# vibevoice-community/VibeVoice

Hardware: AMD Instinct MI355X
Metric: audio-sec/wall-sec (higher is better)
Workload: dtype bf16

## Files before the change

include/vvhip.h:

```cpp
#ifndef VVHIP_H
#define VVHIP_H
#include <stdint.h>
#ifdef __cplusplus
extern "C" {
#endif
typedef struct vv_ctx vv_ctx;

typedef struct vv_config {
    int lm_hidden, lm_layers, lm_heads, lm_kv_heads, lm_head_dim, lm_inter, lm_vocab;
    float lm_eps;
    int head_layers, head_ffn, latent_dim;
    float head_eps;
    int n_filters, n_ratios, ratios[8];
    int n_stages, enc_depths[8];
    int sem_dim;
    int has_acoustic_encoder;
    float codec_eps;
    int n_slots;
    int max_ctx;
    int max_rows;
    int xsplit;
    int attn_splits;
    int enc_frames;
    int use_graph;
// ... 56 lines not shown
int vv_diffusion_sample_rows(vv_ctx*, void* stream, int n, const float* cond_dev, const float* noise_dev,
                             const float* step_noise_dev, const float* cfg_rows_dev, float* latent_out_dev);
int vv_set_schedule_general(vv_ctx* ctx, int n_steps, const float* t, const float* coef8, int stochastic, void* stream);
int vv_diffusion_sample_general(vv_ctx* ctx, void* stream, int n, const float* cond_dev, const float* noise_dev,
                                const float* step_noise_dev, float cfg_scale, const float* cfg_rows_dev, float* latent_out_dev);
int vv_head_forward(vv_ctx* ctx, void* stream, int n, const float* noisy_dev, const float* t_host,
                    const float* cond_dev, float* out_dev);

int vv_codec_decode(vv_ctx* ctx, void* stream, int slot, int frames, const float* latent_dev,
                    float* audio_out_dev, int apply_speech_factors);
int vv_semantic_encode(vv_ctx* ctx, void* stream, int slot, int frames, const float* audio_dev,
                       float* sem_out_dev);
int vv_codec_chain_batch(vv_ctx* ctx, void* stream, int n, const int* slots, const float* latent_dev,
                         float* audio_out_dev, float* sem_out_dev, int apply_speech_factors);
int vv_acoustic_encode(vv_ctx* ctx, void* stream, int frames, const float* wav_dev, float* mean_out_dev);
int vv_acoustic_encode_ragged(vv_ctx* ctx, void* stream, int frames, long long valid_samples, const float* wav_dev, float* mean_out_dev);
int vv_set_enc_pass_frames(vv_ctx* ctx, int frames_per_pass);
int vv_audio_to_pcm16(vv_ctx* ctx, void* stream, int n, int samples, const float* audio_dev, int16_t* pcm_out_dev);
int vv_resampler_set(vv_ctx* ctx, int rs, int L, int M, int T, const float* coef_host, int n_streams, void* stream);
int vv_resampler_reset(vv_ctx* ctx, void* stream, int rs, int n, const int* stream_ids_host);
typedef struct vv_resample_row { int stream; int n_in; int flush; } vv_resample_row;
int vv_resample_rows(vv_ctx* ctx, void* stream, int rs, int n, const vv_resample_row* rows_host, const float* audio_dev, int ld_in,
                     void* out_dev, int ld_out, int out_fmt, int* n_out_host);
int vv_resample_once(vv_ctx* ctx, void* stream, int L, int M, int T, const float* coef_dev, int n, int n_in, const float* audio_dev,
                     int ld_in, float* out_dev, int ld_out);
int vv_tempo_set(vv_ctx* ctx, int tp, const float* window_host, int n_streams, void* stream);
int vv_tempo_reset(vv_ctx* ctx, void* stream, int tp, int n, const int* stream_ids_host);
#define VV_TEMPO_OVER_CAPACITY 3
typedef struct vv_tempo_row { int stream; int n_in; int flush; int P; int Q; } vv_tempo_row;
int vv_tempo_rows(vv_ctx* ctx, void* stream, int tp, int n, const vv_tempo_row* rows_host, const float* audio_dev, int ld_in,
                  void* out_dev, int ld_out, int out_fmt, int* n_out_host, int* offsets_dev, int ld_off);
int vv_tempo_once(vv_ctx* ctx, void* stream, const float* window_dev, int P, int Q, int n, int n_in, const float* audio_dev, int ld_in,
                  float* out_dev, int ld_out, int* offsets_dev, int ld_off);
int vv_level_set(vv_ctx* ctx, int lv, int A, int H, float ceiling, int n_streams, void* stream);
int vv_level_reset(vv_ctx* ctx, void* stream, int lv, int n, const int* stream_ids_host);
typedef struct vv_level_row { int stream; int n_in; int flush; float gain; } vv_level_row;
int vv_level_rows(vv_ctx* ctx, void* stream, int lv, int n, const vv_level_row* rows_host, const float* audio_dev, int ld_in, void* out_dev,
                  int ld_out, int out_fmt, int* n_out_host);
int vv_level_once(vv_ctx* ctx, void* stream, int A, int H, float gain, float ceiling, int n, int n_in, const float* audio_dev, int ld_in,
                  float* out_dev, int ld_out);
int vv_loud_set(vv_ctx* ctx, int ld, const int* taps_host, int n_streams, void* stream);
int vv_loud_reset(vv_ctx* ctx, void* stream, int ld, int n, const int* stream_ids_host);
typedef struct vv_loud_row { int stream; int n_in; int flush; float t; float g0; float wmax; } vv_loud_row;
int vv_loud_rows(vv_ctx* ctx, void* stream, int ld, int n, const vv_loud_row* rows_host, const float* audio_dev, int ld_in, void* out_dev,
                 int ld_out, int out_fmt, int* n_out_host);
int vv_loud_energy(vv_ctx* ctx, void* stream, const double* taps_dev, int n, int n_in, const float* audio_dev, int ld_in,
                   long long* energies_dev, int ld_e, long long* fine_dev, int ld_f);
int vv_loud_once(vv_ctx* ctx, void* stream, const double* taps_dev, float t, float g0, float wmax, int n, int n_in, const float* audio_dev,
                 int ld_in, float* out_dev, int ld_out, float* gain_dev, int ld_gain, long long* energies_dev, int ld_e);
int vv_codec_reset(vv_ctx* ctx, void* stream, int slot);
int vv_connect(vv_ctx* ctx, void* stream, int n, const float* latent_dev, const float* sem_dev,
               float* embeds_out_dev);

int64_t vv_packed_bytes(int N, int K);
int vv_pack_matrix(void* stream, const float* src_dev, void* dst_dev, int N, int K);
int vv_unpack_matrix(void* stream, const void* packed_dev, float* dst_dev, int N, int K);
int vv_lora_merge_raw(void* stream, const void* base_packed_dev, void* dst_packed_dev, int N, int K,
                      const float* a_dev, const float* b_dev, int r, float scale, int delta_bf16);
int vv_gemm_raw(void* stream, const void* w_packed_dev, const void* w2_packed_dev, const float* x_dev,
                float* y_dev, int T, int N, int K, int ldx, int ldy, int pro, int epi,
                const float* nw_dev, float eps, const float* bias_dev, const float* nscale_dev,
                int xsplit, int ksplit, int nontemporal);
#define VV_GEMV_REFUSED 1
typedef struct vv_gemv_case_args {
    const void* W; const void* W2; const float* X; float* Y;
    int T, N, K, ldx, ldy;
    int pro, epi;
    const float* nw; float eps; const float* bias; const float* nscale;
    const float* mod_scale; const float* mod_shift; int ld_mod;
    const float* addvec; int x_row_mod, add_rows_per_vec;
    const float* gate; int ld_gate;
    float* z; float* x0p; const float* coef; float cfg; int n_cfg; const float* sde_noise;
    int kgrid; float* yparts; const float* xa; int n_xa; const float* ya; int n_ya; int part_stride;
    int sl_n, sl_T, sl_x, sl_y; int sl_id[8];
    const float* dw_hist; const float* dw_w; const float* dw_b; const float* dw_gamma; const float* dw_nw;
    float* dw_xout; float* dw_hnew;
    const float* cfg_rows;
} vv_gemv_case_args;
int vv_gemv_case(void* stream, const vv_gemv_case_args* args, int xsplit, int* form_out);
int64_t vv_w13_twin_bytes(int N, int K);
int vv_w13_pack_matrix(void* stream, const void* packed_dev, void* twin_dev, int N, int K);
int vv_w13_unpack_matrix(void* stream, const void* twin_dev, void* packed_dev, int N, int K);
int vv_w13_gemv_case(void* stream, const vv_gemv_case_args* args, const void* twin_dev, const void* twin2_dev, int mr, int wpb);
int vv_gemm3_raw(vv_ctx* ctx, void* stream, const void* w_packed_dev, const void* w2_packed_dev, const float* x_dev, int T, int N, int K,
                 int epi, const float* nw_dev, float eps, const float* bias_dev, float* y_dev, void* xp_scratch, void* yp_scratch);
int vv_profile_begin(vv_ctx* ctx);
int vv_profile_end(vv_ctx* ctx, int64_t* launches, double* total_ms, double* bytes);
int vv_profile_replay(vv_ctx* ctx, void* stream, int reps, int64_t* launches, double* total_ms, double* bytes);
int vv_profile_replay_family(vv_ctx* ctx, void* stream, int family, int reps, int64_t* launches, double* total_ms, double* bytes);
int64_t vv_stat(vv_ctx* ctx, int what);

#pragma GCC visibility pop
#ifdef __cplusplus
}
#endif
#endif
```

vibevoice_amd/_lib.py:

```python
import ctypes as C
import os

HERE = os.path.dirname(os.path.abspath(__file__))
LIB_PATH = os.environ.get("VVHIP_LIB", os.path.join(HERE, "libvvhip.so"))


class VVConfig(C.Structure):
    _fields_ = [
        ("lm_hidden", C.c_int), ("lm_layers", C.c_int), ("lm_heads", C.c_int), ("lm_kv_heads", C.c_int),
        ("lm_head_dim", C.c_int), ("lm_inter", C.c_int), ("lm_vocab", C.c_int), ("lm_eps", C.c_float),
        ("head_layers", C.c_int), ("head_ffn", C.c_int), ("latent_dim", C.c_int), ("head_eps", C.c_float),
        ("n_filters", C.c_int), ("n_ratios", C.c_int), ("ratios", C.c_int * 8),
        ("n_stages", C.c_int), ("enc_depths", C.c_int * 8), ("sem_dim", C.c_int),
        ("has_acoustic_encoder", C.c_int), ("codec_eps", C.c_float),
        ("n_slots", C.c_int), ("max_ctx", C.c_int), ("max_rows", C.c_int), ("xsplit", C.c_int),
        ("attn_splits", C.c_int), ("enc_frames", C.c_int), ("use_graph", C.c_int), ("tts_layers", C.c_int),
    ]


class VVRow(C.Structure):
    _fields_ = [("cache", C.c_int), ("pos", C.c_int)]


_P = C.c_void_p
# ... 35 lines not shown
class VVLoudRow(C.Structure):
    _fields_ = [("stream", C.c_int), ("n_in", C.c_int), ("flush", C.c_int), ("t", C.c_float), ("g0", C.c_float), ("wmax", C.c_float)]


GEMV_REFUSED = 1
TEMPO_OVER_CAPACITY = 3
_SIGS = {
    "vv_create": (C.c_int, [C.POINTER(VVConfig), C.POINTER(_P)]),
    "vv_create_shared": (C.c_int, [C.POINTER(VVConfig), _P, C.POINTER(_P)]),
    "vv_destroy": (None, [_P]),
    "vv_last_error": (C.c_char_p, [_P]),
    "vv_num_weights": (C.c_int, [_P]),
    "vv_weight_info": (C.c_int, [_P, C.c_int, C.c_char_p, C.c_int, C.POINTER(C.c_int64), C.POINTER(C.c_int)]),
    "vv_upload": (C.c_int, [_P, C.c_char_p, _P, C.c_int, C.c_int64]),
    "vv_set_speech_factors": (C.c_int, [_P, C.c_float, C.c_float]),
    "vv_set_valid_tokens": (C.c_int, [_P, C.POINTER(C.c_int), C.c_int]),
    "vv_set_schedule": (C.c_int, [_P, C.c_int, C.POINTER(C.c_float), C.POINTER(C.c_float), _P]),
    "vv_set_schedule_sde": (C.c_int, [_P, C.c_int, C.POINTER(C.c_float), C.POINTER(C.c_float), _P]),
    "vv_set_schedule_general": (C.c_int, [_P, C.c_int, C.POINTER(C.c_float), C.POINTER(C.c_float), C.c_int, _P]),
    "vv_lm_forward": (C.c_int, [_P, _P, C.c_int, C.POINTER(VVRow), _P, _P]),
    "vv_lm_forward_range": (C.c_int, [_P, _P, C.c_int, C.POINTER(VVRow), _P, _P, C.c_int, C.c_int, C.c_int]),
    "vv_kv_import": (C.c_int, [_P, _P, C.c_int, C.c_int, C.c_int, _P, _P, C.c_int]),
    "vv_kv_import_at": (C.c_int, [_P, _P, C.c_int, C.c_int, C.c_int, C.c_int, _P, _P, C.c_int]),
    "vv_add_type_embedding": (C.c_int, [_P, _P, C.c_int, _P, C.c_int, _P]),
    "vv_eos_logit": (C.c_int, [_P, _P, C.c_int, _P, _P]),
    "vv_embed": (C.c_int, [_P, _P, C.c_int, C.POINTER(C.c_int), _P]),
    "vv_lm_logits": (C.c_int, [_P, _P, C.c_int, _P, _P]),
    "vv_lm_logits_full": (C.c_int, [_P, _P, C.c_int, _P, _P]),
    "vv_lm_warp_valid": (C.c_int, [_P, _P, C.c_int, _P, _P, C.c_float, C.c_float, C.c_int, C.c_int, C.c_float, C.c_float, _P, _P]),
    "vv_noise_rows": (C.c_int, [_P, _P, C.c_int, C.POINTER(VVNoiseKey), C.c_uint32, C.c_int, C.c_int, C.c_int, _P]),
    "vv_diffusion_sample": (C.c_int, [_P, _P, C.c_int, _P, _P, C.c_float, _P]),
    "vv_diffusion_sample_sde": (C.c_int, [_P, _P, C.c_int, _P, _P, _P, C.c_float, _P]),
    "vv_diffusion_sample_rows": (C.c_int, [_P, _P, C.c_int, _P, _P, _P, _P, _P]),
    "vv_diffusion_sample_general": (C.c_int, [_P, _P, C.c_int, _P, _P, _P, C.c_float, _P, _P]),
    "vv_head_forward": (C.c_int, [_P, _P, C.c_int, _P, C.POINTER(C.c_float), _P, _P]),
    "vv_codec_decode": (C.c_int, [_P, _P, C.c_int, C.c_int, _P, _P, C.c_int]),
    "vv_semantic_encode": (C.c_int, [_P, _P, C.c_int, C.c_int, _P, _P]),
    "vv_codec_chain_batch": (C.c_int, [_P, _P, C.c_int, _P, _P, _P, _P, C.c_int]),
    "vv_acoustic_encode": (C.c_int, [_P, _P, C.c_int, _P, _P]),
    "vv_acoustic_encode_ragged": (C.c_int, [_P, _P, C.c_int, C.c_longlong, _P, _P]),
    "vv_kv_move": (C.c_int, [_P, _P, C.c_int, C.c_int, C.c_int]),
    "vv_kv_export": (C.c_int, [_P, _P, C.c_int, C.c_int, C.c_int, C.c_int, _P, _P, C.c_int]),
    "vv_kv_snapshot_bytes": (C.c_int64, [_P, C.c_int]),
    "vv_kv_snapshot": (C.c_int, [_P, _P, C.c_int, C.c_int, _P, _P]),
    "vv_kv_restore": (C.c_int, [_P, _P, C.c_int, C.c_int, _P, _P]),
    "vv_set_enc_pass_frames": (C.c_int, [_P, C.c_int]),
    "vv_audio_to_pcm16": (C.c_int, [_P, _P, C.c_int, C.c_int, _P, _P]),
    "vv_resampler_set": (C.c_int, [_P, C.c_int, C.c_int, C.c_int, C.c_int, _P, C.c_int, _P]),
    "vv_resampler_reset": (C.c_int, [_P, _P, C.c_int, C.c_int, C.POINTER(C.c_int)]),
    "vv_resample_rows": (C.c_int, [_P, _P, C.c_int, C.c_int, C.POINTER(VVResampleRow), _P, C.c_int, _P, C.c_int, C.c_int,
                                   C.POINTER(C.c_int)]),
    "vv_resample_once": (C.c_int, [_P, _P, C.c_int, C.c_int, C.c_int, _P, C.c_int, C.c_int, _P, C.c_int, _P, C.c_int]),
    "vv_tempo_set": (C.c_int, [_P, C.c_int, _P, C.c_int, _P]),
    "vv_tempo_reset": (C.c_int, [_P, _P, C.c_int, C.c_int, C.POINTER(C.c_int)]),
    "vv_tempo_rows": (C.c_int, [_P, _P, C.c_int, C.c_int, C.POINTER(VVTempoRow), _P, C.c_int, _P, C.c_int, C.c_int, C.POINTER(C.c_int), _P,
                                C.c_int]),
    "vv_tempo_once": (C.c_int, [_P, _P, _P, C.c_int, C.c_int, C.c_int, C.c_int, _P, C.c_int, _P, C.c_int, _P, C.c_int]),
    "vv_level_set": (C.c_int, [_P, C.c_int, C.c_int, C.c_int, C.c_float, C.c_int, _P]),
    "vv_level_reset": (C.c_int, [_P, _P, C.c_int, C.c_int, C.POINTER(C.c_int)]),
    "vv_level_rows": (C.c_int, [_P, _P, C.c_int, C.c_int, C.POINTER(VVLevelRow), _P, C.c_int, _P, C.c_int, C.c_int, C.POINTER(C.c_int)]),
    "vv_level_once": (C.c_int, [_P, _P, C.c_int, C.c_int, C.c_float, C.c_float, C.c_int, C.c_int, _P, C.c_int, _P, C.c_int]),
    "vv_loud_set": (C.c_int, [_P, C.c_int, _P, C.c_int, _P]),
    "vv_loud_reset": (C.c_int, [_P, _P, C.c_int, C.c_int, C.POINTER(C.c_int)]),
    "vv_loud_rows": (C.c_int, [_P, _P, C.c_int, C.c_int, C.POINTER(VVLoudRow), _P, C.c_int, _P, C.c_int, C.c_int, C.POINTER(C.c_int)]),
    "vv_loud_energy": (C.c_int, [_P, _P, _P, C.c_int, C.c_int, _P, C.c_int, _P, C.c_int, _P, C.c_int]),
    "vv_loud_once": (C.c_int, [_P, _P, _P, C.c_float, C.c_float, C.c_float, C.c_int, C.c_int, _P, C.c_int, _P, C.c_int, _P, C.c_int, _P, C.c_int]),
    "vv_codec_reset": (C.c_int, [_P, _P, C.c_int]),
    "vv_connect": (C.c_int, [_P, _P, C.c_int, _P, _P, _P]),
    "vv_packed_bytes": (C.c_int64, [C.c_int, C.c_int]),
    "vv_pack_matrix": (C.c_int, [_P, _P, _P, C.c_int, C.c_int]),
    "vv_unpack_matrix": (C.c_int, [_P, _P, _P, C.c_int, C.c_int]),
    "vv_lora_merge_raw": (C.c_int, [_P, _P, _P, C.c_int, C.c_int, _P, _P, C.c_int, C.c_float, C.c_int]),
    "vv_weight_read": (C.c_int, [_P, _P, C.c_char_p, _P]),
    "vv_weight_shape": (C.c_int, [_P, C.c_char_p, C.POINTER(C.c_int), C.POINTER(C.c_int)]),
    "vv_lora_merge": (C.c_int, [_P, _P, C.c_char_p, _P, _P, C.c_int, C.c_float, C.c_int]),
    "vv_lora_reset": (C.c_int, [_P, _P, C.c_char_p]),
    "vv_gemm_raw": (C.c_int, [_P, _P, _P, _P, _P, C.c_int, C.c_int, C.c_int, C.c_int, C.c_int, C.c_int, C.c_int,
                              _P, C.c_float, _P, _P, C.c_int, C.c_int, C.c_int]),
    "vv_gemv_case": (C.c_int, [_P, C.POINTER(VVGemvCase), C.c_int, C.POINTER(C.c_int)]),
    "vv_w13_twin_bytes": (C.c_int64, [C.c_int, C.c_int]),
    "vv_w13_pack_matrix": (C.c_int, [_P, _P, _P, C.c_int, C.c_int]),
    "vv_w13_unpack_matrix": (C.c_int, [_P, _P, _P, C.c_int, C.c_int]),
    "vv_w13_gemv_case": (C.c_int, [_P, C.POINTER(VVGemvCase), _P, _P, C.c_int, C.c_int]),
    "vv_gemm3_raw": (C.c_int, [_P, _P, _P, _P, _P, C.c_int, C.c_int, C.c_int, C.c_int, _P, C.c_float, _P, _P, _P, _P]),
    "vv_profile_begin": (C.c_int, [_P]),
    "vv_profile_end": (C.c_int, [_P, C.POINTER(C.c_int64), C.POINTER(C.c_double), C.POINTER(C.c_double)]),
    "vv_profile_replay": (C.c_int, [_P, _P, C.c_int, C.POINTER(C.c_int64), C.POINTER(C.c_double), C.POINTER(C.c_double)]),
    "vv_profile_replay_family": (C.c_int, [_P, _P, C.c_int, C.c_int, C.POINTER(C.c_int64), C.POINTER(C.c_double), C.POINTER(C.c_double)]),
    "vv_stat": (C.c_int64, [_P, C.c_int]),
    "vv_build_id": (C.c_char_p, []),
    "vv_check": (C.c_int, [_P, _P]),
}

EXPORTS = tuple(_SIGS)
_lib = None


def load():
    global _lib
    if _lib is not None:
        return _lib
    if not os.path.exists(LIB_PATH):
        raise RuntimeError(
            f"{LIB_PATH} is missing: the HIP engine has not been built "
            "(run `python -m vibevoice_amd.build`); there is no CPU/PyTorch fallback")
    from . import build as _build
    if _build.have_sources() and _build.binary_id(LIB_PATH) != _build.source_id():
        import sys
        print(f"[vibevoice_amd] {LIB_PATH} was built from other sources (binary id {_build.binary_id(LIB_PATH)}, sources "
              f"{_build.source_id()}): rebuilding with hipcc (about two minutes)", file=sys.stderr, flush=True)
        try:
            _build.build_locked()
        except Exception as ex:
            raise RuntimeError(
                f"{LIB_PATH} was built from different sources (binary id {_build.binary_id(LIB_PATH)}, sources "
                f"{_build.source_id()}) and could not be rebuilt ({ex}); run `python -m vibevoice_amd.build`") from ex
    lib = C.CDLL(LIB_PATH)
    for name, (res, args) in _SIGS.items():
        fn = getattr(lib, name)
        fn.restype = res
        fn.argtypes = args
    _lib = lib
    return lib
```

vibevoice_amd/csrc/engine.hip:

```cpp
#include "engine_ctx.h"
#include "vv_w13.h"

thread_local char g_err[512] = "";
std::shared_mutex g_dev_mu;
std::mutex g_family_mu;

int fail(vv_ctx* ctx, const char* fmt, ...) {
    va_list ap; va_start(ap, fmt);
    char* dst = ctx ? ctx->err : g_err;
    vsnprintf(dst, 512, fmt, ap);
    va_end(ap);
    if (ctx) snprintf(g_err, 512, "%s", ctx->err);
    return -1;
}

int ring_acquire(vv_ctx* ctx) {
    const int slot = ctx->ring_i;
    ctx->ring_i = (ctx->ring_i + 1) % vv_ctx::RING;
    if (ctx->ring_used[slot]) hipEventSynchronize(ctx->ring_ev[slot]);
    ctx->ring_used[slot] = true;
    return slot;
}

void* dalloc(vv_ctx* ctx, size_t bytes, bool zero) {
// ... 9 lines not shown
void dfree(vv_ctx* ctx, void* p) {
    if (!p) return;
    if (ctx) ctx->allocs.erase(p);
    hipFree(p);
}

int add_w(vv_ctx* ctx, const std::string& name, int kind, int64_t nelem, bool optional) {
    Weight w; w.name = name; w.kind = kind; w.nelem = nelem; w.optional = optional;
    ctx->widx[name] = (int)ctx->w.size();
    ctx->w.push_back(w);
    return (int)ctx->w.size() - 1;
}
void add_mat(vv_ctx* ctx, const std::string& name, int N, int K, void* base, int ntile_off, int pk, int Cin, int Cout, int ksz,
             int stride, int64_t src_nelem) {
    int i = add_w(ctx, name, W_MAT, src_nelem < 0 ? (int64_t)N * K : src_nelem);
    Weight& w = ctx->w[i];
    w.N = N; w.K = K; w.pk = pk; w.Cin = Cin; w.Cout = Cout; w.ksz = ksz; w.stride = stride;
    const int k_tiles = (K + 31) / 32;
    w.dev = (char*)base + (int64_t)ntile_off * k_tiles * 1024;
}
void* walloc(vv_ctx* ctx, size_t bytes, bool zero) {
    if (!ctx->creating) return dalloc(ctx, bytes, zero);
    if (ctx->parent) {
        vv_ctx* p = ctx->parent;
        if (ctx->wshare_i >= p->wallocs.size() || p->wallocs[ctx->wshare_i].second != bytes) {
            fail(ctx, "vv_create_shared: weight allocation %zu (%zu bytes) does not match the parent's -- different model configuration", ctx->wshare_i, bytes);
            return nullptr;
        }
        void* q = p->wallocs[ctx->wshare_i++].first;
        ctx->wallocs.push_back({q, bytes});
        return q;
    }
    void* q = dalloc(ctx, bytes, zero);
    ctx->wallocs.push_back({q, bytes});
    return q;
}
void* alloc_packed(vv_ctx* ctx, int N, int K) { return walloc(ctx, (size_t)vv_packed_elems(N, K) * 2); }
float* add_vec(vv_ctx* ctx, const std::string& name, int64_t n, float* dst, int kind, int rep) {
    int i = add_w(ctx, name, kind, n);
    if (!dst) dst = (float*)walloc(ctx, (size_t)n * rep * 4);
    ctx->w[i].dev = dst; ctx->w[i].rep = rep;
    return dst;
}

VVGemm mk_gemm(const void* W, const float* X, float* Y, int T, int N, int K, int ldx, int ldy) {
    VVGemm g; memset(&g, 0, sizeof(g));
    g.W = (const u32x4*)W; g.X = X; g.Y = Y; g.T = T; g.N = N; g.K = K; g.ldx = ldx; g.ldy = ldy;
    g.pro = VV_PRO_NONE; g.epi = VV_EPI_STORE; g.ksplit = 0; g.nt = 0; g.eps = 1e-6f;
    return g;
}
int ksplit_parts(const vv_ctx* ctx, VVGemm& g, float* parts, int part_stride) {
    const int n_tiles = (g.N + 15) / 16, k_tiles = (g.K + 31) / 32;
    constexpr int max_tiles = 128;
    if (g.T > 4 || n_tiles > max_tiles || k_tiles < 96) return 0;
    const int ks = 3;
    g.kgrid = ks; g.yparts = parts; g.part_stride = part_stride;
    if (!vv_gemv_ok(&g)) { g.kgrid = 0; g.yparts = nullptr; g.part_stride = 0; return 0; }
    return ks - 1;
}
int graphed_run(vv_ctx* ctx, const std::string& key, hipStream_t st, const std::function<int()>& body) {
    if (!ctx->c.use_graph || ctx->prof_on) { VV_SHARED; return body(); }
    auto it = ctx->graphs.find(key);
    if (it == ctx->graphs.end()) {
        if (ctx->seen.size() > 8192) ctx->seen.clear();
        if (ctx->seen.insert(key).second) { VV_SHARED; return body(); }
        hipGraph_t graph = nullptr;
        GraphEntry ge; ge.last_use = 0;
        bool captured = false;
        {
            std::unique_lock<std::shared_mutex> lk(g_dev_mu);
            HIPCHK(ctx, hipStreamBeginCapture(st, hipStreamCaptureModeRelaxed));
            const int r = body();
            const hipError_t e = hipStreamEndCapture(st, &graph);
            if (r == 0 && e == hipSuccess) {
                size_t nn = 0;
                if (hipGraphGetNodes(graph, nullptr, &nn) == hipSuccess && nn) {
                    std::vector<hipGraphNode_t> nodes(nn);
                    if (hipGraphGetNodes(graph, nodes.data(), &nn) == hipSuccess)
                        for (size_t i = 0; i < nn; ++i) { hipGraphNodeType t; if (hipGraphNodeGetType(nodes[i], &t) == hipSuccess && t != hipGraphNodeTypeKernel) ctx->foreign_nodes++; }
                }
                HIPCHK(ctx, hipGraphInstantiate(&ge.exec, graph, nullptr, nullptr, 0));
                hipGraphDestroy(graph);
                captured = true;
            } else {
                (void)hipGetLastError();
                ctx->capture_fallbacks++;
                snprintf(ctx->last_capture_issue, sizeof(ctx->last_capture_issue), "capture of '%s': body rc %d, hipStreamEndCapture: %s", key.c_str(), r, hipGetErrorString(e));
            }
        }
        if (!captured) {
            VV_SHARED;
            const int r2 = body();
            if (r2 != 0) {
                char prev[200]; snprintf(prev, sizeof(prev), "%s", ctx->err);
                return fail(ctx, "%s; the eager re-run failed as well (%s).  If another host thread called a device-wide synchronize "
                                 "(torch.cuda.synchronize()) during the capture, the stream is lost: synchronize streams or events instead", ctx->last_capture_issue, prev);
            }
            return 0;
        }
        if (ctx->graphs.size() >= ctx->graph_cap) {
            std::vector<std::pair<uint64_t, std::string>> order;
            for (auto& g : ctx->graphs) order.push_back({g.second.last_use, g.first});
            std::sort(order.begin(), order.end());
            std::unique_lock<std::shared_mutex> lk(g_dev_mu);
            HIPCHK(ctx, hipDeviceSynchronize());
            for (size_t i = 0; i < order.size() / 4 + 1; ++i) {
                auto v = ctx->graphs.find(order[i].second);
                hipGraphExecDestroy(v->second.exec);
                ctx->graphs.erase(v);
            }
        }
        it = ctx->graphs.emplace(key, ge).first;
    }
    it->second.last_use = ++ctx->graph_tick;
    VV_SHARED;
    HIPCHK(ctx, hipGraphLaunch(it->second.exec, st));
    return 0;
}

int drop_graphs(vv_ctx* ctx, std::initializer_list<const char*> prefixes) {
    auto hit = [&](const std::string& key) {
        for (const char* p : prefixes) if (key.rfind(p, 0) == 0) return true;
        return false;
    };
    bool any = false;
    for (auto& g : ctx->graphs) if (hit(g.first)) { any = true; break; }
    if (!any) return 0;
    HIPCHK(ctx, hipDeviceSynchronize());
    for (auto it = ctx->graphs.begin(); it != ctx->graphs.end();) {
        if (hit(it->first)) { hipGraphExecDestroy(it->second.exec); it = ctx->graphs.erase(it); } else ++it;
    }
    return 0;
}

extern "C" const char* vv_last_error(vv_ctx* ctx) { return ctx ? ctx->err : g_err; }

#ifndef VV_BUILD_ID
#define VV_BUILD_ID "unknown"
#endif
extern "C" const char* vv_build_id() { return "VVHIP_BUILD_ID=" VV_BUILD_ID; }

static int create_impl(const vv_config* cfg, vv_ctx* parent, vv_ctx** out) {
    VV_SHARED;
    vv_ctx* ctx = new vv_ctx();
    ctx->c = *cfg; ctx->err[0] = 0;
    ctx->parent = parent; ctx->creating = true;
    vv_config& c = ctx->c;
    if (c.max_rows < 1 || c.max_rows > 16384) { delete ctx; return fail(nullptr, "max_rows must be in [1,16384]"); }
    if (c.lm_head_dim != 64 && c.lm_head_dim != 128) { delete ctx; return fail(nullptr, "head_dim must be 64 or 128"); }
    if (c.lm_kv_heads < 1 || c.lm_heads % c.lm_kv_heads != 0 || c.lm_heads / c.lm_kv_heads > 16) {
        const int hq = c.lm_heads, hkv = c.lm_kv_heads;
        delete ctx;
        return fail(nullptr, "lm_heads=%d / lm_kv_heads=%d: the GQA group size must be an integer <= 16", hq, hkv);
    }
    if (c.xsplit < 1 || c.xsplit > 3) c.xsplit = 2;
    if (c.attn_splits < 1) c.attn_splits = 128;
    if (c.enc_frames < 1) c.enc_frames = 1;
    if (getenv("VVHIP_GRAPH_CAP")) ctx->graph_cap = (size_t)std::max(4, atoi(getenv("VVHIP_GRAPH_CAP")));
    c.max_ctx = (c.max_ctx + 127) & ~127;
    const int H = ctx->H = c.lm_hidden, D = ctx->D = c.lm_head_dim, Hq = ctx->Hq = c.lm_heads, Hkv = ctx->Hkv = c.lm_kv_heads;
    const int I = ctx->I = c.lm_inter;
    const int QKV = ctx->QKV = (Hq + 2 * Hkv) * D;
    const int R = c.max_rows;
    ctx->embed = walloc(ctx, (size_t)c.lm_vocab * H * 2);
    { int i = add_w(ctx, "lm.embed_tokens.weight", W_TABLE, (int64_t)c.lm_vocab * H); ctx->w[i].dev = ctx->embed; }
    { int i = add_w(ctx, "lm_head.weight", W_TABLE, (int64_t)c.lm_vocab * H, true); ctx->w[i].dev = nullptr; }
    ctx->inv_freq = add_vec(ctx, "lm.rope.inv_freq", D / 2);
    ctx->lm_norm = add_vec(ctx, "lm.norm.weight", H);
    if (c.tts_layers > 0) {
        if (c.tts_layers >= c.lm_layers) { delete ctx; return fail(nullptr, "tts_layers must be < lm_layers"); }
        ctx->tts_types = add_vec(ctx, "tts_input_types.weight", 2 * (int64_t)H);
        ctx->eos_w1 = alloc_packed(ctx, H, H); add_mat(ctx, "eos.fc1.weight", H, H, ctx->eos_w1, 0);
        ctx->eos_b1 = add_vec(ctx, "eos.fc1.bias", H);
        ctx->eos_w2 = alloc_packed(ctx, 1, H); add_mat(ctx, "eos.fc2.weight", 1, H, ctx->eos_w2, 0);
        ctx->eos_b2 = add_vec(ctx, "eos.fc2.bias", 1);
    }
    {
        const char* e = getenv("VVHIP_W13");
        const bool on = !(e && e[0] == '0') && c.xsplit == 1;
        ctx->w13_on = parent ? parent->w13_on : on && vv_w13_shape_ok(c.head_ffn, H) && vv_w13_shape_ok(H, c.head_ffn);
        ctx->w13_lm = parent ? parent->w13_lm : on && !(e && !strcmp(e, "head"));
    }
    auto twin = [&](bool want, bool lm, const void* src, int N, int K, int n_par = 1) -> void* {
        if (!want || !vv_w13_shape_ok(N, K)) return nullptr;
        ctx->twins.push_back({walloc(ctx, (size_t)vv_w13_bytes(N, K)), src, N, K, lm});
        for (int j = 0; j < n_par; ++j) ctx->w[ctx->w.size() - 1 - j].twin = (int)ctx->twins.size() - 1;
        return ctx->twins.back().planes;
    };
    ctx->layers.resize(c.lm_layers);
    for (int l = 0; l < c.lm_layers; ++l) {
        auto& L = ctx->layers[l];
        char nm[128]; snprintf(nm, 128, "lm.layers.%d.", l);
        std::string p(nm);
        L.ln1 = add_vec(ctx, p + "input_layernorm.weight", H);
        L.ln2 = add_vec(ctx, p + "post_attention_layernorm.weight", H);
        L.wqkv = alloc_packed(ctx, QKV, H);
        L.bqkv = (float*)walloc(ctx, (size_t)QKV * 4);
        add_mat(ctx, p + "self_attn.q_proj.weight", Hq * D, H, L.wqkv, 0);
        add_mat(ctx, p + "self_attn.k_proj.weight", Hkv * D, H, L.wqkv, Hq * D / 16);
        add_mat(ctx, p + "self_attn.v_proj.weight", Hkv * D, H, L.wqkv, (Hq + Hkv) * D / 16);
        L.tqkv = twin(ctx->w13_lm, true, L.wqkv, QKV, H, 3);
        add_vec(ctx, p + "self_attn.q_proj.bias", Hq * D, L.bqkv);
        add_vec(ctx, p + "self_attn.k_proj.bias", Hkv * D, L.bqkv + Hq * D);
        add_vec(ctx, p + "self_attn.v_proj.bias", Hkv * D, L.bqkv + (Hq + Hkv) * D);
        L.wo = alloc_packed(ctx, H, Hq * D); add_mat(ctx, p + "self_attn.o_proj.weight", H, Hq * D, L.wo, 0); L.to = twin(ctx->w13_lm, true, L.wo, H, Hq * D);
        L.wg = alloc_packed(ctx, I, H); add_mat(ctx, p + "mlp.gate_proj.weight", I, H, L.wg, 0); L.tg = twin(ctx->w13_lm, true, L.wg, I, H);
        L.wu = alloc_packed(ctx, I, H); add_mat(ctx, p + "mlp.up_proj.weight", I, H, L.wu, 0); L.tu = twin(ctx->w13_lm, true, L.wu, I, H);
        L.wd = alloc_packed(ctx, H, I); add_mat(ctx, p + "mlp.down_proj.weight", H, I, L.wd, 0); L.td = twin(ctx->w13_lm, true, L.wd, H, I);
    }
    const int n_caches = 2 * c.n_slots;
    ctx->head_stride = (int64_t)c.max_ctx * D;
    ctx->layer_stride = ctx->head_stride * Hkv;
    ctx->cache_stride = ctx->layer_stride * c.lm_layers;
    ctx->kc = dalloc(ctx, (size_t)ctx->cache_stride * n_caches * 2);
    ctx->vc = dalloc(ctx, (size_t)ctx->cache_stride * n_caches * 2);
    ctx->rows_cap = std::max(2048, c.max_rows);
    ctx->rows_dev = (VVRow*)dalloc(ctx, sizeof(VVRow) * ctx->rows_cap);
    hipHostMalloc((void**)&ctx->rows_pin, sizeof(VVRow) * (size_t)ctx->rows_cap * vv_ctx::RING);
    for (int i = 0; i < vv_ctx::RING; ++i) hipEventCreateWithFlags(&ctx->ring_ev[i], hipEventDisableTiming);
    ctx->ids_cap = std::max(64, c.max_rows);
    ctx->ids_dev = (int*)dalloc(ctx, sizeof(int) * ctx->ids_cap);
    hipHostMalloc((void**)&ctx->ids_pin, sizeof(int) * (size_t)ctx->ids_cap * vv_ctx::RING);
    ctx->h = (float*)dalloc(ctx, (size_t)R * H * 4);
    ctx->h_parts = (float*)dalloc(ctx, (size_t)2 * R * H * 4);
    ctx->qkv = (float*)dalloc(ctx, (size_t)R * QKV * 4);
    ctx->qrot = (float*)dalloc(ctx, (size_t)R * Hq * D * 4);
    ctx->attn = (float*)dalloc(ctx, (size_t)R * Hq * D * 4);
    ctx->act = (float*)dalloc(ctx, (size_t)R * I * 4);
    if (R >= 64 && (H % 8) == 0 && ((Hq * D) % 8) == 0 && (I % 8) == 0) {
        ctx->xp = dalloc(ctx, (size_t)vv_packed_elems(R, std::max(H, Hq * D)) * 2);
        ctx->actp = dalloc(ctx, (size_t)vv_packed_elems(R, I) * 2);
        ctx->tile3_ok = c.xsplit == 1;
        if (ctx->tile3_ok) {
            ctx->gws.g3_bytes = (size_t)8 * std::min(R, 1024) * std::max(ctx->QKV, H) * 4;
            ctx->gws.g3_partials = (float*)dalloc(ctx, ctx->gws.g3_bytes, false);
            if (!ctx->gws.g3_partials) ctx->gws.g3_bytes = 0;
        }
        const char* no_ks = getenv("VVHIP_NO_KSPLIT");
        if (ctx->tile3_ok && R >= 1024 && !(no_ks && no_ks[0] == '1')) {
            ctx->gws.partials = (float*)dalloc(ctx, (size_t)256 * 32 * 512 * 16, false);
            ctx->gws.flags = (unsigned*)dalloc(ctx, 256 * sizeof(unsigned));
            if (hipHostMalloc((void**)&ctx->gws.err, sizeof(unsigned), hipHostMallocMapped) == hipSuccess && ctx->gws.err) *ctx->gws.err = 0u;
            else ctx->gws.err = nullptr;
        }
    }
    ctx->attn2_ok = c.xsplit == 1;
    if (c.xsplit == 1 && R > 4 && (H % 32) == 0 && ((Hq * D) % 32) == 0 && (I % 32) == 0) {
        const int kx = std::max(H, Hq * D), ka = std::max(I, c.head_ffn);
        ctx->p16_x = dalloc(ctx, (size_t)vv_packed_elems(16, kx) * 2);
        ctx->p16_act = dalloc(ctx, (size_t)vv_packed_elems(16, ka + 32) * 2);
        ctx->p16_y = dalloc(ctx, (size_t)vv_packed_elems(16, kx) * 2);
        ctx->ssq_a = (float*)dalloc(ctx, (size_t)(H / 16) * 16 * 4);
        ctx->ssq_b = (float*)dalloc(ctx, (size_t)(H / 16) * 16 * 4);
        ctx->p16_ok = ctx->p16_x && ctx->p16_act && ctx->p16_y && ctx->ssq_a && ctx->ssq_b;
    }
    ctx->rope_tab = dalloc(ctx, (size_t)c.max_ctx * (D / 2) * 8, false);
    ctx->ws_rows = std::min(R, 64);
    const size_t np = (size_t)ctx->ws_rows * Hkv * c.attn_splits * 16;
    ctx->pm = (float*)dalloc(ctx, np * 4); ctx->pl = (float*)dalloc(ctx, np * 4); ctx->po = (float*)dalloc(ctx, np * D * 4);
    const int L = c.latent_dim, HL = c.head_layers, HF = ctx->HF = c.head_ffn;
    const int MODW = ctx->MODW = HL * 3 * H + 2 * H;
    ctx->h_in = alloc_packed(ctx, H, L); add_mat(ctx, "head.noisy_images_proj.weight", H, L, ctx->h_in, 0);
    ctx->h_cond = alloc_packed(ctx, H, H); add_mat(ctx, "head.cond_proj.weight", H, H, ctx->h_cond, 0);
    ctx->h_t0 = alloc_packed(ctx, H, 256); add_mat(ctx, "head.t_embedder.mlp.0.weight", H, 256, ctx->h_t0, 0);
    ctx->h_t2 = alloc_packed(ctx, H, H); add_mat(ctx, "head.t_embedder.mlp.2.weight", H, H, ctx->h_t2, 0);
    ctx->h_ada = alloc_packed(ctx, MODW, H);
    ctx->hl.resize(HL);
    auto htwin = [&](const void* src, int N, int K) {
        twin(ctx->w13_on, false, src, N, K);
        return (int)ctx->w.size() - 1;
    };
    for (int l = 0; l < HL; ++l) {
        char nm[128]; snprintf(nm, 128, "head.layers.%d.", l);
        std::string p(nm);
        ctx->hl[l].norm = add_vec(ctx, p + "norm.weight", H);
        add_mat(ctx, p + "adaLN_modulation.1.weight", 3 * H, H, ctx->h_ada, l * 3 * H / 16);
        ctx->hl[l].wg = alloc_packed(ctx, HF, H); add_mat(ctx, p + "ffn.gate_proj.weight", HF, H, ctx->hl[l].wg, 0); ctx->hl[l].ig = htwin(ctx->hl[l].wg, HF, H);
        ctx->hl[l].wu = alloc_packed(ctx, HF, H); add_mat(ctx, p + "ffn.up_proj.weight", HF, H, ctx->hl[l].wu, 0); ctx->hl[l].iu = htwin(ctx->hl[l].wu, HF, H);
        ctx->hl[l].wd = alloc_packed(ctx, H, HF); add_mat(ctx, p + "ffn.down_proj.weight", H, HF, ctx->hl[l].wd, 0); ctx->hl[l].id = htwin(ctx->hl[l].wd, H, HF);
    }
    add_mat(ctx, "head.final_layer.adaLN_modulation.1.weight", 2 * H, H, ctx->h_ada, HL * 3 * H / 16);
    ctx->h_out = alloc_packed(ctx, L, H); add_mat(ctx, "head.final_layer.linear.weight", L, H, ctx->h_out, 0);
    const int R2 = 16;
    ctx->cproj = (float*)dalloc(ctx, (size_t)R2 * H * 4);
    ctx->mod = (float*)dalloc(ctx, (size_t)R2 * MODW * 4);
    for (HeadGen& g : ctx->hg) {
        g.zz = (float*)dalloc(ctx, (size_t)R2 * L * 4);
        g.x0p = (float*)dalloc(ctx, (size_t)R2 * L * 4);
        g.xh = (float*)dalloc(ctx, (size_t)R2 * H * 4);
    }
    ctx->head_tail = c.xsplit == 1 && L == 64 && (H % 32) == 0 && vv_head_tail_init() == 0;
    if (const char* e = getenv("VVHIP_SOLVER_FUSE"); e && e[0] == '0') ctx->solver_fuse = false;
    if (const char* e = getenv("VVHIP_NAN_PROBE"); e && e[0] == '1') {
        ctx->probe_rec = (unsigned*)dalloc(ctx, PROBE_MAX * 16);
        ctx->probe_on = ctx->probe_rec != nullptr;
    }
    ctx->xh_parts = (float*)dalloc(ctx, (size_t)4 * R2 * H * 4);
    ctx->hact = (float*)dalloc(ctx, (size_t)R2 * HF * 4);
    ctx->eps = (float*)dalloc(ctx, (size_t)R2 * L * 4);
    ctx->tmp1 = (float*)dalloc(ctx, (size_t)64 * H * 4);
    ctx->tmp2 = (float*)dalloc(ctx, (size_t)64 * 256 * 4);
    auto mk_conn = [&](vv_ctx::Conn& cn, const std::string& p, int din) {
        cn.fc1 = alloc_packed(ctx, H, din); add_mat(ctx, p + "fc1.weight", H, din, cn.fc1, 0);
        cn.b1 = add_vec(ctx, p + "fc1.bias", H);
        cn.norm = add_vec(ctx, p + "norm.weight", H);
        cn.fc2 = alloc_packed(ctx, H, H); add_mat(ctx, p + "fc2.weight", H, H, cn.fc2, 0);
        cn.b2 = add_vec(ctx, p + "fc2.bias", H);
    };
    mk_conn(ctx->ac_conn, "ac_conn.", L);
    if (c.sem_dim > 0) mk_conn(ctx->sem_conn, "sem_conn.", c.sem_dim);
    ctx->ct1 = (float*)dalloc(ctx, (size_t)256 * H * 4);
    if (build_codec(ctx, ctx->dec, "dec.", true, L, 1, c.n_slots)) { *out = ctx; return -1; }
    if (c.sem_dim > 0 && build_codec(ctx, ctx->senc, "senc.", false, c.sem_dim, 1, c.n_slots)) { *out = ctx; return -1; }
    if (c.has_acoustic_encoder && build_codec(ctx, ctx->aenc, "aenc.", false, L, c.enc_frames, 1)) { *out = ctx; return -1; }
    if (hipDeviceSynchronize() != hipSuccess || ctx->err[0]) { *out = ctx; return fail(ctx, "vv_create: allocation failed: %s", ctx->err); }
    ctx->creating = false;
    if (parent) {
        if (ctx->wshare_i != parent->wallocs.size() || ctx->w.size() != parent->w.size()) {
            *out = ctx;
            return fail(ctx, "vv_create_shared: the child registered %zu weight buffers / %zu parameters, the parent %zu / %zu -- different model configuration",
                        ctx->wshare_i, ctx->w.size(), parent->wallocs.size(), parent->w.size());
        }
        for (size_t i = 0; i < ctx->w.size(); ++i) {
            if (ctx->w[i].name != parent->w[i].name || ctx->w[i].nelem != parent->w[i].nelem) { *out = ctx; return fail(ctx, "vv_create_shared: parameter table differs at '%s'", ctx->w[i].name.c_str()); }
            ctx->w[i].loaded = parent->w[i].loaded;
            if (ctx->w[i].name == "lm_head.weight") ctx->w[i].dev = parent->w[i].dev;
        }
        ctx->lm_head = parent->lm_head; ctx->lm_head_loaded = parent->lm_head_loaded;
        ctx->scaling = parent->scaling; ctx->bias = parent->bias;
        { std::lock_guard<std::mutex> fl(g_family_mu); parent->n_children++; }
    }
    *out = ctx;
    return 0;
}

extern "C" int vv_create(const vv_config* cfg, vv_ctx** out) { return create_impl(cfg, nullptr, out); }

extern "C" int vv_create_shared(const vv_config* cfg, vv_ctx* parent, vv_ctx** out) {
    if (!parent) return fail(nullptr, "vv_create_shared: no parent context");
    if (parent->parent) return fail(nullptr, "vv_create_shared: the parent is itself a shared context; share from the owner of the weights");
    for (auto& w : parent->w)
        if (!w.loaded && !w.optional) return fail(nullptr, "vv_create_shared: parent parameter '%s' is not uploaded yet", w.name.c_str());
    vv_config a = *cfg, b = parent->c;
    a.n_slots = b.n_slots; a.max_ctx = b.max_ctx; a.max_rows = b.max_rows; a.attn_splits = b.attn_splits; a.use_graph = b.use_graph;
    if (a.xsplit < 1 || a.xsplit > 3) a.xsplit = 2;
    if (a.enc_frames < 1) a.enc_frames = 1;
    if (memcmp(&a, &b, sizeof(vv_config)) != 0) return fail(nullptr, "vv_create_shared: the model fields of the configuration differ from the parent's");
    int r = create_impl(cfg, parent, out);
    if (r != 0 && *out) { vv_ctx* c = *out; c->parent = nullptr; }
    return r;
}

static void destroy_impl(vv_ctx* ctx) {
    if (!ctx) return;
    hipDeviceSynchronize();
    {
        std::lock_guard<std::mutex> fl(g_family_mu);
        if (ctx->n_children > 0) { ctx->zombie = true; return; }
    }
    vv_ctx* par = ctx->parent;
    for (auto& g : ctx->graphs) hipGraphExecDestroy(g.second.exec);
    if (ctx->side_ready) {
        for (int j = 0; j < 8; ++j) { hipStreamDestroy(ctx->side[j]); hipEventDestroy(ctx->ev_join[j]); }
        hipEventDestroy(ctx->ev_fork);
    }
    for (void* p : ctx->allocs) hipFree(p);
    ctx->allocs.clear();
    if (ctx->stage) hipFree(ctx->stage);
    hipHostFree(ctx->rows_pin); hipHostFree(ctx->ids_pin);
    if (ctx->gws.err) hipHostFree(ctx->gws.err);
    for (int i = 0; i < vv_ctx::RING; ++i) if (ctx->ring_ev[i]) hipEventDestroy(ctx->ring_ev[i]);
    delete ctx;
    bool last_child = false;
    if (par) { std::lock_guard<std::mutex> fl(g_family_mu); last_child = (--par->n_children == 0 && par->zombie); }
    if (last_child) destroy_impl(par);
}
extern "C" void vv_destroy(vv_ctx* ctx) {
    VV_SHARED;
    destroy_impl(ctx);
}

extern "C" int vv_num_weights(vv_ctx* ctx) { return (int)ctx->w.size(); }
extern "C" int vv_weight_info(vv_ctx* ctx, int idx, char* name, int cap, int64_t* nelem, int* loaded) {
    if (idx < 0 || idx >= (int)ctx->w.size()) return fail(ctx, "weight index out of range");
    const Weight& w = ctx->w[idx];
    snprintf(name, cap, "%s", w.name.c_str());
    if (nelem) *nelem = w.nelem;
    if (loaded) *loaded = (w.loaded || w.optional) ? 1 : 0;
    return 0;
}

extern "C" int vv_upload(vv_ctx* ctx, const char* name, const void* src, int src_dtype, int64_t nelem) {
    VV_SHARED;
    auto it = ctx->widx.find(name);
    if (it == ctx->widx.end()) return fail(ctx, "unknown parameter '%s'", name);
    Weight& w = ctx->w[it->second];
    if (ctx->parent) return fail(ctx, "parameter '%s': this context shares its parent's weights -- upload through the parent", name);
    {
        std::lock_guard<std::mutex> fl(g_family_mu);
        if (ctx->n_children > 0)
            return fail(ctx, "parameter '%s': %d shared context(s) were created from this one and hold snapshots derived from its parameters -- "
                             "destroy them (model.close_lanes()), upload / merge, then fork again", name, ctx->n_children);
    }
    if (nelem != w.nelem) return fail(ctx, "parameter '%s': expected %lld elements, got %lld", name, (long long)w.nelem, (long long)nelem);
    const size_t esz = src_dtype ? 2 : 4;
    hipPointerAttribute_t attr;
    bool on_dev = (hipPointerGetAttributes(&attr, src) == hipSuccess) && (attr.type == hipMemoryTypeDevice);
    (void)hipGetLastError();
    const void* dsrc = src;
    if (!on_dev) {
        const size_t need = (size_t)nelem * esz;
        if (need > ctx->stage_bytes) {
            if (ctx->stage) hipFree(ctx->stage);
            ctx->stage = nullptr; ctx->stage_bytes = 0;
            HIPCHK(ctx, hipMalloc(&ctx->stage, need));
            ctx->stage_bytes = need;
        }
        HIPCHK(ctx, hipMemcpy(ctx->stage, src, need, hipMemcpyHostToDevice));
        dsrc = ctx->stage;
    }
    hipStream_t st = 0;
    if (w.kind == W_TABLE) {
        if (w.name == "lm_head.weight" && !ctx->lm_head_loaded) {
            ctx->lm_head = dalloc(ctx, (size_t)nelem * 2, false);
            if (!ctx->lm_head) return -1;
            ctx->lm_head_loaded = true; w.dev = ctx->lm_head;
        }
        if (src_dtype) HIPCHK(ctx, hipMemcpy(w.dev, dsrc, (size_t)nelem * 2, hipMemcpyDeviceToDevice));
        else VVCHK(vv_cvt_launch(dsrc, w.dev, nelem, 1, st));
    } else if (w.kind == W_MAT) {
        VVCHK(vv_pack_launch(dsrc, src_dtype, w.dev, w.N, w.K, w.pk, w.Cin, w.Cout, w.ksz, w.stride, st));
        VVTRY(lora_rebase(ctx, it->second, st));
        VVTRY(w13_repack(ctx, it->second, st));
    } else {
        const float* f32 = (const float*)dsrc;
        float* tmp = nullptr;
        if (src_dtype) {
            tmp = (float*)dalloc(ctx, (size_t)nelem * 4, false);
            if (!tmp) return -1;
            VVCHK(vv_cvt_launch(dsrc, tmp, nelem, 0, st));
            f32 = tmp;
        }
        if (w.kind == W_DW) {
            VVCHK(vv_dw_transpose_launch(f32, (float*)w.dev, (int)(nelem / 7), st));
        } else if (w.kind == W_BIAS_REP) {
            for (int r = 0; r < w.rep; ++r)
                HIPCHK(ctx, hipMemcpyAsync((float*)w.dev + (size_t)r * nelem, f32, (size_t)nelem * 4, hipMemcpyDeviceToDevice, st));
        } else {
            HIPCHK(ctx, hipMemcpyAsync(w.dev, f32, (size_t)nelem * 4, hipMemcpyDeviceToDevice, st));
        }
        HIPCHK(ctx, hipStreamSynchronize(st));
        dfree(ctx, tmp);
    }
    HIPCHK(ctx, hipStreamSynchronize(st));
    w.loaded = true;
    ctx->rope_ready = false;
    return 0;
}

int w13_repack(vv_ctx* ctx, int widx, hipStream_t st) {
    const Weight& w = ctx->w[widx];
    if (w.twin < 0) return 0;
    W13Twin& t = ctx->twins[w.twin];
    const int tile0 = (int)(((const char*)w.dev - (const char*)t.src) / ((int64_t)(t.K / 32) * 1024));
    VVCHK(vv_w13_pack_rows_launch(t.src, t.planes, t.N, t.K, tile0, w.N / 16, st));
    t.exact = -1;
    return 0;
}

static bool w13_ok_words(const W13Twin& t, std::vector<unsigned>& ok, bool folded) {
    const int n_tiles = t.N / 16;
    ok.resize(folded ? 1 : n_tiles);
    return hipMemcpy(ok.data(), (const char*)t.planes + vv_w13_plane_bytes(t.N, t.K) + (size_t)(folded ? 2 * n_tiles : n_tiles) * 4, ok.size() * 4,
                     hipMemcpyDeviceToHost) == hipSuccess;
}

extern "C" int vv_set_speech_factors(vv_ctx* ctx, float scaling, float bias) {
    VV_SHARED;
    ctx->scaling = scaling; ctx->bias = bias;
    return drop_graphs(ctx, {"dec:1:", "chain:1:"});
}

extern "C" int vv_set_valid_tokens(vv_ctx* ctx, const int* ids, int n) {
    VV_SHARED;
    if (n < 1 || n > 16) return fail(ctx, "n_valid must be in [1,16]");
    const int H = ctx->H;
    const void* table = ctx->lm_head_loaded ? ctx->lm_head : ctx->embed;
    void* rows = dalloc(ctx, (size_t)n * H * 2, false);
    if (!rows) return -1;
    for (int i = 0; i < n; ++i) {
        if (ids[i] < 0 || ids[i] >= ctx->c.lm_vocab) return fail(ctx, "token id %d out of range", ids[i]);
        HIPCHK(ctx, hipMemcpy((char*)rows + (size_t)i * H * 2, (const char*)table + (size_t)ids[i] * H * 2, (size_t)H * 2, hipMemcpyDeviceToDevice));
    }
    if (!ctx->valid_w) ctx->valid_w = alloc_packed(ctx, 16, H);
    VVCHK(vv_pack_launch(rows, 1, ctx->valid_w, n, H, 0, 0, 0, 0, 0, 0));
    HIPCHK(ctx, hipDeviceSynchronize());
    dfree(ctx, rows);
    ctx->n_valid = n;
    for (int i = 0; i < n; ++i) ctx->valid_ids[i] = ids[i];
    return 0;
}
extern "C" int vv_check(vv_ctx* ctx, void* stream) {
    if (!ctx) return -1;
    return ksplit_check(ctx, (hipStream_t)stream);
}
extern "C" int vv_audio_to_pcm16(vv_ctx* ctx, void* stream, int n, int samples, const float* audio_dev, int16_t* pcm_out_dev) {
    VV_SHARED;
    hipStream_t st = (hipStream_t)stream;
    if (n < 1 || samples < 1) return fail(ctx, "vv_audio_to_pcm16: n and samples must be positive");
    VVCHK(vv_pcm16_launch(audio_dev, (short*)pcm_out_dev, n, samples, st));
    return 0;
}
extern "C" int vv_connect(vv_ctx* ctx, void* stream, int n, const float* latent_dev, const float* sem_dev, float* out_dev) {
    VV_SHARED;
    hipStream_t st = (hipStream_t)stream;
    const int H = ctx->H, L = ctx->c.latent_dim;
    for (int i0 = 0; i0 < n; i0 += 16) {
        const int nn = std::min(16, n - i0);
        float* out = out_dev + (size_t)i0 * H;
        VVGemm a1 = mk_gemm(ctx->ac_conn.fc1, latent_dev + (size_t)i0 * L, ctx->ct1, nn, H, L, L, H);
        a1.epi = VV_EPI_BIAS; a1.bias = ctx->ac_conn.b1; GEMM(a1);
        VVGemm a2 = mk_gemm(ctx->ac_conn.fc2, ctx->ct1, out, nn, H, H, H, H);
        a2.pro = VV_PRO_RMS; a2.nw = ctx->ac_conn.norm; a2.eps = 1e-6f; a2.epi = VV_EPI_BIAS; a2.bias = ctx->ac_conn.b2; GEMM(a2);
        if (sem_dev) {
            const int S = ctx->c.sem_dim;
            VVGemm s1 = mk_gemm(ctx->sem_conn.fc1, sem_dev + (size_t)i0 * S, ctx->ct1, nn, H, S, S, H);
            s1.epi = VV_EPI_BIAS; s1.bias = ctx->sem_conn.b1; GEMM(s1);
            VVGemm s2 = mk_gemm(ctx->sem_conn.fc2, ctx->ct1, out, nn, H, H, H, H);
            s2.pro = VV_PRO_RMS; s2.nw = ctx->sem_conn.norm; s2.eps = 1e-6f; s2.epi = VV_EPI_RESID; s2.bias = ctx->sem_conn.b2; GEMM(s2);
        }
    }
    return 0;
}

extern "C" int64_t vv_packed_bytes(int N, int K) { return vv_packed_elems(N, K) * 2; }
extern "C" int vv_pack_matrix(void* stream, const float* src_dev, void* dst_dev, int N, int K) {
    return vv_pack_launch(src_dev, 0, dst_dev, N, K, 0, 0, 0, 0, 0, (hipStream_t)stream);
}
extern "C" int64_t vv_stat(vv_ctx* ctx, int what) {
    switch (what) {
        case 0: return ctx->launches;
        case 2: return ctx->prof_raw_ns;
        case 3: return ctx->prof_ev_over_ns;
        case 5: return ctx->foreign_nodes;
        case 4: return ctx->capture_fallbacks;
        case 6: return ctx->seam_launches;
        case 8: return ctx->solver_fused;
        case 7: return ctx->lora_base_bytes;
        case 9: case 11: {
            VV_SHARED;
            if (hipDeviceSynchronize() != hipSuccess) return -1;
            std::vector<unsigned> tail;
            if (what == 11) {
                int64_t n = 0;
                for (const W13Twin& t : ctx->twins) {
                    if (!w13_ok_words(t, tail, false)) return -1;
                    for (unsigned v : tail) n += v == 0;
                }
                return n;
            }
            auto exact = [&](int widx) {
                const int ti = ctx->w[widx].twin;
                return ti >= 0 && w13_ok_words(ctx->twins[ti], tail, true) && tail[0] == 1;
            };
            int64_t n = 0;
            for (const auto& l : ctx->hl) {
                if (exact(l.ig) && exact(l.iu)) n += 2;
                if (exact(l.id)) n += 1;
            }
            return n;
        }
        case 10: {
            int64_t n = 0;
            for (const W13Twin& t : ctx->twins) n += t.lm;
            return n;
        }
        default: return (int64_t)ctx->graphs.size();
    }
}
```

vibevoice_amd/csrc/engine_ctx.h:

```cpp
#pragma once
#include <algorithm>
#include <cmath>
#include <cstdarg>
#include <cstdio>
#include <cstdlib>
#include <cstring>
#include <functional>
#include <initializer_list>
#include <map>
#include <mutex>
#include <set>
#include <shared_mutex>
#include <string>
#include <vector>
#include "../../include/vvhip.h"
#include "vv_common.h"
#include "vv_launch.h"

namespace vv_engine {
struct VVShiftH { float* buf; int T, hist, C; };
enum WKind { W_MAT = 0, W_VEC = 1, W_DW = 2, W_TABLE = 3, W_BIAS_REP = 4 };

struct Weight {
    std::string name;
    int kind = W_VEC;
    int64_t nelem = 0;
    void* dev = nullptr;
    int N = 0, K = 0, pk = 0, Cin = 0, Cout = 0, ksz = 0, stride = 0;
    int rep = 1;
    bool loaded = false;
    bool optional = false;
    int twin = -1;
};

struct W13Twin { void* planes; const void* src; int N, K; bool lm; int exact = -1, used = -1; };

struct Block {
    int C;
    float *norm_w, *ffn_norm_w, *gamma, *ffn_gamma, *dw_w, *dw_b, *b1, *b2;
    void *w1, *w2;
    float* nb;
    float* nst;
    int64_t nb_stride;
};

struct ConvG {
    void* w; float* bias;
    int K, N, ldx;
    int rows_per_frame;
};

struct Stage {
    int C, Tpf;
    int hist;
    float* xs;
    float* xs2;
    float* xfinal;
    bool fused;
    bool pp;
    int64_t sl_stride;
    std::vector<Block> blocks;
    ConvG in;
};

struct CodecNet {
    bool decoder = false;
    int Fmax = 1, in_dim = 1, out_dim = 1, in_hist = 6, in_Tpf = 1;
    std::vector<float*> in_buf;
    std::vector<std::vector<Stage>> st;
    ConvG head;
    std::vector<float*> u;
    std::map<std::pair<uint64_t, int>, std::pair<void*, int>> shift_tab;
    int maxC = 1;
    int kd = 0, ke = 1 << 30;
    bool head_batch = false;
    int64_t in_stride = 0, u_stride = 0;
};

struct GraphEntry { hipGraphExec_t exec; uint64_t last_use; };

struct HeadGen { float *xh = nullptr, *zz = nullptr, *x0p = nullptr, *m2 = nullptr; };

}
using namespace vv_engine;

constexpr int PROBE_MAX = 1024;

struct vv_ctx {
    vv_config c;
    char err[512];
    std::vector<Weight> w;
    std::map<std::string, int> widx;
    int H, D, Hq, Hkv, I, QKV;
    struct Layer { float *ln1, *ln2, *bqkv; void *wqkv, *wo, *wg, *wu, *wd; void *tqkv, *to, *tg, *tu, *td; };
    std::vector<Layer> layers;
    float *lm_norm = nullptr, *inv_freq = nullptr;
    int ws_rows = 0;
    void* rope_tab = nullptr; bool rope_ready = false;
    float *tts_types = nullptr, *eos_b1 = nullptr, *eos_b2 = nullptr; void *eos_w1 = nullptr, *eos_w2 = nullptr;
    void *embed = nullptr, *lm_head = nullptr;
    bool lm_head_loaded = false;
    void* valid_w = nullptr; int n_valid = 0;
    int valid_ids[16] = {0};
    void *kc = nullptr, *vc = nullptr;
    int64_t cache_stride = 0, head_stride = 0, layer_stride = 0;
    VVRow* rows_dev = nullptr; VVRow* rows_pin = nullptr; int rows_cap = 2048;
    int* ids_dev = nullptr; int* ids_pin = nullptr; int ids_cap = 64;
    static constexpr int RING = 32;
    hipEvent_t ring_ev[RING] = {}; bool ring_used[RING] = {}; int ring_i = 0;
    float *h = nullptr, *qkv = nullptr, *qrot = nullptr, *attn = nullptr, *act = nullptr;
    float *h_parts = nullptr, *xh_parts = nullptr;
    void *xp = nullptr, *actp = nullptr;
    bool tile3_ok = false, attn2_ok = false;
    VVGemmWs gws = {nullptr, nullptr, nullptr, nullptr, 0};
    void *p16_x = nullptr, *p16_act = nullptr, *p16_y = nullptr, *p16_shift = nullptr; float *ssq_a = nullptr, *ssq_b = nullptr; bool p16_ok = false;
    size_t p16_shift_tile = 0;
    float *pm = nullptr, *pl = nullptr, *po = nullptr;
    int HF = 0, MODW = 0;
    struct HLayer { float* norm; void *wg, *wu, *wd; int ig, iu, id; };
    bool w13_on = false, w13_lm = false;
    std::vector<W13Twin> twins;
    std::vector<HLayer> hl;
    void *h_in = nullptr, *h_cond = nullptr, *h_t0 = nullptr, *h_t2 = nullptr, *h_ada = nullptr, *h_out = nullptr;
    int n_steps = 0;
    float *temb = nullptr, *coef = nullptr, *tvals = nullptr;
    bool sde_on = false;
    bool general_on = false;
    float* mod_all = nullptr; size_t mod_all_bytes = 0;
    float* ada_in = nullptr;
    void* ada_p = nullptr;
    float *cproj = nullptr, *mod = nullptr, *hact = nullptr, *eps = nullptr;
    HeadGen hg[2];
    bool head_tail = false;
    bool solver_fuse = true;
    float *tmp1 = nullptr, *tmp2 = nullptr;
    struct Conn { void *fc1, *fc2; float *b1, *b2, *norm; } ac_conn, sem_conn;
    float *ct1 = nullptr;
    CodecNet dec, aenc, senc;
    int enc_pass = 0;
    hipStream_t side[8] = {}; hipEvent_t ev_fork = nullptr, ev_join[8] = {}; bool side_ready = false;
    float scaling = 1.f, bias = 0.f;
    int hop = 3200;
    void* stage = nullptr; size_t stage_bytes = 0;
    std::map<std::string, GraphEntry> graphs;
    uint64_t graph_tick = 0; size_t graph_cap = 512;
    std::set<std::string> seen;
    std::set<void*> allocs;
    vv_ctx* parent = nullptr; int n_children = 0; bool zombie = false, creating = false;
    unsigned* probe_rec = nullptr; std::vector<std::string> probe_names; bool probe_on = false; int probe_calls = 0;
    int64_t foreign_nodes = 0;
    int64_t capture_fallbacks = 0; char last_capture_issue[256] = "";
    std::vector<std::pair<void*, size_t>> wallocs; size_t wshare_i = 0;
    struct LoraBase { void* snap; size_t bytes; bool merged; };
    std::map<int, LoraBase> lora_base;
    int64_t lora_base_bytes = 0;
    struct RowStage { int n_streams = 0; std::vector<int64_t> total; std::vector<char> flushed; };
    struct Resampler : RowStage { int L = 0, M = 0, T = 0; float* coef = nullptr; float* hist = nullptr; };
    static constexpr int N_RESAMPLERS = 4;
    Resampler rs[N_RESAMPLERS];
    struct Tempo : RowStage { float* window = nullptr; float* hist = nullptr; int* dstate = nullptr; std::vector<int> P, Q; };
    static constexpr int N_TEMPOS = 4;
    Tempo tp[N_TEMPOS];
    struct Level : RowStage { int A = 0, H = 0; float c = 0.f; float* hist = nullptr; std::vector<float> gain; };
    static constexpr int N_LEVELS = 4;
    Level lv[N_LEVELS];
    struct Loud : RowStage { double* taps = nullptr; int* hist = nullptr; VVLdState* state = nullptr; long long* part = nullptr;
                             std::vector<float> t, g0, wmax; };
    static constexpr int N_LOUDS = 4;
    Loud loud[N_LOUDS];
    int64_t launches = 0;
    int64_t solver_fused = 0;
    int64_t seam_launches = 0;
    bool prof_on = false;
    std::vector<hipEvent_t> prof_ev;
    int prof_n = 0;
    double prof_bytes = 0.0;
    struct ProfRec { int T, N, K, pro, epi, dual; double bytes; int gemv; };
    std::vector<ProfRec> prof_rec;
    std::vector<VVGemm> prof_gemv;
    double prof_gemv_bytes = 0.0;
    struct ProfLaunch { int family; double bytes; std::function<int(hipStream_t)> fn; };
    std::vector<ProfLaunch> prof_other;
    int64_t prof_raw_ns = 0, prof_ev_over_ns = 0;
    hipStream_t prof_stream = nullptr;
#ifdef VV_GEMM_TIMING
    unsigned long long* tl_base = nullptr; int tl_idx = 0;
    struct TlRec { int T, N, K, pro, epi; };
    std::vector<TlRec> tl_rec;
#endif
};

extern thread_local char g_err[512];
extern std::shared_mutex g_dev_mu;
#define VV_SHARED std::shared_lock<std::shared_mutex> _vv_dev_lk(g_dev_mu)
extern std::mutex g_family_mu;
int fail(vv_ctx* ctx, const char* fmt, ...);
#define HIPCHK(ctx, e) do { hipError_t _e = (e); if (_e != hipSuccess) return fail(ctx, "%s:%d hip error %s", __FILE__, __LINE__, hipGetErrorString(_e)); } while (0)
#define VVCHK(e) do { int _r = (e); if (_r != 0) return _r < 0 ? fail(ctx, "%s:%d launch failed (%d): hip error %d (%s)", __FILE__, __LINE__, _r, g_vv_launch_err, hipGetErrorString((hipError_t)g_vv_launch_err)) : _r; } while (0)
#define VVTRY(e) do { if (int _r = (e)) return _r; } while (0)

void* dalloc(vv_ctx* ctx, size_t bytes, bool zero = true);
void dfree(vv_ctx* ctx, void* p);
void* walloc(vv_ctx* ctx, size_t bytes, bool zero = true);
void* alloc_packed(vv_ctx* ctx, int N, int K);
int add_w(vv_ctx* ctx, const std::string& name, int kind, int64_t nelem, bool optional = false);
void add_mat(vv_ctx* ctx, const std::string& name, int N, int K, void* base, int ntile_off, int pk = 0, int Cin = 0, int Cout = 0,
             int ksz = 0, int stride = 0, int64_t src_nelem = -1);
float* add_vec(vv_ctx* ctx, const std::string& name, int64_t n, float* dst = nullptr, int kind = W_VEC, int rep = 1);
VVGemm mk_gemm(const void* W, const float* X, float* Y, int T, int N, int K, int ldx, int ldy);
int ksplit_parts(const vv_ctx* ctx, VVGemm& g, float* parts, int part_stride);
int ring_acquire(vv_ctx* ctx);
int build_codec(vv_ctx* ctx, CodecNet& net, const std::string& pfx, bool decoder, int vae_dim, int Fmax, int n_slots);
int ksplit_check(vv_ctx* ctx, hipStream_t st);
int p16_gemv(vv_ctx* ctx, hipStream_t st, const void* W, const void* W2, const void* Xp, float* Y, void* Yp, const float* bias,
             const float* gate, int T, int N, int K, int ldy, int ld_gate, int epi);
int p16_go(vv_ctx* ctx, hipStream_t st, const VVGemv16p& a, int epi, int flags);
VVGemv16p p16_args(const void* W, const void* W2, const void* Xp, float* Y, void* Yp, int T, int N, int K, int ldy);
void nan_probe(vv_ctx* ctx, hipStream_t st, const char* name, const void* p, size_t n);
void nan_probe_report(vv_ctx* ctx, hipStream_t st, const char* what);
int gemm_prof(vv_ctx* ctx, const VVGemm& g, hipStream_t st);
int lora_rebase(vv_ctx* ctx, int widx, hipStream_t st);
int w13_repack(vv_ctx* ctx, int widx, hipStream_t st);

#ifdef VV_GEMM_TIMING
int gemm_tl(vv_ctx* ctx, VVGemm g, hipStream_t st);
#define GEMM(g) do { ctx->launches++; VVCHK(gemm_tl(ctx, g, st)); } while (0)
#else
#define GEMM(g) do { ctx->launches++; if (ctx->prof_on) VVCHK(gemm_prof(ctx, g, st)); else VVCHK(vv_gemm_launch(g, ctx->c.xsplit, st)); } while (0)
#endif

int graphed_run(vv_ctx* ctx, const std::string& key, hipStream_t st, const std::function<int()>& body);
int drop_graphs(vv_ctx* ctx, std::initializer_list<const char*> prefixes);
template <class F>
static int graphed(vv_ctx* ctx, const std::string& key, hipStream_t st, F&& body) { return graphed_run(ctx, key, st, std::ref(body)); }
```

vibevoice_amd/csrc/engine_head.hip:

```cpp
#include "engine_ctx.h"
#include "pass_plan.h"
#include "vv_w13.h"

static int set_schedule(vv_ctx* ctx, int n_steps, const float* t, const float* coef, int width, void* stream, bool stochastic = false) {
    VV_SHARED;
    hipStream_t st = (hipStream_t)stream;
    if (n_steps < 1 || n_steps > 64) return fail(ctx, "n_steps must be in [1,64]");
    const int H = ctx->H;
    if (!ctx->temb) {
        ctx->temb = (float*)dalloc(ctx, (size_t)64 * H * 4);
        ctx->coef = (float*)dalloc(ctx, 64 * 8 * 4);
        ctx->tvals = (float*)dalloc(ctx, 64 * 4);
    }
    const bool general = width == 8;
    if (general && !ctx->hg[0].m2) {
        for (HeadGen& g : ctx->hg) g.m2 = (float*)dalloc(ctx, (size_t)8 * ctx->c.latent_dim * 4);
        if (!ctx->hg[0].m2 || !ctx->hg[1].m2) return fail(ctx, "vv_set_schedule_general: out of device memory");
    }
    float rows[64 * 8] = {};
    for (int i = 0; i < n_steps; ++i)
        for (int j = 0; j < width; ++j) rows[i * 8 + j] = coef[i * width + j];
    ctx->sde_on = general ? stochastic : (width == 6);
    ctx->general_on = general;
    HIPCHK(ctx, hipStreamSynchronize(st));
// ... 167 lines not shown
                      r.step_noise ? r.step_noise + (size_t)s.step * r.n * ctx->c.latent_dim : nullptr};
    s.end = &end;
    const int hr = head_eval(ctx, st, p, s);
    return {hr, hr == 1};
}

static StepDone step_general(vv_ctx* ctx, hipStream_t st, const VVHeadPlan& p, const SampleReq& r, const HeadStep& s) {
    const int L = ctx->c.latent_dim;
    if (head_eval(ctx, st, p, s) < 0) return {-1, false};
    VVSolverStep v{};
    v.eps = s.eps_out; v.coef = ctx->coef + s.step * 8; v.cfg = r.cfg; v.cfg_rows = r.cfg_rows; v.n = r.n; v.L = L;
    v.noise = r.step_noise ? r.step_noise + (size_t)s.step * r.n * L : nullptr;
    v.z_in = s.cur.zz; v.m1_in = s.cur.x0p; v.m2_in = s.cur.m2;
    v.z_out = s.nxt.zz; v.m1_out = s.nxt.x0p; v.m2_out = s.nxt.m2;
    if (s.step + 1 < p.n_steps && ctx->solver_fuse) { v.Win = (const u32x4*)ctx->h_in; v.Xout = s.nxt.xh; v.H = ctx->H; v.xs = ctx->c.xsplit; }
    ctx->launches++;
    const int sr = vv_solver_step_launch(&v, st);
    if (sr == VV_RC_NO_FORM) return {fail(ctx, "vv_diffusion_sample_general: solver.hip has no form for n = %d, latent_dim = %d", r.n, L), false};
    if (sr < 0) return {fail(ctx, "%s:%d launch failed (%d): hip error %d (%s)", __FILE__, __LINE__, sr, g_vv_launch_err, hipGetErrorString((hipError_t)g_vv_launch_err)), false};
    if (sr == 1) ctx->solver_fused++;
    return {sr == 1, true};
}

static int sample_body(vv_ctx* ctx, hipStream_t st, const SampleReq& r) {
    const int H = ctx->H, L = ctx->c.latent_dim, HL = ctx->c.head_layers;
    const int n = r.n, rows = 2 * n;
    ctx->seam_launches = ctx->solver_fused = 0;
    ctx->probe_names.clear();
    nan_probe(ctx, st, "cond (input)", r.cond, (size_t)rows * H);
    nan_probe(ctx, st, "noise (input)", r.noise, (size_t)n * L);
    VVCHK(vv_sampler_init_launch(r.noise, ctx->hg[0].zz, ctx->hg[0].x0p, n * L, st));
    VVGemm gc = mk_gemm(ctx->h_cond, r.cond, ctx->cproj, rows, H, H, H, H);
    gc.nt = 1;
    GEMM(gc);
    const int MODW = ctx->MODW;
    const VVHeadPlan p = head_plan(ctx, rows, ctx->n_steps, true);
    const bool batch_ada = p.ada != VV_ADA_PER_STEP;
    if (batch_ada) {
        const int total = rows * ctx->n_steps;
        if (p.ada == VV_ADA_TILE) {
            ctx->launches += 2;
            VVCHK(vv_ada_pack_launch(ctx->cproj, ctx->temb, ctx->ada_p, rows, ctx->n_steps, H, st));
            VVCHK(vv_gemm3_launch(ctx->h_ada, nullptr, ctx->ada_p, ctx->mod_all, nullptr, nullptr, total, MODW, H, MODW, VV_EPI_STORE, nullptr, st));
        } else {
        VVCHK(vv_ada_in_launch(ctx->cproj, ctx->temb, ctx->ada_in, rows, ctx->n_steps, H, st));
        ctx->launches++;
        for (int t0 = 0; t0 < total; t0 += 16) {
            const int T = std::min(16, total - t0);
            VVGemm ga = mk_gemm(ctx->h_ada, ctx->ada_in + (size_t)t0 * H, ctx->mod_all + (size_t)t0 * MODW, T, MODW, H, H, MODW);
            GEMM(ga);
        }
        }
    }
    nan_probe(ctx, st, "cproj", ctx->cproj, (size_t)rows * H);
    if (batch_ada) nan_probe(ctx, st, "mod_all", ctx->mod_all, (size_t)rows * ctx->n_steps * MODW);
    if (p.sh_tiles) {
        ctx->launches++;
        VVCHK(vv_pack16_tiles_launch(ctx->mod_all, MODW, (int64_t)rows * MODW, HL + 1, (int64_t)3 * H, ctx->p16_shift,
                                     (int64_t)ctx->p16_shift_tile, rows, H, ctx->n_steps * (HL + 1), st));
    }
    int gen = 0; bool have_x = false;
    for (int i = 0; i < ctx->n_steps; ++i) {
        const HeadGen& cur = ctx->hg[gen];
        const HeadStep s{.step = i, .z = cur.zz, .temb = ctx->temb + (size_t)i * H,
                         .mod = batch_ada ? ctx->mod_all + (size_t)i * rows * MODW : nullptr,
                         .sh_tiles = p.sh_tiles ? (const unsigned char*)ctx->p16_shift + (size_t)i * (HL + 1) * ctx->p16_shift_tile : nullptr,
                         .eps_out = ctx->eps, .cur = cur, .nxt = ctx->hg[gen ^ 1], .have_x = have_x, .end = nullptr};
        const StepDone d = p.solver_step ? step_general(ctx, st, p, r, s) : step_shipped(ctx, st, p, r, s);
        if (d.rc < 0) return -1;
        have_x = d.rc == 1;
        gen ^= d.flipped;
        if (ctx->probe_on) {
            const HeadGen& now = ctx->hg[gen];
            char nm[64];
            snprintf(nm, 64, "step %d z%s", i, p.solver_step ? " (general)" : have_x ? " (seam, next gen)" : ""); nan_probe(ctx, st, nm, now.zz, (size_t)rows * L);
            if (!p.solver_step) { snprintf(nm, 64, "step %d x0p", i); nan_probe(ctx, st, nm, now.x0p, (size_t)n * L); }
            if (!p.solver_step && have_x) { snprintf(nm, 64, "step %d next xh", i); nan_probe(ctx, st, nm, now.xh, (size_t)rows * H); }
        }
    }
    VVCHK(vv_copy_launch(r.out, ctx->hg[gen].zz, (size_t)n * L * 4, st));
    return 0;
}

static int head_w13_resolve(vv_ctx* ctx, hipStream_t st) {
    if (!ctx->w13_on) return 0;
    bool changed = false, waited = false;
    for (W13Twin& t : ctx->twins) {
        if (t.lm || t.exact >= 0) continue;
        if (!waited) { HIPCHK(ctx, hipStreamSynchronize(st)); waited = true; }
        unsigned ok = 0;
        HIPCHK(ctx, hipMemcpy(&ok, (const char*)t.planes + vv_w13_plane_bytes(t.N, t.K) + (size_t)2 * (t.N / 16) * 4, 4, hipMemcpyDeviceToHost));
        t.exact = ok == 1;
        if (t.used >= 0 && t.used != t.exact) changed = true;
        t.used = t.exact;
    }
    return changed ? drop_graphs(ctx, {"samp:", "sde:", "rows:", "gen:"}) : 0;
}

static int run_sampler(vv_ctx* ctx, hipStream_t st, const char* key, const SampleReq& r) {
    ctx->launches = 0;
    { VV_SHARED; VVTRY(head_w13_resolve(ctx, st)); }
    const int rc = graphed(ctx, key, st, [&]() { return sample_body(ctx, st, r); });
    nan_probe_report(ctx, st, key);
    return rc;
}

extern "C" int vv_diffusion_sample(vv_ctx* ctx, void* stream, int n, const float* cond_dev, const float* noise_dev, float cfg_scale, float* latent_out_dev) {
    if (ctx->n_steps < 1) return fail(ctx, "vv_set_schedule has not been called");
    if (n < 1 || n > 8) return fail(ctx, "vv_diffusion_sample: n must be in [1,8]");
    if (ctx->general_on) return fail(ctx, "the installed table is a general one (vv_set_schedule_general): sample with vv_diffusion_sample_general");
    if (ctx->sde_on) return fail(ctx, "the schedule is stochastic (vv_set_schedule_sde): sample with vv_diffusion_sample_sde and its per-step noise");
    char key[128]; snprintf(key, 128, "samp:%d:%p:%p:%p:%a", n, (const void*)cond_dev, (const void*)noise_dev, (void*)latent_out_dev, cfg_scale);
    return run_sampler(ctx, (hipStream_t)stream, key, {n, cond_dev, noise_dev, nullptr, cfg_scale, nullptr, latent_out_dev});
}

extern "C" int vv_diffusion_sample_sde(vv_ctx* ctx, void* stream, int n, const float* cond_dev, const float* noise_dev,
                                       const float* step_noise_dev, float cfg_scale, float* latent_out_dev) {
    if (ctx->n_steps < 1) return fail(ctx, "vv_set_schedule_sde has not been called");
    if (n < 1 || n > 8) return fail(ctx, "vv_diffusion_sample_sde: n must be in [1,8]");
    if (ctx->general_on) return fail(ctx, "the installed table is a general one (vv_set_schedule_general): sample with vv_diffusion_sample_general");
    if (!ctx->sde_on) return fail(ctx, "the schedule is deterministic (vv_set_schedule): sample with vv_diffusion_sample");
    if (!step_noise_dev) return fail(ctx, "vv_diffusion_sample_sde: step_noise is null");
    char key[160]; snprintf(key, 160, "sde:%d:%p:%p:%p:%p:%a", n, (const void*)cond_dev, (const void*)noise_dev, (const void*)step_noise_dev,
                            (void*)latent_out_dev, cfg_scale);
    return run_sampler(ctx, (hipStream_t)stream, key, {n, cond_dev, noise_dev, step_noise_dev, cfg_scale, nullptr, latent_out_dev});
}

extern "C" int vv_diffusion_sample_rows(vv_ctx* ctx, void* stream, int n, const float* cond_dev, const float* noise_dev,
                                        const float* step_noise_dev, const float* cfg_rows_dev, float* latent_out_dev) {
    if (ctx->n_steps < 1) return fail(ctx, "vv_set_schedule / vv_set_schedule_sde has not been called");
    if (n < 1 || n > 8) return fail(ctx, "vv_diffusion_sample_rows: n must be in [1,8]");
    if (ctx->general_on) return fail(ctx, "the installed table is a general one (vv_set_schedule_general): sample with vv_diffusion_sample_general");
    if (!cfg_rows_dev) return fail(ctx, "vv_diffusion_sample_rows: cfg_rows is null");
    if (ctx->sde_on && !step_noise_dev) return fail(ctx, "the schedule is stochastic (vv_set_schedule_sde): vv_diffusion_sample_rows needs its per-step noise");
    if (!ctx->sde_on && step_noise_dev) return fail(ctx, "the schedule is deterministic (vv_set_schedule): vv_diffusion_sample_rows takes no step noise");
    char key[192]; snprintf(key, 192, "rows:%d:%p:%p:%p:%p:%p", n, (const void*)cond_dev, (const void*)noise_dev, (const void*)step_noise_dev,
                            (const void*)cfg_rows_dev, (void*)latent_out_dev);
    return run_sampler(ctx, (hipStream_t)stream, key, {n, cond_dev, noise_dev, step_noise_dev, 0.f, cfg_rows_dev, latent_out_dev});
}

extern "C" int vv_diffusion_sample_general(vv_ctx* ctx, void* stream, int n, const float* cond_dev, const float* noise_dev,
                                           const float* step_noise_dev, float cfg_scale, const float* cfg_rows_dev, float* latent_out_dev) {
    if (ctx->n_steps < 1) return fail(ctx, "vv_set_schedule_general has not been called");
    if (n < 1 || n > 8) return fail(ctx, "vv_diffusion_sample_general: n must be in [1,8]");
    if (!ctx->general_on) return fail(ctx, "the installed table is a shipped one (vv_set_schedule / vv_set_schedule_sde): sample with vv_diffusion_sample, _sde or _rows");
    if (ctx->sde_on && !step_noise_dev) return fail(ctx, "the general table is stochastic: vv_diffusion_sample_general needs its per-step noise");
    if (!ctx->sde_on && step_noise_dev) return fail(ctx, "the general table is deterministic: vv_diffusion_sample_general takes no step noise");
    char key[224]; snprintf(key, 224, "gen:%d:%p:%p:%p:%p:%p:%a", n, (const void*)cond_dev, (const void*)noise_dev, (const void*)step_noise_dev,
                            (const void*)cfg_rows_dev, (void*)latent_out_dev, cfg_rows_dev ? 0.f : cfg_scale);
    return run_sampler(ctx, (hipStream_t)stream, key, {n, cond_dev, noise_dev, step_noise_dev, cfg_scale, cfg_rows_dev, latent_out_dev});
}

extern "C" int vv_head_forward(vv_ctx* ctx, void* stream, int n, const float* noisy_dev, const float* t_host, const float* cond_dev, float* out_dev) {
    VV_SHARED;
    hipStream_t st = (hipStream_t)stream;
    if (n < 1 || n > 16) return fail(ctx, "vv_head_forward: n must be in [1,16]");
    const int H = ctx->H;
    for (int i = 1; i < n; ++i) if (t_host[i] != t_host[0]) return fail(ctx, "vv_head_forward: all rows must share one timestep");
    VVTRY(head_w13_resolve(ctx, st));
    float* tdev = ctx->tmp2 + 63 * 256;
    HIPCHK(ctx, hipStreamSynchronize(st));
    HIPCHK(ctx, hipMemcpy(tdev + 128, t_host, 4, hipMemcpyHostToDevice));
    VVCHK(vv_tfreq_launch(tdev + 128, ctx->tmp2, 1, st));
    VVGemm g = mk_gemm(ctx->h_t0, ctx->tmp2, ctx->tmp1, 1, H, 256, 256, H); GEMM(g);
    VVCHK(vv_silu_launch(ctx->tmp1, H, st));
    VVGemm g2 = mk_gemm(ctx->h_t2, ctx->tmp1, ctx->tmp1 + H, 1, H, H, H, H); GEMM(g2);
    VVGemm gc = mk_gemm(ctx->h_cond, cond_dev, ctx->cproj, n, H, H, H, H); GEMM(gc);
    const HeadStep s{.step = 0, .z = noisy_dev, .temb = ctx->tmp1 + H, .mod = nullptr, .sh_tiles = nullptr, .eps_out = out_dev,
                     .cur = ctx->hg[0], .nxt = ctx->hg[1], .have_x = false, .end = nullptr};
    if (head_eval(ctx, st, head_plan(ctx, n, 1, false), s)) return -1;
    HIPCHK(ctx, hipStreamSynchronize(st));
    return 0;
}
```

vibevoice_amd/csrc/engine_lm.hip:

```cpp
#include "engine_ctx.h"
#include "pass_plan.h"

int p16_gemv(vv_ctx* ctx, hipStream_t st, const void* W, const void* W2, const void* Xp, float* Y, void* Yp, const float* bias,
                    const float* gate, int T, int N, int K, int ldy, int ld_gate, int epi) {
    if (ctx->prof_on) {
        const double by = (double)vv_packed_elems(N, K) * 2.0 * (W2 ? 2.0 : 1.0) + (double)vv_packed_elems(16, K) * 2.0 +
                          (Yp ? (double)T * N * 2.0 : (double)T * N * 4.0 * (epi == VV_EPI_RESID || epi == VV_EPI_GATED_RESID ? 2.0 : 1.0));
        ctx->prof_other.push_back({1, by, [=](hipStream_t s) { return vv_gemv16p_launch(W, W2, Xp, Y, Yp, bias, gate, T, N, K, ldy, ld_gate, epi, s); }});
    }
    return vv_gemv16p_launch(W, W2, Xp, Y, Yp, bias, gate, T, N, K, ldy, ld_gate, epi, st);
}

int p16_go(vv_ctx* ctx, hipStream_t st, const VVGemv16p& a, int epi, int flags) {
    if (ctx->prof_on) {
        const double by = (double)vv_packed_elems(a.N, a.K) * 2.0 * (a.W2 ? 2.0 : 1.0) + (double)vv_packed_elems(16, a.K) * 2.0 * ((flags & 2) ? 2.0 : 1.0) +
                          ((epi == VV_EPI_SWIGLU) ? (double)a.T * a.N * 2.0 : (double)a.T * a.N * 4.0 * (epi == VV_EPI_RESID || epi == VV_EPI_GATED_RESID ? 2.0 : 1.0)) +
                          ((flags & 4) ? (double)a.T * a.N * 2.0 : 0.0);
        const VVGemv16p ac = a;
        ctx->prof_other.push_back({1, by, [=](hipStream_t s) { return vv_gemv16p_launch2(&ac, epi, flags, s); }});
    }
    return vv_gemv16p_launch2(&a, epi, flags, st);
}
VVGemv16p p16_args(const void* W, const void* W2, const void* Xp, float* Y, void* Yp, int T, int N, int K, int ldy) {
    VVGemv16p a{};
// ... 22 lines not shown
    const int H = ctx->H, D = ctx->D, Hq = ctx->Hq, Hkv = ctx->Hkv, I = ctx->I, QKV = ctx->QKV;
    for (int l = l0; l < l1; ++l) {
        auto& L = ctx->layers[l];
        char *kl = lm_kc(ctx, l), *vl = lm_vc(ctx, l);
        ctx->launches += 9;
        VVCHK(vv_pack_rows_launch(ctx->h, H, L.ln1, c.lm_eps, ctx->xp, R, H, st));
        const int fq = vv_gemm_qkv_rope_launch(L.wqkv, ctx->xp, L.bqkv, R, H, D, Hq, Hkv, ctx->rows_dev, ctx->rope_tab, ctx->qrot, kl, vl,
                                               ctx->cache_stride, ctx->head_stride, &ctx->gws, st);
        if (fq < 0) return fail(ctx, "vv_gemm_qkv_rope_launch failed (%d)", fq);
        if (fq == 0) {
            VVCHK(vv_gemm3_launch(L.wqkv, nullptr, ctx->xp, ctx->qkv, nullptr, L.bqkv, R, QKV, H, QKV, VV_EPI_BIAS, &ctx->gws, st));
            VVCHK(vv_rope_append_launch(D, ctx->qkv, ctx->rows_dev, ctx->inv_freq, ctx->qrot, kl, vl,
                                        R, Hq, Hkv, ctx->cache_stride, ctx->head_stride, st));
        }
        const bool apk = ((Hq * D) & 31) == 0;
        VVCHK(vv_attn_prefill4_launch(D, ctx->qrot, ctx->rows_dev, kl, vl, R, Hq, Hkv, ctx->cache_stride, ctx->head_stride, ctx->attn,
                                      apk ? ctx->xp : nullptr, st));
        if (!apk) VVCHK(vv_pack_rows_launch(ctx->attn, Hq * D, nullptr, 0.f, ctx->xp, R, Hq * D, st));
        VVCHK(vv_gemm3_launch(L.wo, nullptr, ctx->xp, ctx->h, nullptr, nullptr, R, H, Hq * D, H, VV_EPI_RESID, &ctx->gws, st));
        VVCHK(vv_pack_rows_launch(ctx->h, H, L.ln2, c.lm_eps, ctx->xp, R, H, st));
        VVCHK(vv_gemm3_launch(L.wg, L.wu, ctx->xp, nullptr, ctx->actp, nullptr, R, I, H, 0, VV_EPI_SWIGLU, &ctx->gws, st));
        VVCHK(vv_gemm3_launch(L.wd, nullptr, ctx->actp, ctx->h, nullptr, nullptr, R, H, I, H, VV_EPI_RESID, &ctx->gws, st));
    }
    return lm_finish(ctx, st, R, hidden_out, final_norm);
}

static int lm_decode_attn(vv_ctx* ctx, hipStream_t st, int R, int l, const VVLmPlan& p, void* out_packed) {
    const vv_config& c = ctx->c;
    const int D = ctx->D, Hq = ctx->Hq, Hkv = ctx->Hkv;
    char *kl = lm_kc(ctx, l), *vl = lm_vc(ctx, l);
    const int attn_S = p.attn_S;
    ctx->launches += (attn_S > 1) ? 2 : 1;
    if (ctx->prof_on) {
        const double by = (double)p.kv_positions * Hkv * D * 2.0 * 2.0 + (double)R * (ctx->QKV + Hq * D) * 4.0;
        const int xs = c.xsplit; vv_ctx* cx = ctx;
        ctx->prof_other.push_back({2, by, [=](hipStream_t s) {
            return vv_attn_fused_launch(D, xs, cx->qkv, cx->rows_dev, cx->rope_tab, kl, vl, R, Hq, Hkv, cx->cache_stride,
                                        cx->head_stride, attn_S, cx->pm, cx->pl, cx->po, cx->attn, out_packed, s); }});
    }
    VVCHK(vv_attn_fused_launch(D, c.xsplit, ctx->qkv, ctx->rows_dev, ctx->rope_tab, kl, vl, R, Hq, Hkv, ctx->cache_stride,
                               ctx->head_stride, attn_S, ctx->pm, ctx->pl, ctx->po, ctx->attn, out_packed, st));
    return 0;
}

static int lm_p16_layer(vv_ctx* ctx, hipStream_t st, int R, int l, int l0, int l1, const VVLmPlan& p) {
    const vv_config& c = ctx->c;
    const int H = ctx->H, Hq = ctx->Hq, D = ctx->D, I = ctx->I, QKV = ctx->QKV;
    auto& L = ctx->layers[l];
    if (l > l0) {
        ctx->launches += 1;
        VVGemv16p a = p16_args(L.wqkv, nullptr, ctx->p16_x, ctx->qkv, nullptr, R, QKV, H, QKV);
        a.bias = L.bqkv; a.ssq_in = ctx->ssq_b; a.ssq_tiles = H / 16; a.eps = c.lm_eps;
        VVCHK(p16_go(ctx, st, a, VV_EPI_BIAS, 1));
    } else {
        ctx->launches += 2;
        VVCHK(vv_pack16_launch(ctx->h, H, 1, L.ln1, c.lm_eps, nullptr, nullptr, 0, ctx->p16_x, R, H, st));
        VVCHK(p16_gemv(ctx, st, L.wqkv, nullptr, ctx->p16_x, ctx->qkv, nullptr, L.bqkv, nullptr, R, QKV, H, QKV, 0, VV_EPI_BIAS));
    }
    VVTRY(lm_decode_attn(ctx, st, R, l, p, ctx->p16_y));
    ctx->launches += 3;
    VVGemv16p ao = p16_args(L.wo, nullptr, ctx->p16_y, ctx->h, ctx->p16_x, R, H, Hq * D, H);
    ao.pk_nw = L.ln2; ao.ssq_out = ctx->ssq_a;
    VVCHK(p16_go(ctx, st, ao, VV_EPI_RESID, 4));
    VVGemv16p ag = p16_args(L.wg, L.wu, ctx->p16_x, nullptr, ctx->p16_act, R, I, H, 0);
    ag.ssq_in = ctx->ssq_a; ag.ssq_tiles = H / 16; ag.eps = c.lm_eps;
    VVCHK(p16_go(ctx, st, ag, VV_EPI_SWIGLU, 1));
    VVGemv16p ad = p16_args(L.wd, nullptr, ctx->p16_act, ctx->h, nullptr, R, H, I, H);
    if (l + 1 < l1) {
        ad.Yp = (unsigned char*)ctx->p16_x; ad.pk_nw = ctx->layers[l + 1].ln1; ad.ssq_out = ctx->ssq_b;
        VVCHK(p16_go(ctx, st, ad, VV_EPI_RESID, 4));
    } else VVCHK(p16_go(ctx, st, ad, VV_EPI_RESID, 0));
    return 0;
}

static int lm_gemv_layer(vv_ctx* ctx, hipStream_t st, int R, int l, int l1, const VVLmPlan& p, int& hp) {
    const vv_config& c = ctx->c;
    const int H = ctx->H, D = ctx->D, Hq = ctx->Hq, Hkv = ctx->Hkv, I = ctx->I, QKV = ctx->QKV;
    const int hps = ctx->c.max_rows * H;
    auto& L = ctx->layers[l];
    VVGemm g = mk_gemm(L.wqkv, ctx->h, ctx->qkv, R, QKV, H, H, QKV);
    g.pro = VV_PRO_RMS; g.nw = L.ln1; g.eps = c.lm_eps; g.epi = VV_EPI_BIAS; g.bias = L.bqkv; g.nt = 1;
    g.xa = ctx->h_parts; g.n_xa = hp; g.part_stride = hps;
    const auto w13 = [&](const VVGemm& a, const void* t) { return p.w13 && t && vv_gemv_w13_form(&a, c.xsplit) >= 0; };
    if (w13(g, L.tqkv)) g.w13 = L.tqkv;
    GEMM(g);
    if (p.attn == VV_ATTN_FUSED) {
        VVTRY(lm_decode_attn(ctx, st, R, l, p, nullptr));
    } else {
        char *kl = lm_kc(ctx, l), *vl = lm_vc(ctx, l);
        ctx->launches += 3;
        VVCHK(vv_rope_append_launch(D, ctx->qkv, ctx->rows_dev, ctx->inv_freq, ctx->qrot, kl, vl,
                                    R, Hq, Hkv, ctx->cache_stride, ctx->head_stride, st));
        if (p.attn == VV_ATTN_PREFILL4)
            VVCHK(vv_attn_prefill4_launch(D, ctx->qrot, ctx->rows_dev, kl, vl, R, Hq, Hkv, ctx->cache_stride, ctx->head_stride, ctx->attn, nullptr, st));
        else {
            for (int k = 0; k < p.attn_groups; ++k) {
                const int g0 = k * ctx->ws_rows, ng = std::min(ctx->ws_rows, R - g0);
                if (g0) ctx->launches += 2;
                VVCHK(vv_attn_launch(D, c.xsplit, ctx->qrot + (size_t)g0 * Hq * D, ctx->rows_dev + g0, kl, vl, ng, Hq, Hkv, ctx->cache_stride,
                                     ctx->head_stride, p.attn_S, ctx->pm, ctx->pl, ctx->po, ctx->attn + (size_t)g0 * Hq * D, st));
            }
        }
    }
    VVGemm go = mk_gemm(L.wo, ctx->attn, ctx->h, R, H, Hq * D, Hq * D, H);
    go.epi = VV_EPI_RESID; go.nt = 1;
    go.ya = ctx->h_parts; go.n_ya = hp; go.part_stride = hps;
    GEMM(go);
    hp = 0;
    VVGemm gm = mk_gemm(L.wg, ctx->h, ctx->act, R, I, H, H, I);
    gm.W2 = (const u32x4*)L.wu; gm.pro = VV_PRO_RMS; gm.nw = L.ln2; gm.eps = c.lm_eps; gm.epi = VV_EPI_SWIGLU; gm.nt = 1;
    if (L.tu && w13(gm, L.tg)) { gm.w13 = L.tg; gm.w13_2 = L.tu; }
    GEMM(gm);
    VVGemm gd = mk_gemm(L.wd, ctx->act, ctx->h, R, H, I, I, H);
    gd.epi = VV_EPI_RESID; gd.nt = 1;
    if (l + 1 < l1) hp = ksplit_parts(ctx, gd, ctx->h_parts, hps);
    if (w13(gd, L.td)) gd.w13 = L.td;
    GEMM(gd);
    return 0;
}

static int lm_body(vv_ctx* ctx, hipStream_t st, int R, const float* x_in, float* hidden_out, int l0, int l1, int final_norm, const VVLmPlan& p) {
    VVCHK(vv_copy_launch(ctx->h, x_in, (size_t)R * ctx->H * 4, st));
    if (p.zero_v_tail) VVTRY(lm_zero_v_tail(ctx, st, R, l0, l1));
    if (p.route == VV_LM_PREFILL) return lm_prefill_layers(ctx, st, R, hidden_out, l0, l1, final_norm);
    int hp = 0;
    for (int l = l0; l < l1; ++l)
        VVTRY(p.route == VV_LM_P16 ? lm_p16_layer(ctx, st, R, l, l0, l1, p) : lm_gemv_layer(ctx, st, R, l, l1, p, hp));
    return lm_finish(ctx, st, R, hidden_out, final_norm);
}

int ksplit_check(vv_ctx* ctx, hipStream_t st) {
    if (!(ctx->gws.err && *ctx->gws.err)) return 0;
    {
        VV_SHARED;
        hipStreamSynchronize(st);
        if (ctx->gws.flags) { hipMemsetAsync(ctx->gws.flags, 0, 256 * sizeof(unsigned), st); hipStreamSynchronize(st); }
    }
    *ctx->gws.err = 0u;
    return fail(ctx, "prefill GEMM: a K-split hand-off timed out (lost producer workgroup); the prompt pass that was in flight is invalid -- "
                     "the arrival words were re-armed, retry the pass (VVHIP_NO_KSPLIT=1 disables the split)");
}
extern "C" int vv_lm_forward(vv_ctx* ctx, void* stream, int n_rows, const vv_row* rows, const float* x_in_dev, float* hidden_out_dev) {
    return vv_lm_forward_range(ctx, stream, n_rows, rows, x_in_dev, hidden_out_dev, 0, ctx->c.lm_layers, 1);
}
extern "C" int vv_lm_forward_range(vv_ctx* ctx, void* stream, int n_rows, const vv_row* rows, const float* x_in_dev,
                                   float* hidden_out_dev, int l0, int l1, int final_norm) {
    hipStream_t st = (hipStream_t)stream;
    if (l0 < 0 || l1 > ctx->c.lm_layers || l0 >= l1) return fail(ctx, "layer range [%d,%d) invalid", l0, l1);
    if (n_rows < 1 || n_rows > ctx->c.max_rows) return fail(ctx, "n_rows %d out of range [1,%d]", n_rows, ctx->c.max_rows);
    if (ksplit_check(ctx, st)) return -1;
    (void)hipGetLastError();
    for (int i = 0; i < n_rows; ++i) {
        if (rows[i].cache < 0 || rows[i].cache >= 2 * ctx->c.n_slots) return fail(ctx, "row %d: cache id %d out of range", i, rows[i].cache);
        if (rows[i].pos < 0 || rows[i].pos >= ctx->c.max_ctx) return fail(ctx, "row %d: position %d exceeds max_ctx %d", i, rows[i].pos, ctx->c.max_ctx);
    }
    const int slot = ring_acquire(ctx);
    VVRow* pin = ctx->rows_pin + (size_t)slot * ctx->rows_cap;
    for (int i = 0; i < n_rows; ++i) { pin[i].cache = rows[i].cache; pin[i].pos = rows[i].pos; }
    HIPCHK(ctx, hipMemcpyAsync(ctx->rows_dev, pin, sizeof(VVRow) * n_rows, hipMemcpyHostToDevice, st));
    HIPCHK(ctx, hipEventRecord(ctx->ring_ev[slot], st));
    ctx->launches = 0;
    if (!ctx->rope_ready) {
        VVCHK(vv_rope_table_launch(ctx->inv_freq, ctx->rope_tab, ctx->c.max_ctx, ctx->D / 2, st));
        ctx->rope_ready = true;
    }
    VVLmPlan plan;
    if (vv_lm_pass_plan(pin, n_rows, {ctx->ws_rows, ctx->c.attn_splits, ctx->Hkv, ctx->tile3_ok, ctx->attn2_ok, ctx->p16_ok, ctx->w13_lm}, &plan))
        return fail(ctx, "a launch of %d rows must be consecutive positions of one cache (decode / ragged launches take <= %d rows)", n_rows, ctx->ws_rows);
    char key[160]; snprintf(key, 160, "lm:%d:%p:%p:%d:%d:%d:%d:%d", n_rows, (const void*)x_in_dev, (void*)hidden_out_dev, l0, l1, final_norm,
                            plan.key_mode, plan.key_split);
    return graphed(ctx, key, st, [&]() { return lm_body(ctx, st, n_rows, x_in_dev, hidden_out_dev, l0, l1, final_norm, plan); });
}

extern "C" int vv_kv_import_at(vv_ctx* ctx, void* stream, int cache, int layer, int pos0, int n_pos, const void* k_dev, const void* v_dev, int src_dtype) {
    VV_SHARED;
    hipStream_t st = (hipStream_t)stream;
    if (cache < 0 || cache >= 2 * ctx->c.n_slots) return fail(ctx, "cache id %d out of range", cache);
    if (layer < 0 || layer >= ctx->c.lm_layers) return fail(ctx, "layer %d out of range", layer);
    if (pos0 < 0 || n_pos < 0 || (int64_t)pos0 + n_pos > ctx->c.max_ctx) return fail(ctx, "positions [%d, %d) exceed max_ctx %d", pos0, pos0 + n_pos, ctx->c.max_ctx);
    if (n_pos == 0) return 0;
    const size_t off = ((size_t)cache * ctx->cache_stride + (size_t)layer * ctx->layer_stride) * 2;
    VVCHK(vv_kv_import_launch(k_dev, v_dev, src_dtype, (char*)ctx->kc + off, (char*)ctx->vc + off, n_pos, ctx->Hkv, ctx->D, ctx->head_stride, pos0, st));
    return 0;
}
extern "C" int vv_kv_move(vv_ctx* ctx, void* stream, int cache, int src_pos, int dst_pos) {
    VV_SHARED;
    hipStream_t st = (hipStream_t)stream;
    if (cache < 0 || cache >= 2 * ctx->c.n_slots) return fail(ctx, "cache id %d out of range", cache);
    if (src_pos < 0 || dst_pos < 0 || src_pos >= ctx->c.max_ctx || dst_pos >= ctx->c.max_ctx)
        return fail(ctx, "vv_kv_move: positions %d -> %d outside [0, %d)", src_pos, dst_pos, ctx->c.max_ctx);
    if (src_pos == dst_pos) return 0;
    const size_t off = (size_t)cache * ctx->cache_stride * 2;
    ctx->launches++;
    VVCHK(vv_kv_move_launch((char*)ctx->kc + off, (char*)ctx->vc + off, ctx->c.lm_layers, ctx->Hkv, ctx->D, ctx->layer_stride, ctx->head_stride,
                            src_pos, dst_pos, st));
    return 0;
}
extern "C" int vv_kv_import(vv_ctx* ctx, void* stream, int cache, int layer, int n_pos, const void* k_dev, const void* v_dev, int src_dtype) {
    return vv_kv_import_at(ctx, stream, cache, layer, 0, n_pos, k_dev, v_dev, src_dtype);
}
extern "C" int vv_kv_export(vv_ctx* ctx, void* stream, int cache, int layer, int pos0, int n_pos, void* k_out_dev, void* v_out_dev, int dst_dtype) {
    VV_SHARED;
    hipStream_t st = (hipStream_t)stream;
    if (cache < 0 || cache >= 2 * ctx->c.n_slots) return fail(ctx, "cache id %d out of range", cache);
    if (layer < 0 || layer >= ctx->c.lm_layers) return fail(ctx, "layer %d out of range", layer);
    if (pos0 < 0 || n_pos < 0 || (int64_t)pos0 + n_pos > ctx->c.max_ctx)
        return fail(ctx, "vv_kv_export: positions [%d, %lld) exceed max_ctx %d", pos0, (long long)pos0 + n_pos, ctx->c.max_ctx);
    if (dst_dtype != 0 && dst_dtype != 1) return fail(ctx, "vv_kv_export: dst_dtype %d (0 = fp32, 1 = bf16)", dst_dtype);
    if (n_pos == 0) return 0;
    if (!k_out_dev || !v_out_dev) return fail(ctx, "vv_kv_export: null output");
    if (((uintptr_t)k_out_dev | (uintptr_t)v_out_dev) & 15) return fail(ctx, "vv_kv_export: outputs must be 16-byte aligned");
    const size_t off = ((size_t)cache * ctx->cache_stride + (size_t)layer * ctx->layer_stride) * 2;
    VVCHK(vv_kv_export_launch((char*)ctx->kc + off, (char*)ctx->vc + off, k_out_dev, v_out_dev, dst_dtype, n_pos, ctx->Hkv, ctx->D, ctx->head_stride, pos0, st));
    return 0;
}
extern "C" int64_t vv_kv_snapshot_bytes(vv_ctx* ctx, int n_pos) {
    if (n_pos < 0 || n_pos > ctx->c.max_ctx) return fail(ctx, "vv_kv_snapshot_bytes: %d positions outside [0, max_ctx %d]", n_pos, ctx->c.max_ctx);
    return (int64_t)ctx->c.lm_layers * ctx->Hkv * ((n_pos + 31) & ~31) * ctx->D * 2;
}
static int kv_span_copy(vv_ctx* ctx, void* stream, const char* who, int cache, int n_pos, void* k_dev, void* v_dev, int to_cache) {
    VV_SHARED;
    hipStream_t st = (hipStream_t)stream;
    if (cache < 0 || cache >= 2 * ctx->c.n_slots) return fail(ctx, "%s: cache id %d out of range", who, cache);
    if (n_pos < 0 || n_pos > ctx->c.max_ctx) return fail(ctx, "%s: %d positions outside [0, max_ctx %d]", who, n_pos, ctx->c.max_ctx);
    if (n_pos == 0) return 0;
    if (!k_dev || !v_dev) return fail(ctx, "%s: null snapshot buffer", who);
    if (((uintptr_t)k_dev | (uintptr_t)v_dev) & 15) return fail(ctx, "%s: snapshot buffers must be 16-byte aligned", who);
    const size_t off = (size_t)cache * ctx->cache_stride * 2;
    VVCHK(vv_kv_span_copy_launch((char*)ctx->kc + off, (char*)ctx->vc + off, k_dev, v_dev, to_cache, ctx->c.lm_layers, ctx->Hkv, ctx->D,
                                 ctx->layer_stride, ctx->head_stride, n_pos, st));
    return 0;
}
extern "C" int vv_kv_snapshot(vv_ctx* ctx, void* stream, int cache, int n_pos, void* k_out_dev, void* v_out_dev) {
    return kv_span_copy(ctx, stream, "vv_kv_snapshot", cache, n_pos, k_out_dev, v_out_dev, 0);
}
extern "C" int vv_kv_restore(vv_ctx* ctx, void* stream, int cache, int n_pos, const void* k_dev, const void* v_dev) {
    return kv_span_copy(ctx, stream, "vv_kv_restore", cache, n_pos, (void*)k_dev, (void*)v_dev, 1);
}
extern "C" int vv_add_type_embedding(vv_ctx* ctx, void* stream, int n, const float* x_dev, int type, float* out_dev) {
    VV_SHARED;
    hipStream_t st = (hipStream_t)stream;
    if (!ctx->tts_types) return fail(ctx, "engine was not configured with tts_layers");
    if (type < 0 || type > 1) return fail(ctx, "type must be 0 (speech) or 1 (text)");
    VVCHK(vv_add_rows_launch(x_dev, ctx->tts_types + (size_t)type * ctx->H, out_dev, n, ctx->H, st));
    return 0;
}

extern "C" int vv_eos_logit(vv_ctx* ctx, void* stream, int n, const float* hidden_dev, float* out_dev) {
// ... 80 lines not shown
```

vibevoice_amd/csrc/engine_prof.hip:

```cpp
#include "engine_ctx.h"
#include "vv_w13.h"

static __global__ void vv_nan_probe_kernel(const float* __restrict__ p, int n, unsigned* __restrict__ rec) {
    unsigned cnt = 0, first = 0xffffffffu, mx = 0;
    for (int i = blockIdx.x * blockDim.x + threadIdx.x; i < n; i += gridDim.x * blockDim.x) {
        const float v = p[i];
        if (!(fabsf(v) <= 3.0e38f)) { cnt++; first = min(first, (unsigned)i); }
        else mx = max(mx, __float_as_uint(fabsf(v)));
    }
    if (cnt) { atomicAdd(rec, cnt); atomicMax(rec + 1, 0xffffffffu - first); }
    atomicMax(rec + 2, mx);
}
void nan_probe(vv_ctx* ctx, hipStream_t st, const char* name, const void* p, size_t n) {
    if (!ctx->probe_on || !p || n == 0) return;
    const int id = (int)ctx->probe_names.size();
    if (id >= PROBE_MAX) return;
    ctx->probe_names.push_back(name);
    if (id == 0) (void)vv_zero_launch(ctx->probe_rec, PROBE_MAX * 16, st);
    hipLaunchKernelGGL(vv_nan_probe_kernel, dim3(64), dim3(256), 0, st, (const float*)p, (int)n, ctx->probe_rec + 4 * id);
}
void nan_probe_report(vv_ctx* ctx, hipStream_t st, const char* what) {
    if (!ctx->probe_on) return;
    std::vector<unsigned> h(PROBE_MAX * 4);
    const hipError_t e1 = hipStreamSynchronize(st);
// ... 32 lines not shown
        for (size_t i = old; i < ctx->prof_ev.size(); ++i) hipEventCreate(&ctx->prof_ev[i]);
    }
    ctx->prof_stream = st;
    hipEventRecord(ctx->prof_ev[2 * ctx->prof_n], st);
    int r = vv_gemm_launch(g, ctx->c.xsplit, st);
    hipEventRecord(ctx->prof_ev[2 * ctx->prof_n + 1], st);
    ctx->prof_n++;
    ctx->prof_bytes += gemm_bytes(g);
    const bool is_gemv = vv_gemm_route(&g, ctx->c.xsplit) == VV_ROUTE_GEMV;
    ctx->prof_rec.push_back({g.T, g.N, g.K, g.pro, g.epi, g.W2 ? 1 : 0, gemm_bytes(g), is_gemv});
    if (is_gemv) { ctx->prof_gemv.push_back(g); ctx->prof_gemv_bytes += gemm_bytes(g); }
    return r;
}
#ifdef VV_GEMM_TIMING
constexpr int TL_MAX = 4096, TL_STRIDE = 16 + 2 * 3200;
int gemm_tl(vv_ctx* ctx, VVGemm g, hipStream_t st) {
    if (!ctx->tl_base && getenv("VVHIP_TIMELINE")) {
        if (hipMalloc(&ctx->tl_base, (size_t)TL_MAX * TL_STRIDE * 8) != hipSuccess) return -9;
        hipMemset(ctx->tl_base, 0, (size_t)TL_MAX * TL_STRIDE * 8);
    }
    const bool gv = vv_gemm_route(&g, ctx->c.xsplit) == VV_ROUTE_GEMV;
    const bool want = gv ? ((g.T <= 4 || g.T != 16 || g.N > 16384) && (g.N + 15) / 16 <= 3200) : (g.T > 16);
    if (ctx->tl_base && ctx->tl_idx < TL_MAX && want) {
        g.dbg = ctx->tl_base + (size_t)ctx->tl_idx * TL_STRIDE;
        ctx->tl_rec.push_back({g.T, g.N, g.K, g.pro, gv ? g.epi : g.epi + 100});
        ctx->tl_idx++;
    }
    return vv_gemm_launch(g, ctx->c.xsplit, st);
}
extern "C" int vv_timeline_dump(vv_ctx* ctx, unsigned long long* out_host, int* meta_host, int max_launches) {
    VV_SHARED;
    hipDeviceSynchronize();
    const int n = std::min(max_launches, ctx->tl_idx);
    if (n > 0) hipMemcpy(out_host, ctx->tl_base, (size_t)n * TL_STRIDE * 8, hipMemcpyDeviceToHost);
    for (int i = 0; i < n; ++i) { const auto& r = ctx->tl_rec[i]; int* m = meta_host + 5 * i; m[0] = r.T; m[1] = r.N; m[2] = r.K; m[3] = r.pro; m[4] = r.epi; }
    return n;
}
#endif

extern "C" int vv_gemm_raw(void* stream, const void* w, const void* w2, const float* x, float* y, int T, int N, int K,
                           int ldx, int ldy, int pro, int epi, const float* nw, float eps, const float* bias,
                           const float* nscale, int xsplit, int ksplit, int nontemporal) {
    VVGemm g = mk_gemm(w, x, y, T, N, K, ldx, ldy);
    g.W2 = (const u32x4*)w2; g.pro = pro; g.epi = epi; g.nw = nw; g.eps = eps; g.bias = bias; g.nscale = nscale;
    g.ksplit = ksplit & 0xff; g.nt = 1;
    g.dbg = (unsigned long long*)(uintptr_t)0;
    if (nontemporal > 1) g.dbg = reinterpret_cast<unsigned long long*>(const_cast<float*>(nscale));
    if (g.dbg) g.nscale = nullptr;
    return vv_gemm_launch(g, xsplit, (hipStream_t)stream);
}
static VVGemm case_gemm(const vv_gemv_case_args* c) {
    VVGemm g = mk_gemm(c->W, c->X, c->Y, c->T, c->N, c->K, c->ldx, c->ldy);
    g.W2 = (const u32x4*)c->W2; g.pro = c->pro; g.epi = c->epi; g.nw = c->nw; g.eps = c->eps; g.bias = c->bias; g.nscale = c->nscale;
    g.mod_scale = c->mod_scale; g.mod_shift = c->mod_shift; g.ld_mod = c->ld_mod;
    g.addvec = c->addvec; g.x_row_mod = c->x_row_mod; g.add_rows_per_vec = c->add_rows_per_vec;
    g.gate = c->gate; g.ld_gate = c->ld_gate;
    g.z = c->z; g.x0p = c->x0p; g.coef = c->coef; g.cfg = c->cfg; g.n_cfg = c->n_cfg; g.sde_noise = c->sde_noise;
    g.cfg_rows = c->cfg_rows;
    g.kgrid = c->kgrid; g.yparts = c->yparts; g.xa = c->xa; g.n_xa = c->n_xa; g.ya = c->ya; g.n_ya = c->n_ya; g.part_stride = c->part_stride;
    g.sl_n = c->sl_n; g.sl_T = c->sl_T; g.sl_x = c->sl_x; g.sl_y = c->sl_y;
    for (int j = 0; j < 8; ++j) g.sl_id[j] = c->sl_id[j];
    g.dw_hist = c->dw_hist; g.dw_w = c->dw_w; g.dw_b = c->dw_b; g.dw_gamma = c->dw_gamma; g.dw_nw = c->dw_nw;
    g.dw_xout = c->dw_xout; g.dw_hnew = c->dw_hnew;
    g.nt = 1;
    return g;
}
extern "C" int vv_gemv_case(void* stream, const vv_gemv_case_args* c, int xsplit, int* form_out) {
    if (!c || xsplit < 1 || xsplit > 3) return -1;
    VVGemm g = case_gemm(c);
    if (!vv_gemv_ok(&g)) return VV_GEMV_REFUSED;
    int form[5] = {0, 0, 0, 0, 0};
    const int r = vv_gemv_launch(g, xsplit, (hipStream_t)stream, form);
    if (r == VV_RC_NO_FORM) return VV_GEMV_REFUSED;
    if (r == 0 && form_out) for (int j = 0; j < 5; ++j) form_out[j] = form[j];
    return r;
}
extern "C" int64_t vv_w13_twin_bytes(int N, int K) { return vv_w13_shape_ok(N, K) ? vv_w13_bytes(N, K) : 0; }
extern "C" int vv_w13_pack_matrix(void* stream, const void* packed_dev, void* twin_dev, int N, int K) {
    return vv_w13_pack_launch(packed_dev, twin_dev, N, K, (hipStream_t)stream);
}
extern "C" int vv_w13_unpack_matrix(void* stream, const void* twin_dev, void* packed_dev, int N, int K) {
    return vv_w13_unpack_launch(twin_dev, packed_dev, N, K, (hipStream_t)stream);
}
extern "C" int vv_w13_gemv_case(void* stream, const vv_gemv_case_args* c, const void* twin_dev, const void* twin2_dev, int mr, int wpb) {
    if (!c) return -1;
    VVGemm g = case_gemm(c);
    g.w13 = twin_dev; g.w13_2 = twin2_dev;
    const int r = vv_gemv_w13_form_launch(g, mr, wpb, (hipStream_t)stream);
    return r == VV_RC_NO_FORM ? VV_GEMV_REFUSED : r;
}
extern "C" int vv_gemm3_raw(vv_ctx* ctx, void* stream, const void* w, const void* w2, const float* x_dev, int T, int N, int K, int epi,
                            const float* nw_dev, float eps, const float* bias_dev, float* y_dev, void* xp_scratch, void* yp_scratch) {
    hipStream_t st = (hipStream_t)stream;
    if (ctx && ksplit_check(ctx, st)) return -1;
    int r = vv_pack_rows_launch(x_dev, K, nw_dev, eps, xp_scratch, T, K, st);
    if (r) return r;
    r = vv_gemm3_launch(w, w2, xp_scratch, y_dev, yp_scratch, bias_dev, T, N, K, N, epi, ctx ? &ctx->gws : nullptr, st);
    if (r) return r;
    if (epi == VV_EPI_SWIGLU) r = vv_unpack_rows_launch(yp_scratch, y_dev, T, N, st);
    return r;
}
extern "C" int vv_profile_begin(vv_ctx* ctx) {
    { VV_SHARED; HIPCHK(ctx, hipDeviceSynchronize()); }
    ctx->prof_on = true; ctx->prof_n = 0; ctx->prof_bytes = 0.0; ctx->prof_rec.clear();
    ctx->prof_gemv.clear(); ctx->prof_gemv_bytes = 0.0; ctx->prof_other.clear();
    return 0;
}
extern "C" int vv_profile_end(vv_ctx* ctx, int64_t* launches, double* total_ms, double* bytes) {
    { VV_SHARED; HIPCHK(ctx, hipDeviceSynchronize()); }
    double ms = 0.0, raw_ms = 0.0;
    int64_t n_other = 0; double ms_other = 0.0, by_other = 0.0;
    double ev_over = 0.0;
    {
        const int reps = 64;
        std::vector<hipEvent_t> ev(2 * reps);
        for (auto& e : ev) hipEventCreate(&e);
        hipStream_t ps = ctx->prof_stream;
        if (ctx->tmp1) vv_silu_launch(ctx->tmp1, 64, ps);
        for (int i = 0; i < reps; ++i) { hipEventRecord(ev[2 * i], ps); hipEventRecord(ev[2 * i + 1], ps); }
        hipStreamSynchronize(ps);
        std::vector<float> d(reps);
        for (int i = 0; i < reps; ++i) { d[i] = 0.f; hipEventElapsedTime(&d[i], ev[2 * i], ev[2 * i + 1]); }
        std::sort(d.begin(), d.end());
        ev_over = d[reps / 2];
        for (auto& e : ev) hipEventDestroy(e);
    }
    const char* csv = getenv("VVHIP_PROF_CSV");
    FILE* f = csv ? fopen(csv, "w") : nullptr;
    if (f) fprintf(f, "idx,T,N,K,pro,epi,dual,bytes,us\n");
    for (int i = 0; i < ctx->prof_n; ++i) {
        float e = 0.f;
        HIPCHK(ctx, hipEventElapsedTime(&e, ctx->prof_ev[2 * i], ctx->prof_ev[2 * i + 1]));
        if (ctx->prof_rec[i].gemv) raw_ms += e;
        e = (float)std::max(0.0, (double)e - ev_over);
        if (ctx->prof_rec[i].gemv) ms += e;
        else { n_other++; ms_other += e; by_other += ctx->prof_rec[i].bytes; }
        if (f) { const auto& r = ctx->prof_rec[i]; fprintf(f, "%d,%d,%d,%d,%d,%d,%d,%.0f,%.3f\n", i, r.T, r.N, r.K, r.pro, r.epi, r.dual, r.bytes, e * 1e3); }
    }
    if (f) fclose(f);
    if (launches) { launches[0] = ctx->prof_n - n_other; launches[1] = n_other; }
    if (total_ms) { total_ms[0] = ms; total_ms[1] = ms_other; }
    if (bytes) { bytes[0] = ctx->prof_bytes - by_other; bytes[1] = by_other; }
    ctx->prof_raw_ns = (int64_t)(raw_ms * 1e6); ctx->prof_ev_over_ns = (int64_t)(ev_over * 1e6);
    ctx->prof_on = false;
    return 0;
}
extern "C" int vv_profile_replay_family(vv_ctx* ctx, void* stream, int family, int reps, int64_t* launches, double* total_ms, double* bytes) {
    hipStream_t st = (hipStream_t)stream;
    if (ctx->prof_on) return fail(ctx, "vv_profile_replay: call vv_profile_end first");
    int64_t n = 0; double by = 0.0;
    if (family == 0) { n = (int64_t)ctx->prof_gemv.size(); by = ctx->prof_gemv_bytes; }
    else for (const auto& l : ctx->prof_other) if (l.family == family) { ++n; by += l.bytes; }
    if (launches) *launches = 0;
    if (total_ms) *total_ms = 0.0;
    if (bytes) *bytes = 0.0;
    if (n == 0) return family == 0 ? fail(ctx, "vv_profile_replay: the last profile window recorded no GEMV launches") : 0;
    if (reps < 1) reps = 1;
    HIPCHK(ctx, hipStreamSynchronize(st));
    hipGraph_t graph; hipGraphExec_t exec;
    HIPCHK(ctx, hipStreamBeginCapture(st, hipStreamCaptureModeRelaxed));
    int rr = 0;
    if (family == 0) { for (const VVGemm& g : ctx->prof_gemv) { rr = vv_gemm_launch(g, ctx->c.xsplit, st); if (rr) break; } }
    else for (const auto& l : ctx->prof_other) if (l.family == family) { rr = l.fn(st); if (rr) break; }
    hipError_t e = hipStreamEndCapture(st, &graph);
    if (rr) return fail(ctx, "vv_profile_replay: launch failed (%d)", rr);
    HIPCHK(ctx, e);
    HIPCHK(ctx, hipGraphInstantiate(&exec, graph, nullptr, nullptr, 0));
    hipGraphDestroy(graph);
    hipEvent_t e0, e1;
    hipEventCreate(&e0); hipEventCreate(&e1);
    HIPCHK(ctx, hipGraphLaunch(exec, st));
    HIPCHK(ctx, hipEventRecord(e0, st));
// ... 16 lines not shown
```

vibevoice_amd/csrc/gemv.hip:

```cpp
#include <array>
#include <utility>
#include "vv_common.h"
#include "vv_device.h"
#include "vv_launch.h"
#include "vv_w13.h"

#ifdef VV_GEMM_TIMING
#define VV_STAMP(i) do { if (a.dbg && blockIdx.x == 0 && threadIdx.x == 0) a.dbg[i] = __builtin_amdgcn_s_memtime(); } while (0)
#define VV_BSTAMP(i) do { if (a.dbg && threadIdx.x == 0 && blockIdx.y * gridDim.x + blockIdx.x < 3200) a.dbg[16 + 2 * (blockIdx.y * gridDim.x + blockIdx.x) + (i)] = __builtin_amdgcn_s_memrealtime(); } while (0)
#else
#define VV_BSTAMP(i) do { } while (0)
#define VV_STAMP(i) do { } while (0)
#endif

namespace {

constexpr int U = 8;


template <int XS, int PRO, int EPI, int MR, int WPB, int PARTS = 0, int SL = 0, int WF = 0>
__global__ __launch_bounds__(WPB * 64) void vv_gemv_kernel(const u32x4* __restrict__ pW, const u32x4* __restrict__ pW2,
                                                           const float* __restrict__ pX, float* __restrict__ pY,
                                                           const float* __restrict__ pnw, int pT, int pN, int pK, int pldx,
                                                           int pldy, const VVGemm a) {
    constexpr bool DUAL = (EPI == VV_EPI_SWIGLU);
    constexpr int NM = DUAL ? 2 : 1;
    constexpr bool FOLD = (PRO == VV_PRO_RMS_MOD) && MR <= 4;
    constexpr int NOP = (PRO == VV_PRO_RMS_MOD && !FOLD) ? 2 : 1;
    constexpr int MRS = FOLD ? 2 * MR : MR;
    static_assert(WF == 0 || (XS == 1 && NOP == 1 && MR <= 4 && PARTS == 0 && SL == 0), "W13 forms: bf16 mode, decode rows, one operand");
    constexpr int GSB = MRS * 16 + (MR == 16 ? 16 : 0);
    __shared__ __attribute__((aligned(16))) unsigned char stg_all[WPB * NOP * XS * U * 4 * GSB];
    __shared__ f32x4 red[WPB][NM * NOP][64];
    __shared__ float ssq_sh[WPB][MR];
    __shared__ float ssq1_sh[PRO == VV_PRO_NORMDW ? WPB : 1];
    asm volatile("" ::"s"(a.mod_scale), "s"(a.mod_shift), "s"(a.addvec), "s"(a.bias), "s"(a.nscale), "s"(a.gate));
    asm volatile("" ::"s"(a.ld_mod), "s"(a.ld_gate), "s"(a.x_row_mod), "s"(a.add_rows_per_vec),
                 "s"(a.eps), "s"(a.z), "s"(a.x0p), "s"(a.coef), "s"(a.cfg), "s"(a.n_cfg));
    asm volatile("" ::"s"(a.yparts), "s"(a.xa), "s"(a.ya), "s"(a.n_xa), "s"(a.n_ya), "s"(a.part_stride));
    if constexpr (EPI == VV_EPI_CFG_DPM) asm volatile("" ::"s"(a.sde_noise), "s"(a.cfg_rows));
    VV_STAMP(0);
    VV_BSTAMP(0);
    int lane = threadIdx.x & 63;
    const int wave = __builtin_amdgcn_readfirstlane((int)(threadIdx.x >> 6));
    const int t_base = (MR == 16) ? (int)blockIdx.y * 16 : 0;
    const int T = min(MR, pT - t_base);
    const unsigned tile = blockIdx.x;
    const unsigned k_tiles = (unsigned)(pK + 31) >> 5;
    const unsigned KSB = (MR <= 4) ? gridDim.y : 1u;
    const unsigned ksb = (MR <= 4) ? blockIdx.y : 0u;
    const unsigned kchunk = (k_tiles + KSB - 1) / KSB;
    const unsigned kb0 = min(k_tiles, ksb * kchunk), kb1 = min(k_tiles, kb0 + kchunk);
    const unsigned kper = (kb1 - kb0 + WPB - 1) / WPB;
    const unsigned kt0 = kb0 + wave * kper;
    const unsigned kt1 = min(kb1, kt0 + kper);
    const bool has_k = kt0 < kt1;
    int frow = lane & 15, fq = lane >> 4;
    unsigned char* stg = stg_all + (size_t)wave * (NOP * XS * U * 4 * GSB);
    unsigned kk = lane * 4;
    unsigned st_off = ((kk >> 5) * 4 + ((kk & 31) >> 3)) * GSB + (kk & 7) * 2;

    const u32x4* wbase = WF ? nullptr : pW + (size_t)tile * k_tiles * 64 + lane;
    const u32x4* wbase2 = DUAL && !WF ? pW2 + (size_t)tile * k_tiles * 64 + lane : nullptr;
    const unsigned char* gbase = reinterpret_cast<const unsigned char*>(pW) + (size_t)tile * (k_tiles >> 2) * VV_W13_GROUP;
    const unsigned char* gbase2 = reinterpret_cast<const unsigned char*>(pW2) + (size_t)tile * (k_tiles >> 2) * VV_W13_GROUP;
    constexpr int RG = WF ? (DUAL ? 2 : 3) : 1;
    const unsigned g_lo = kt0 >> 2, g_hi = (kt1 + 3) >> 2, ph = kt0 & 3;
    VVW13Raw raw[RG][NM];
    auto g_load = [&](unsigned g, VVW13Raw (&dst)[NM]) {
        g = min(g, g_hi - 1);
        dst[0] = vv_w13_load(gbase + g * VV_W13_GROUP, lane);
        if constexpr (DUAL) dst[1] = vv_w13_load(gbase2 + g * VV_W13_GROUP, lane);
    };

    unsigned xoff_sl[SL ? MR : 1];
    if constexpr (SL) {
#pragma unroll
        for (int r = 0; r < MR; ++r) {
            const int rg = t_base + r;
            const int j = rg / a.sl_T, tt = rg - j * a.sl_T;
            xoff_sl[r] = (r < T) ? (a.sl_x ? (unsigned)(vv_slot_id(a.sl_id, j) * a.sl_x + tt * pldx) : (unsigned)(rg * pldx)) : 0u;
        }
    }
    constexpr int MODR = (PRO == VV_PRO_RMS_MOD) ? MR : 1;
    constexpr int ADDR = (PRO == VV_PRO_ADD_SILU) ? MR : 1;
    constexpr int PR = (PARTS == 1) ? MR : 1;
    constexpr int DWH = (PRO == VV_PRO_NORMDW) ? 6 : 1, DWT = (PRO == VV_PRO_NORMDW) ? 7 : 1;
    struct XR { float4 x[MR]; float4 p0[PR]; float4 p1[PR]; float4 sc[MODR]; float4 sh[MODR]; float4 addv[ADDR]; float4 nwv;
                float4 dh[DWH]; float4 dt[DWT]; float4 db, dg, dn; };
    auto x_load = [&](unsigned ktb, XR& R) {
        unsigned k = ktb * 32 + kk;
        const bool kin = k < min(kt1 * 32, (unsigned)pK);
        if (!kin) k = 0;
        R.nwv = pnw ? *reinterpret_cast<const float4*>(pnw + k) : float4{1.f, 1.f, 1.f, 1.f};
        if constexpr (PRO == VV_PRO_NORMDW) {
#pragma unroll
            for (int j = 0; j < 6; ++j) R.dh[j] = *reinterpret_cast<const float4*>(a.dw_hist + (unsigned)(j * pK) + k);
#pragma unroll
            for (int j = 0; j < 7; ++j) R.dt[j] = *reinterpret_cast<const float4*>(a.dw_w + (unsigned)(j * pK) + k);
            R.db = *reinterpret_cast<const float4*>(a.dw_b + k);
            R.dg = *reinterpret_cast<const float4*>(a.dw_gamma + k);
            R.dn = *reinterpret_cast<const float4*>(a.dw_nw + k);
        }
#pragma unroll
        for (int r = 0; r < MR; ++r) {
            if (r < T) {
                const int rg = t_base + r;
                const int xr_idx = a.x_row_mod > 0 ? rg % a.x_row_mod : rg;
                if constexpr (SL) R.x[r] = *reinterpret_cast<const float4*>(pX + xoff_sl[r] + k);
                else R.x[r] = *reinterpret_cast<const float4*>(pX + (unsigned)(xr_idx * pldx) + k);
                if constexpr (PARTS == 1) {
                    R.p0[r] = *reinterpret_cast<const float4*>(a.xa + (unsigned)(xr_idx * pldx) + k);
                    R.p1[r] = *reinterpret_cast<const float4*>(a.xa + (unsigned)(a.part_stride + xr_idx * pldx) + k);
                }
                if constexpr (PRO == VV_PRO_ADD_SILU) {
                    const int av = a.add_rows_per_vec > 0 ? rg / a.add_rows_per_vec : 0;
                    R.addv[r] = *reinterpret_cast<const float4*>(a.addvec + (unsigned)(av * pK) + k);
                }
                if constexpr (PRO == VV_PRO_RMS_MOD) {
                    R.sc[r] = *reinterpret_cast<const float4*>(a.mod_scale + (unsigned)(rg * a.ld_mod) + k);
                    R.sh[r] = *reinterpret_cast<const float4*>(a.mod_shift + (unsigned)(rg * a.ld_mod) + k);
                }
            }
        }
    };
    auto w_load = [&](unsigned ktb, u32x4 (&dst)[U][NM]) {
#pragma unroll
        for (int u = 0; u < U; ++u) {
            const unsigned kt = min(ktb + u, kt1 - 1);
            dst[u][0] = __builtin_nontemporal_load(wbase + kt * 64);
            if constexpr (DUAL) dst[u][1] = __builtin_nontemporal_load(wbase2 + kt * 64);
        }
    };
    XR R;
    u32x4 wA[U][NM], wB[U][NM];
    if constexpr (WF) {
        if (has_k) {
            x_load(kt0, R);
#pragma unroll
            for (int q = 0; q < RG; ++q) g_load(g_lo + q, raw[q]);
        }
    } else
    if (has_k) { x_load(kt0, R); w_load(kt0, wA); }
    __builtin_amdgcn_sched_barrier(0);
    VV_STAMP(1);
    float rs1 = 1.0f;
    if constexpr (PRO == VV_PRO_NORMDW) {
        float s1 = 0.f;
        for (unsigned ktb = kt0; ktb < kt1; ktb += U) {
// ... 433 lines not shown
```

vibevoice_amd/csrc/gemv_plan.h:

```cpp
#pragma once
#include "vv_common.h"

struct VVGemvForm { int xs, mr, wpb, parts, sl; };
struct VVGemvPlan { VVGemvForm form; dim3 grid; };

struct VVGemvPair { int pro, epi; };
struct VVGemvFamily {
    int mr, wpb, parts, sl, xs_max, n;
    const VVGemvPair* pair;
    template <int N>
    constexpr VVGemvFamily(int mr_, int wpb_, int parts_, int sl_, int xs_max_, const VVGemvPair (&p)[N])
        : mr(mr_), wpb(wpb_), parts(parts_), sl(sl_), xs_max(xs_max_), n(N), pair(p) {}
    constexpr bool has(int pro, int epi) const {
        for (int i = 0; i < n; ++i) if (pair[i].pro == pro && pair[i].epi == epi) return true;
        return false;
    }
};
inline constexpr VVGemvPair vv_gemv_pairs[] = {
    {VV_PRO_NONE, VV_EPI_STORE}, {VV_PRO_NONE, VV_EPI_BIAS}, {VV_PRO_NONE, VV_EPI_RESID}, {VV_PRO_NONE, VV_EPI_GATED_RESID},
    {VV_PRO_RMS, VV_EPI_BIAS}, {VV_PRO_RMS, VV_EPI_BIAS_GELU}, {VV_PRO_RMS, VV_EPI_SWIGLU}, {VV_PRO_RMS, VV_EPI_RESID}, {VV_PRO_RMS, VV_EPI_STORE},
    {VV_PRO_RMS_MOD, VV_EPI_SWIGLU}, {VV_PRO_RMS_MOD, VV_EPI_CFG_DPM}, {VV_PRO_RMS_MOD, VV_EPI_STORE},
    {VV_PRO_ADD_SILU, VV_EPI_STORE}, {VV_PRO_NORMDW, VV_EPI_BIAS_GELU}};
inline constexpr VVGemvPair vv_gemv_pairs_w4[] = {
    {VV_PRO_RMS, VV_EPI_SWIGLU}, {VV_PRO_RMS_MOD, VV_EPI_SWIGLU}, {VV_PRO_RMS, VV_EPI_BIAS_GELU}, {VV_PRO_RMS, VV_EPI_BIAS},
// ... 21 lines not shown
    {2, 4, 0, 0, 1, vv_gemv_pairs_w4},
    {4, 4, 0, 0, 1, vv_gemv_pairs_w4},
    {4, 16, 0, 0, 1, vv_gemv_pairs_w16},
    {16, 8, 0, 0, 2, vv_gemv_pairs_wide},
    {16, 4, 0, 0, 1, vv_gemv_pairs_wide4},
    {16, 4, 0, 0, 1, vv_gemv_pairs_wide_mod},
    {4, 8, 1, 0, 3, vv_gemv_pairs_parts_x},
    {2, 4, 1, 0, 1, vv_gemv_pairs_parts_x_wide},
    {4, 4, 1, 0, 1, vv_gemv_pairs_parts_x_wide},
    {4, 8, 2, 0, 3, vv_gemv_pairs_parts_y},
    {16, 8, 0, 1, 2, vv_gemv_pairs_slots},
    {16, 4, 0, 1, 1, vv_gemv_pairs_slots}};

inline bool vv_gemv_eligible(const VVGemm* a) {
    const VVGemvFamily* const fam = vv_gemv_families;
    if (a->T < 1) return false;
    if (a->T > 4 || a->sl_n > 0) { if (!fam[VV_GF_WIDE].has(a->pro, a->epi) && !fam[VV_GF_WIDE_MOD].has(a->pro, a->epi)) return false; }
    else if (!fam[VV_GF_DEFAULT].has(a->pro, a->epi)) return false;
    if (a->sl_n > 0) {
        if (a->sl_n > 8 || a->sl_T < 1 || a->T != a->sl_n * a->sl_T || a->sl_x < 0 || a->sl_y < 0 || (a->sl_x & 3) || (a->sl_y & 3)) return false;
        if (a->kgrid > 1 || a->n_xa || a->n_ya || a->x_row_mod > 0 || a->add_rows_per_vec > 0) return false;
        if (!fam[VV_GF_SLOTS].has(a->pro, a->epi)) return false;
        for (int j = 0; j < a->sl_n; ++j)
            if (a->sl_id[j] < 0 || (int64_t)a->sl_id[j] * a->sl_x + (int64_t)a->sl_T * a->ldx >= (1LL << 30) ||
                (int64_t)a->sl_id[j] * a->sl_y + (int64_t)a->sl_T * a->ldy >= (1LL << 30)) return false;
    }
    if ((a->x_row_mod > 0 || a->add_rows_per_vec > 0) && a->pro != VV_PRO_ADD_SILU) return false;
    if (a->epi == VV_EPI_CFG_DPM && (a->n_cfg < 1 || a->T != 2 * a->n_cfg || a->T > 16 || !a->z || !a->x0p || !a->coef)) return false;
    if (a->pro == VV_PRO_NORMDW) {
        if (a->T != 1 || a->sl_n > 0 || a->kgrid > 1 || a->n_xa || a->n_ya || !a->dw_hist || !a->dw_w || !a->dw_b || !a->dw_gamma ||
            !a->dw_nw || !a->dw_xout || !a->dw_hnew || a->dw_xout == a->X) return false;
        if ((((uintptr_t)a->dw_hist) | ((uintptr_t)a->dw_w) | ((uintptr_t)a->dw_b) | ((uintptr_t)a->dw_gamma) | ((uintptr_t)a->dw_nw) |
             ((uintptr_t)a->dw_xout) | ((uintptr_t)a->dw_hnew)) & 15) return false;
        if ((int64_t)7 * a->K >= (1LL << 30)) return false;
    }
    if ((a->K & 3) || (a->ldx & 3) || (((uintptr_t)a->X) & 15)) return false;
    if (a->pro == VV_PRO_RMS_MOD && (a->ld_mod & 3)) return false;
    if (a->nw && (((uintptr_t)a->nw) & 15)) return false;
    if (a->K < 32) return false;
    if ((int64_t)a->T * a->ldy >= (1LL << 30) || (int64_t)a->T * a->ldx >= (1LL << 30)) return false;
    if ((a->N & 3) || (a->ldy & 3)) return false;
    if ((((uintptr_t)a->Y) & 15) || (a->bias && (((uintptr_t)a->bias) & 15))) return false;
    if (a->nscale && (((uintptr_t)a->nscale) & 15)) return false;
    if (a->epi == VV_EPI_GATED_RESID && ((a->ld_gate & 3) || (((uintptr_t)a->gate) & 15))) return false;
    if (a->pro == VV_PRO_RMS_MOD && ((((uintptr_t)a->mod_scale) & 15) || (((uintptr_t)a->mod_shift) & 15))) return false;
    if (a->pro == VV_PRO_ADD_SILU && (((uintptr_t)a->addvec) & 15)) return false;
    if (a->kgrid > 1 && (a->T > 4 || a->kgrid != 3 || a->pro != VV_PRO_NONE || !a->yparts || (a->part_stride & 3) ||
                         (a->epi != VV_EPI_RESID && a->epi != VV_EPI_GATED_RESID) || (((uintptr_t)a->yparts) & 15))) return false;
    if ((a->n_xa > 0 && (!a->xa || (((uintptr_t)a->xa) & 15))) || (a->n_ya > 0 && (!a->ya || (((uintptr_t)a->ya) & 15)))) return false;
    if ((a->n_xa != 0 && a->n_xa != 2) || (a->n_ya != 0 && a->n_ya != 2) || (a->n_xa && a->n_ya)) return false;
    if ((a->n_xa || a->n_ya) && ((a->part_stride & 3) || a->T > 4 || !fam[a->n_xa > 0 ? VV_GF_PARTS_X : VV_GF_PARTS_Y].has(a->pro, a->epi))) return false;
    return true;
}

constexpr int VV_GEMV_WIDE_TILES = 256;
constexpr int VV_GEMV_W16_MAX_TILES = 128, VV_GEMV_W16_MIN_KTILES = 96;
constexpr int VV_GEMV_WIDE4_WGS = 128;

inline bool vv_gemv_plan(const VVGemm* a, int xs, VVGemvPlan* out) {
    if (!vv_gemv_eligible(a)) return false;
    const VVGemvFamily* const fam = vv_gemv_families;
    const int n_tiles = (a->N + 15) / 16, k_tiles = (a->K + 31) / 32;
    const bool rows16 = a->T > 4 || a->sl_n > 0;
    const int grid_y = rows16 ? (a->T + 15) / 16 : a->kgrid > 1 ? a->kgrid : 1;
    const auto fits = [&](int f) { return xs >= 1 && xs <= fam[f].xs_max && fam[f].has(a->pro, a->epi); };
    const bool wide = n_tiles > VV_GEMV_WIDE_TILES, wide4 = (int64_t)n_tiles * grid_y > VV_GEMV_WIDE4_WGS;
    int f = VV_GF_DEFAULT;
    if (a->sl_n > 0) f = wide4 && fits(VV_GF_SLOTS4) ? VV_GF_SLOTS4 : VV_GF_SLOTS;
    else if (rows16 && wide4 && fits(VV_GF_WIDE4)) f = VV_GF_WIDE4;
    else if (rows16) f = fits(VV_GF_WIDE) ? VV_GF_WIDE : VV_GF_WIDE_MOD;
    else if (a->n_xa > 0 && wide && a->T <= 2 && fits(VV_GF_PARTS_X_ROWS2_W4)) f = VV_GF_PARTS_X_ROWS2_W4;
    else if (a->n_xa > 0) f = wide && fits(VV_GF_PARTS_X_W4) ? VV_GF_PARTS_X_W4 : VV_GF_PARTS_X;
    else if (a->n_ya > 0) f = VV_GF_PARTS_Y;
    else if (a->kgrid > 1) f = VV_GF_DEFAULT;
    else if (wide && a->T <= 2 && fits(VV_GF_ROWS2_W4)) f = VV_GF_ROWS2_W4;
    else if (wide && fits(VV_GF_ROWS4_W4)) f = VV_GF_ROWS4_W4;
    else if (n_tiles <= VV_GEMV_W16_MAX_TILES && k_tiles >= VV_GEMV_W16_MIN_KTILES && fits(VV_GF_W16)) f = VV_GF_W16;
    if (!fits(f)) return false;
    out->form = {xs, fam[f].mr, fam[f].wpb, fam[f].parts, fam[f].sl};
    out->grid = dim3(n_tiles, grid_y);
    return true;
}

struct VVGemvW13Form { int pro, epi, mr, wpb; };
inline constexpr VVGemvW13Form vv_gemv_w13_forms[] = {
    {VV_PRO_RMS_MOD, VV_EPI_SWIGLU, 2, 4}, {VV_PRO_RMS_MOD, VV_EPI_SWIGLU, 4, 8}, {VV_PRO_NONE, VV_EPI_GATED_RESID, 4, 8},
    {VV_PRO_RMS, VV_EPI_BIAS, 2, 4}, {VV_PRO_RMS, VV_EPI_SWIGLU, 2, 4}, {VV_PRO_NONE, VV_EPI_RESID, 4, 8}};
constexpr int VV_GEMV_W13_FORMS = sizeof(vv_gemv_w13_forms) / sizeof(vv_gemv_w13_forms[0]);
inline int vv_gemv_w13_find(int pro, int epi, int mr, int wpb) {
    for (int i = 0; i < VV_GEMV_W13_FORMS; ++i) {
        const VVGemvW13Form& f = vv_gemv_w13_forms[i];
        if (f.pro == pro && f.epi == epi && f.mr == mr && f.wpb == wpb) return i;
    }
    return -1;
}
inline bool vv_gemv_w13_shape(const VVGemm* a, int xs) {
    return xs == 1 && (a->K & 127) == 0 && (a->N & 15) == 0 && a->T <= 4 && a->kgrid <= 1 && a->n_xa == 0 && a->n_ya == 0 && a->sl_n == 0;
}
inline int vv_gemv_w13_form(const VVGemm* a, int xs) {
    VVGemvPlan p;
    if (!vv_gemv_w13_shape(a, xs) || !vv_gemv_plan(a, xs, &p) || p.form.parts || p.form.sl) return -1;
    return vv_gemv_w13_find(a->pro, a->epi, p.form.mr, p.form.wpb);
}

constexpr int VV_TILE_BM = 64;
#define VV_TILE_COMBOS(X)                                                                      \
    X(VV_PRO_NONE, VV_EPI_STORE) X(VV_PRO_NONE, VV_EPI_BIAS) X(VV_PRO_NONE, VV_EPI_RESID)      \
    X(VV_PRO_RMS, VV_EPI_BIAS) X(VV_PRO_RMS, VV_EPI_BIAS_GELU) X(VV_PRO_RMS, VV_EPI_SWIGLU)    \
    X(VV_PRO_RMS, VV_EPI_STORE)

inline bool vv_tile_eligible(const VVGemm* a, int xs) {
    if (a->T < 32 || xs > 2) return false;
    {
        const int per_wg = 4 * (a->epi == VV_EPI_SWIGLU ? 1 : 2);
        const int64_t wgs = (int64_t)(((a->N + 15) / 16 + per_wg - 1) / per_wg) * ((a->T + VV_TILE_BM - 1) / VV_TILE_BM);
        const int min_wgs = a->sl_n > 0 ? 40 : 48;
        if (wgs < min_wgs) return false;
    }
    if (a->sl_n > 0) {
        if (a->sl_n > 8 || a->sl_T < 1 || a->T != a->sl_n * a->sl_T || a->sl_x < 0 || a->sl_y < 0 || (a->sl_x & 3) || (a->sl_y & 3)) return false;
    }
    if ((a->K & 3) || (a->ldx & 3) || (a->N & 3) || (a->ldy & 3)) return false;
    if ((((uintptr_t)a->X) | ((uintptr_t)a->Y)) & 15) return false;
    if ((a->nw && (((uintptr_t)a->nw) & 15)) || (a->bias && (((uintptr_t)a->bias) & 15)) || (a->nscale && (((uintptr_t)a->nscale) & 15))) return false;
    if (a->x_row_mod > 0 || a->add_rows_per_vec > 0 || a->kgrid > 1 || a->n_xa > 0 || a->n_ya > 0 || a->ksplit > 0) return false;
    if (a->K < 32) return false;
    if (a->epi == VV_EPI_SWIGLU && !a->W2) return false;
#define X(P, E) if (a->pro == P && a->epi == E) return true;
    VV_TILE_COMBOS(X)
#undef X
    return false;
}

enum { VV_ROUTE_TILE, VV_ROUTE_GEMV, VV_ROUTE_GENERAL, VV_ROUTE_NONE };
inline int vv_gemm_route(const VVGemm* a, int xs) {
    VVGemvPlan p;
    if (vv_tile_eligible(a, xs)) return VV_ROUTE_TILE;
    if (a->sl_n > 0) return xs <= 2 && vv_gemv_plan(a, xs, &p) ? VV_ROUTE_GEMV : VV_ROUTE_NONE;
    if (a->ksplit <= 0 && vv_gemv_plan(a, xs, &p)) return VV_ROUTE_GEMV;
    if (a->kgrid > 1 || a->n_xa > 0 || a->n_ya > 0) return VV_ROUTE_NONE;
    return VV_ROUTE_GENERAL;
}

struct VVGemmGeneralPlan {
    bool vec, dual;
    int wpb, maxr, nt;
    int ks, t_pad;
    dim3 grid;
    size_t lds;
};
constexpr int VV_GG_NT2_TILE_PAIRS = 4096;
constexpr int VV_GG_WAVES = 2048, VV_GG_MIN_KSTEPS = 8;
constexpr int VV_GG_FEW_TILES = 512;
inline int vv_pow2_floor(int v) { int p = 1; while (p * 2 <= v) p *= 2; return p; }

inline int vv_gemm_general_plan(const VVGemm* a, int xs, VVGemmGeneralPlan* p) {
    const int n_tiles = (a->N + 15) / 16, k_tiles = (a->K + 31) / 32, t_tiles = (a->T + 15) / 16;
    p->dual = a->epi == VV_EPI_SWIGLU;
    if (p->dual && !a->W2) return -1;
    p->vec = ((a->K & 3) == 0) && ((a->ldx & 3) == 0) && ((((uintptr_t)a->X) & 15) == 0) && (a->pro != VV_PRO_RMS_MOD || (a->ld_mod & 3) == 0);
    if (!p->vec && p->dual) return VV_RC_NO_FORM;
    p->t_pad = a->T < 16 ? a->T : 16;
    p->wpb = (p->t_pad <= 4 && p->vec) ? 8 : 4;
    p->maxr = p->wpb == 8 ? 4 : 16;
    p->nt = (!p->dual && p->vec && (long)n_tiles * t_tiles >= VV_GG_NT2_TILE_PAIRS) ? 2 : 1;
    const long work = ((long)n_tiles + p->nt - 1) / p->nt * t_tiles;
    int ks = 1;
    if (a->ksplit > 0) ks = a->ksplit;
    else {
        const int want = (int)((VV_GG_WAVES + work - 1) / work);
        ks = vv_pow2_floor(want < 1 ? 1 : want);
// ... 14 lines not shown
```

vibevoice_amd/csrc/vv_launch.h:

```cpp
#pragma once
#include "vv_common.h"
#include "gemv_plan.h"

struct VVSolverStep {
    const float* eps;
    const float* z_in; const float* m1_in; const float* m2_in;
    float* z_out; float* m1_out; float* m2_out;
    const float* coef;
    float cfg; const float* cfg_rows;
    const float* noise;
    int n, L;
    const u32x4* Win;
    float* Xout;
    int H, xs;
};
extern "C" {
int vv_gemm_launch(VVGemm a, int xs, hipStream_t s);
int vv_pack_launch(const void* src, int src_is_bf16, void* dst, int N, int K, int kind, int Cin, int Cout, int ksz, int stride, hipStream_t s);
int vv_rope_append_launch(int D, const float* qkv, const VVRow* rows, const float* inv_freq, float* q_out, void* kc, void* vc, int R, int Hq, int Hkv,
                          int64_t cache_stride, int64_t head_stride, hipStream_t s);
int vv_rope_table_launch(const float* inv_freq, void* tab, int n_pos, int half, hipStream_t s);
int vv_attn_fused_launch(int D, int xs, const float* qkv, const VVRow* rows, const void* rope_tab, void* kc, void* vc, int R, int Hq, int Hkv,
                         int64_t cache_stride, int64_t head_stride, int S, float* pm, float* pl, float* po, float* out, void* out_packed,
                         hipStream_t s);
int vv_attn_launch(int D, int xs, const float* q, const VVRow* rows, const void* kc, const void* vc, int R, int Hq, int Hkv, int64_t cache_stride,
                   int64_t head_stride, int S, float* pm, float* pl, float* po, float* out, hipStream_t s);
int vv_embed_launch(const void* table, const int* ids, float* out, int n, int H, hipStream_t s);
int vv_logits_full_launch(const void* table, const float* hidden, float* out, int n, int V, int H, hipStream_t s);
int vv_warp_valid_launch(const float* logits, const unsigned char* seen, float* out, int* survivors, int n, int V, const int* ids, int n_valid,
                         float pen, float temp, int do_sample, int top_k, float top_p, float min_p, hipStream_t s);
int vv_noise_rows_launch(float* out, int n, const uint32_t* keys, uint32_t stream0, int n_streams, int n_t, int width, hipStream_t s);
int vv_rmsnorm_rows_launch(const float* x, int ldx, float* y, int ldy, const float* w, int T, int C, float eps, hipStream_t s);
int vv_dwconv_res_launch(const float* nb, const float* x, float* xo, const float* w, const float* b, const float* gamma, int T, int C, hipStream_t s);
int vv_normdw_sliced_ok(int T, int C);
int vv_normdw_sliced_slots_launch(const float* xin, float* xout, float* nb, const float* nw, const float* w, const float* b, const float* gamma,
                                  int T, int C, float eps, const int* ids, int n, int64_t sx, int64_t snb, hipStream_t s);
int vv_normdw_rows_slots_launch(const float* xin, float* xout, float* nb, const float* nw, const float* w, const float* b, const float* gamma, int T,
                                int C, float eps, const int* ids, int n, int64_t sx, int64_t snb, hipStream_t s);
int vv_stem_conv_slots_launch(const float* in, const void* wp, const float* bias, float* out, int T, int N, const int* ids, int n, int64_t s_in,
                              int64_t s_out, hipStream_t s);
int vv_head_conv1_slots_launch(const float* x, const void* wp, const float* bias, float* out, int T, int Cin, const int* ids, int n, int64_t s_in,
                               int64_t s_out, hipStream_t s);
int vv_block1d_slots_launch(int C, int xs, const float* xin, float* xout, float* nst, const float* norm_w, const float* ffn_norm_w,
                            const float* gamma, const float* ffn_gamma, const float* dw_w, const float* dw_b, const float* b1, const float* b2,
                            const void* w1, const void* w2, int T, float eps, const int* ids, int n, int64_t sx, int64_t snst, hipStream_t s);
int vv_affine_slots_launch(const float* x, float* y, float mul, float add, int L, const int* ids, int n, int64_t stride, hipStream_t s);
int vv_normdw_launch(float* x, float* nb, const float* nw, const float* w, const float* b, const float* gamma, int T, int C, float eps,
                     hipStream_t s);
int vv_normdw_rows_ok(int T, int C);
int vv_shift_rows_launch(const void* tab, int n_entries, int maxC, hipStream_t s);
int vv_zero_hist_launch(const void* tab, int n_entries, hipStream_t s);
int vv_affine_launch(const float* x, float* y, float mul, float add, int n, hipStream_t s);
int vv_copy_launch(void* dst, const void* src, size_t bytes, hipStream_t s);
int vv_zero_launch(void* dst, size_t bytes, hipStream_t s);
int vv_sampler_init_launch(const float* noise, float* z, float* x0p, int nL, hipStream_t s);
int vv_tfreq_launch(const float* t, float* out, int n, hipStream_t s);
int vv_silu_launch(float* x, int n, hipStream_t s);
int vv_ada_in_launch(const float* cproj, const float* temb, float* out, int rows, int n_steps, int H, hipStream_t s);
int vv_add_rows_launch(const float* x, const float* v, float* y, int n, int C, hipStream_t s);
int vv_relu_launch(float* x, int n, hipStream_t s);
int vv_kv_import_launch(const void* k, const void* v, int src_bf16, void* kc, void* vc, int L, int Hkv, int D, int64_t head_stride, int pos0,
                        hipStream_t s);
int vv_kv_move_launch(void* kc, void* vc, int layers, int Hkv, int D, int64_t layer_stride, int64_t head_stride, int src, int dst, hipStream_t s);
int vv_kv_zero_v_tail_launch(void* vc, const VVRow* rows, int R, int layers, int Hkv, int D, int64_t cache_stride, int64_t layer_stride,
                             int64_t head_stride, int max_ctx, hipStream_t s);
int vv_kv_span_copy_launch(void* kc, void* vc, void* ks, void* vs, int to_cache, int layers, int Hkv, int D, int64_t layer_stride,
                           int64_t head_stride, int n_pos, hipStream_t s);
int vv_kv_export_launch(const void* kc, const void* vc, void* k, void* v, int dst_bf16, int L, int Hkv, int D, int64_t head_stride, int pos0,
                        hipStream_t s);
int vv_pcm16_launch(const float* x, short* out, int n, int samples, hipStream_t s);
int vv_cvt_launch(const void* src, void* dst, int64_t n, int to_bf16, hipStream_t s);
int vv_dw_transpose_launch(const float* src, float* dst, int C, hipStream_t s);
int vv_pack_rows_launch(const float* x, int ldx, const float* nw, float eps, void* xp, int T, int K, hipStream_t s);
int vv_unpack_rows_launch(const void* xp, float* x, int T, int K, hipStream_t s);
int vv_pack16_launch(const float* x, int ldx, int mode, const float* nw, float eps, const float* sc, const float* sh, int ld_mod, void* xp, int T,
                     int K, hipStream_t s);
int vv_gemv16p_launch(const void* W, const void* W2, const void* Xp, float* Y, void* Yp, const float* bias, const float* gate, int T, int N, int K,
                      int ldy, int ld_gate, int epi, hipStream_t s);
int vv_gemv16p_launch2(const VVGemv16p* a, int epi, int flags, hipStream_t s);
int vv_head_tail_ok(const VVTail* a);
int vv_head_tail_init();
int vv_head_tail_launch(const VVTail* a, hipStream_t s);
int vv_solver_step_ok(const VVSolverStep* a);
int vv_solver_step_fused_ok(const VVSolverStep* a);
int vv_solver_step_launch(const VVSolverStep* a, hipStream_t s);
int vv_pack16_tiles_launch(const float* x, int ldx, int64_t stride_outer, int n_inner, int64_t stride_inner, void* xp, int64_t tile_bytes, int T,
                           int K, int n_tiles, hipStream_t s);
int vv_ada_pack_launch(const float* cproj, const float* temb, void* xp, int rows, int n_steps, int H, hipStream_t s);
int vv_gemm3_launch(const void* W, const void* W2, const void* Xp, float* Y, void* Yp, const float* bias, int T, int N, int K, int ldy, int epi,
                    const VVGemmWs* ws, hipStream_t s);
int vv_gemm_qkv_rope_launch(const void* W, const void* Xp, const float* bias, int T, int K, int D, int Hq, int Hkv, const VVRow* rows_dev,
                            const void* rope_tab, float* q_out, void* kc, void* vc, int64_t cache_stride, int64_t head_stride, const VVGemmWs* ws,
                            hipStream_t s);
int vv_attn_prefill4_launch(int D, const float* q, const VVRow* rows, const void* kc, const void* vc, int R, int Hq, int Hkv, int64_t cache_stride,
                            int64_t head_stride, float* out, void* out_packed, hipStream_t s);
int vv_block1d_supported(int C);
int vv_gemv_ok(const VVGemm* a);
int vv_gemv_launch(VVGemm a, int xs, hipStream_t s, int* form);
int vv_gemv_w13_form_launch(VVGemm a, int mr, int wpb, hipStream_t s);
int vv_w13_pack_launch(const void* packed, void* twin, int N, int K, hipStream_t s);
int vv_w13_pack_rows_launch(const void* packed, void* twin, int N, int K, int tile0, int tiles, hipStream_t s);
int vv_w13_unpack_launch(const void* twin, void* packed, int N, int K, hipStream_t s);
int vv_tile_ok(const VVGemm* a, int xs);
int vv_tile_launch(VVGemm a, int xs, hipStream_t s);
int vv_lora_merge_launch(const void* base, void* dst, int N, int K, const float* a, const float* b, int r, float scale, int delta_bf16,
                         hipStream_t s);
int vv_unpack_launch(const void* packed, float* dst, int N, int K, hipStream_t s);
int vv_resample_lds_bytes(int L, int T, int n_in);
int vv_resample_rows_launch(const VVRsRows* rows, int n, int L, int M, int T, const float* coef, float* hist, int n_streams, const float* x,
                            int ld_in, void* out, int ld_out, int pcm16, hipStream_t s);
int vv_resample_once_launch(int L, int M, int T, const float* coef, int n, int n_in, const float* x, int ld_in, float* out, int ld_out, hipStream_t s);
int vv_resample_reset_launch(float* hist, int T, int n_streams, const int* ids, int n, hipStream_t s);
int vv_tempo_rows_launch(const VVTpRows* rows, int n, const float* window, float* hist, int* dstate, int n_streams, const float* x, int ld_in,
                         void* out, int ld_out, int pcm16, int* offsets, int ld_off, hipStream_t s);
int vv_tempo_once_launch(const float* window, int P, int Q, int n, int n_in, const float* x, int ld_in, float* out, int ld_out, int* offsets,
                         int ld_off, hipStream_t s);
int vv_tempo_reset_launch(float* hist, int* dstate, int n_streams, const int* ids, int n, hipStream_t s);
int vv_level_rows_launch(const VVLvRows* rows, int n, int A, int H, float c, float* hist, int n_streams, const float* x, int ld_in, void* out,
                         int ld_out, int pcm16, hipStream_t s);
int vv_level_once_launch(int A, int H, float g, float c, int n, int n_in, const float* x, int ld_in, float* out, int ld_out, hipStream_t s);
int vv_level_reset_launch(float* hist, int nh, int n_streams, const int* ids, int n, hipStream_t s);
int vv_loud_rows_launch(const VVLdRows* rows, int n, const double* taps, int* hist, VVLdState* state, long long* part, int n_streams, const float* x,
                        int ld_in, float* out, int ld_out, hipStream_t s);
int vv_loud_energy_launch(const double* taps, int n, int n_in, const float* x, int ld_in, long long* E, int ld_e, long long* F, int ld_f, hipStream_t s);
int vv_loud_once_launch(const double* taps, float t, float g0, float wmax, int n, int n_in, const float* x, int ld_in, float* out, int ld_out,
                        float* gain, int ld_gain, long long* E, int ld_e, hipStream_t s);
int vv_loud_reset_launch(int* hist, VVLdState* state, int n_streams, const int* ids, int n, hipStream_t s);
}
```

vibevoice_amd/csrc/w13.hip:

```cpp
#include "vv_common.h"
#include "vv_w13.h"
#include "vv_launch.h"

namespace {

constexpr int PACK_WAVES = 4;

__global__ __launch_bounds__(PACK_WAVES * 64) void vv_w13_pack_kernel(const u32x4* __restrict__ W, unsigned char* __restrict__ out, int n_tiles, int k_tiles, int tile0) {
    __shared__ unsigned red[PACK_WAVES];
    const int lane = threadIdx.x & 63, wave = threadIdx.x >> 6;
    const unsigned tile = blockIdx.x + tile0;
    const int groups = k_tiles >> 2;
    const u32x4* src = W + (size_t)tile * k_tiles * 64;
    unsigned emax = 0;
    for (int i = threadIdx.x; i < k_tiles * 64; i += PACK_WAVES * 64) {
        const u32x4 v = src[i];
#pragma unroll
        for (int d = 0; d < 4; ++d) emax = max(emax, max((v[d] >> 7) & 0xffu, (v[d] >> 23) & 0xffu));
    }
#pragma unroll
    for (int o = 32; o > 0; o >>= 1) emax = max(emax, (unsigned)__shfl_xor((int)emax, o));
    if (lane == 0) red[wave] = emax;
    __syncthreads();
    emax = red[0];
#pragma unroll
    for (int w = 1; w < PACK_WAVES; ++w) emax = max(emax, red[w]);
    __syncthreads();
    const float scale = vv_w13_scale(emax);
    unsigned char* planes = out + (size_t)tile * groups * VV_W13_GROUP;
    unsigned ok = 1;
    for (int g = wave; g < groups; g += PACK_WAVES) {
        u32x4 f[4];
#pragma unroll
        for (int t = 0; t < 4; ++t) f[t] = src[(g * 4 + t) * 64 + lane];
        unsigned hi[8] = {0, 0, 0, 0, 0, 0, 0, 0}, lo[5] = {0, 0, 0, 0, 0};
#pragma unroll
        for (int j = 0; j < 16; ++j) {
            const unsigned pair = f[j >> 2][j & 3];
            unsigned x = 0;
#pragma unroll
            for (int h = 0; h < 2; ++h) {
                const unsigned b = (pair >> (16 * h)) & 0xffffu, s = b >> 15, E = (b >> 7) & 0xffu, m = b & 0x7fu;
                const bool zero = (b & 0x7fffu) == 0;
                const bool rep = zero || (E >= 1 && E + 29 >= emax && emax <= 254);
                const unsigned c = (rep && !zero) ? E + 30 - emax : 0u;
                const unsigned hb = (s << 7) | (c << 2) | ((rep && !zero) ? m >> 5 : 0u);
                const unsigned l5 = (rep && !zero) ? m & 31u : 0u;
                hi[j >> 1] |= hb << (8 * (2 * (j & 1) + h));
                x |= l5 << (5 * h);
            }
            const int d = (10 * j) >> 5, s10 = (10 * j) & 31;
            lo[d] |= x << s10;
            if (s10 + 10 > 32) lo[d + 1] |= x >> (32 - s10);
        }
        VVW13Raw r;
        r.h0 = u32x4{hi[0], hi[1], hi[2], hi[3]}; r.h1 = u32x4{hi[4], hi[5], hi[6], hi[7]};
        r.lo = u32x4{lo[0], lo[1], lo[2], lo[3]}; r.l4 = lo[4];
        vv_w13_store(planes + (size_t)g * VV_W13_GROUP, lane, r);
        u32x4 back[4];
        vv_w13_unpack(r, scale, back);
#pragma unroll
        for (int t = 0; t < 4; ++t)
#pragma unroll
            for (int d = 0; d < 4; ++d) if (back[t][d] != f[t][d]) ok = 0;
    }
    ok = __all((int)ok) ? 1u : 0u;
    if (lane == 0) red[wave] = ok;
    __syncthreads();
    if (threadIdx.x == 0) {
        unsigned all = 1;
#pragma unroll
        for (int w = 0; w < PACK_WAVES; ++w) all &= red[w];
        unsigned* tail = reinterpret_cast<unsigned*>(out + (size_t)n_tiles * groups * VV_W13_GROUP);
        tail[tile] = emax;
        tail[n_tiles + tile] = all;
    }
}

__global__ __launch_bounds__(256) void vv_w13_fold_kernel(unsigned* __restrict__ tail, int n_tiles) {
    __shared__ unsigned red[4];
    unsigned ok = 1;
    for (int i = threadIdx.x; i < n_tiles; i += 256) ok &= tail[n_tiles + i];
    ok = __all((int)ok) ? 1u : 0u;
    if ((threadIdx.x & 63) == 0) red[threadIdx.x >> 6] = ok;
    __syncthreads();
    if (threadIdx.x == 0) tail[2 * n_tiles] = red[0] & red[1] & red[2] & red[3];
}

__global__ __launch_bounds__(PACK_WAVES * 64) void vv_w13_unpack_kernel(const unsigned char* __restrict__ in, u32x4* __restrict__ W, int n_tiles, int k_tiles) {
    const int lane = threadIdx.x & 63, wave = threadIdx.x >> 6;
    const unsigned tile = blockIdx.x;
    const int groups = k_tiles >> 2;
    const unsigned* tail = reinterpret_cast<const unsigned*>(in + (size_t)n_tiles * groups * VV_W13_GROUP);
    const float scale = vv_w13_scale(tail[tile]);
    const unsigned char* planes = in + (size_t)tile * groups * VV_W13_GROUP;
    u32x4* dst = W + (size_t)tile * k_tiles * 64;
    for (int g = wave; g < groups; g += PACK_WAVES) {
        const VVW13Raw r = vv_w13_load(planes + (size_t)g * VV_W13_GROUP, lane);
        u32x4 f[4];
        vv_w13_unpack(r, scale, f);
#pragma unroll
        for (int t = 0; t < 4; ++t) dst[(g * 4 + t) * 64 + lane] = f[t];
    }
}

}

extern "C" int vv_w13_pack_rows_launch(const void* packed, void* twin, int N, int K, int tile0, int tiles, hipStream_t s) {
    if (!vv_w13_shape_ok(N, K) || tile0 < 0 || tiles < 1 || tile0 + tiles > N / 16) return VV_RC_NO_FORM;
    const int n_tiles = N / 16, k_tiles = K / 32;
    hipLaunchKernelGGL(vv_w13_pack_kernel, dim3(tiles), dim3(PACK_WAVES * 64), 0, s, (const u32x4*)packed, (unsigned char*)twin, n_tiles, k_tiles, tile0);
    hipLaunchKernelGGL(vv_w13_fold_kernel, dim3(1), dim3(256), 0, s, reinterpret_cast<unsigned*>((unsigned char*)twin + vv_w13_plane_bytes(N, K)), n_tiles);
    return vv_launch_rc(0);
}
extern "C" int vv_w13_pack_launch(const void* packed, void* twin, int N, int K, hipStream_t s) {
    return vv_w13_pack_rows_launch(packed, twin, N, K, 0, N / 16, s);
}
extern "C" int vv_w13_unpack_launch(const void* twin, void* packed, int N, int K, hipStream_t s) {
    if (!vv_w13_shape_ok(N, K)) return VV_RC_NO_FORM;
    const int n_tiles = N / 16, k_tiles = K / 32;
    hipLaunchKernelGGL(vv_w13_unpack_kernel, dim3(n_tiles), dim3(PACK_WAVES * 64), 0, s, (const unsigned char*)twin, (u32x4*)packed, n_tiles, k_tiles);
    return vv_launch_rc(0);
}
```

vibevoice_amd/engine.py:

```python
import ctypes as C
from dataclasses import dataclass, field
from typing import Dict, List, Optional, Sequence

import numpy as np
import torch

from . import _lib
from . import schedule as _schedule


@dataclass
class EngineConfig:
    lm_hidden: int
    lm_layers: int
    lm_heads: int
    lm_kv_heads: int
    lm_inter: int
    lm_vocab: int
    lm_head_dim: Optional[int] = None
    lm_eps: float = 1e-6
    rope_theta: float = 1e6
    head_layers: int = 4
    head_ffn_ratio: float = 3.0
    latent_dim: int = 64
# ... 668 lines not shown
            raise EngineError("vv_unpack_matrix failed: " + self._raw_err())
        return out

    def lora_merge_raw(self, base_packed: torch.Tensor, dst_packed: torch.Tensor, N: int, K: int, a: torch.Tensor, b: torch.Tensor,
                       scale: float, merge_dtype: str = "float32", unaligned_ok=()):
        what = "lora_merge_raw"
        self._shape_ints(what, N=N, K=K)
        flag = self._delta_flag(what, merge_dtype)
        if not isinstance(a, torch.Tensor) or not isinstance(b, torch.Tensor) or a.dim() != 2 or b.dim() != 2:
            raise ValueError(f"{what}: a and b are 2-D tensors")
        r = int(a.shape[0])
        if tuple(a.shape) != (r, K) or tuple(b.shape) != (N, r):
            raise ValueError(f"{what}: a {tuple(a.shape)} / b {tuple(b.shape)} do not factor an [{N}, {K}] matrix")
        nb = int(self.lib.vv_packed_bytes(N, K))
        self._dev_tensor(what, "base_packed", base_packed, nb, torch.uint8, "base_packed" in unaligned_ok)
        self._dev_tensor(what, "dst_packed", dst_packed, nb, torch.uint8, "dst_packed" in unaligned_ok)
        self._dev_tensor(what, "a", a, r * K, unaligned_ok="a" in unaligned_ok)
        self._dev_tensor(what, "b", b, N * r, unaligned_ok="b" in unaligned_ok)
        self._after_producer()
        if self.lib.vv_lora_merge_raw(self._s, self._p(base_packed), self._p(dst_packed), int(N), int(K), self._p(a), self._p(b), r,
                                      float(scale), flag) != 0:
            raise EngineError("vv_lora_merge_raw failed: " + self._raw_err())

    def weight_read(self, name: str, shape: Sequence[int]) -> torch.Tensor:
        nk = self._mat_shape(name)
        if nk is not None and tuple(int(v) for v in shape) != nk:
            raise ValueError(f"weight_read({name}): shape {tuple(shape)}, the parameter is {nk}")
        with torch.cuda.stream(self.stream):
            out = torch.empty(*[int(v) for v in shape], dtype=torch.float32, device=self.device)
        self._chk(self.lib.vv_weight_read(self._ctx, self._s, name.encode(), self._p(out)), f"vv_weight_read({name})")
        return out

    def lora_merge(self, name: str, a: torch.Tensor, b: torch.Tensor, scale: float, merge_dtype: str = "float32", unaligned_ok=()):
        what = f"lora_merge({name})"
        flag = self._delta_flag(what, merge_dtype)
        if not isinstance(a, torch.Tensor) or not isinstance(b, torch.Tensor) or a.dim() != 2 or b.dim() != 2 or a.shape[0] != b.shape[1]:
            raise ValueError(f"{what}: a [r, K] and b [N, r] are 2-D tensors with one r")
        r, K, N = int(a.shape[0]), int(a.shape[1]), int(b.shape[0])
        nk = self._mat_shape(name)
        if nk is not None and (N, K) != nk:
            raise ValueError(f"{what}: b @ a is [{N}, {K}], the parameter is {list(nk)}")
        self._dev_tensor(what, "a", a, r * K, unaligned_ok="a" in unaligned_ok)
        self._dev_tensor(what, "b", b, N * r, unaligned_ok="b" in unaligned_ok)
        self._after_producer()
        self._chk(self.lib.vv_lora_merge(self._ctx, self._s, name.encode(), self._p(a), self._p(b), r, float(scale), flag),
                  f"vv_lora_merge({name})")
        if name.startswith("head."):
            self._n_steps = None

    def lora_reset(self, name: Optional[str] = None):
        self._chk(self.lib.vv_lora_reset(self._ctx, self._s, name.encode() if name is not None else None), f"vv_lora_reset({name})")
        if name is None or name.startswith("head."):
            self._n_steps = None

    def gemm3_raw(self, wp, x, y, N, K, epi=0, w2p=None, nw=None, eps=1e-6, bias=None, ksplit=True):
        T = x.shape[0]
        xp = torch.zeros(int(self.lib.vv_packed_bytes(T, K)), dtype=torch.uint8, device=self.device)
        yp = torch.zeros(int(self.lib.vv_packed_bytes(T, N)), dtype=torch.uint8, device=self.device)
        torch.cuda.synchronize(self.device)
        rc = self.lib.vv_gemm3_raw(self._ctx if ksplit else None, self._s, self._p(wp), self._p(w2p), self._p(x), T, N, K, epi, self._p(nw), float(eps),
                                   self._p(bias), self._p(y), self._p(xp), self._p(yp))
        if rc != 0:
            raise EngineError(f"vv_gemm3_raw failed ({rc})")
        self.sync()

    def gemm_raw(self, wp, x, y, N, K, T=None, ldx=None, ldy=None, pro=0, epi=0, w2p=None, nw=None, eps=1e-6,
                 bias=None, nscale=None, xsplit=None, ksplit=0, nontemporal=0):
        T = x.shape[0] if T is None else T
        rc = self.lib.vv_gemm_raw(self._s, self._p(wp), self._p(w2p), self._p(x), self._p(y), T, N, K,
                                  ldx or K, ldy or N, pro, epi, self._p(nw), float(eps), self._p(bias),
                                  self._p(nscale), xsplit or self.cfg.xsplit, ksplit, nontemporal)
        if rc != 0:
            raise EngineError(f"vv_gemm_raw failed ({rc})")

    PRO_NONE, PRO_RMS, PRO_RMS_MOD, PRO_ADD_SILU, PRO_NORMDW = 0, 1, 2, 3, 4
    EPI_STORE, EPI_BIAS, EPI_BIAS_GELU, EPI_SWIGLU, EPI_RESID, EPI_GATED_RESID, EPI_CFG_DPM = 0, 1, 2, 3, 4, 5, 6

    def gemv_case(self, wp, x, y, T, N, K, *, ldx=None, ldy=None, pro=0, epi=0, w2p=None, nw=None, eps=1e-6, bias=None, nscale=None,
                  mod_scale=None, mod_shift=None, ld_mod=0, addvec=None, x_row_mod=0, add_rows_per_vec=0, gate=None, ld_gate=0,
                  z=None, x0p=None, coef=None, cfg=0.0, n_cfg=0, sde_noise=None, cfg_rows=None,
                  kgrid=0, yparts=None, xa=None, n_xa=0, ya=None, n_ya=0, part_stride=0,
                  sl_n=0, sl_T=0, sl_x=0, sl_y=0, sl_id=(),
                  dw_hist=None, dw_w=None, dw_b=None, dw_gamma=None, dw_nw=None, dw_xout=None, dw_hnew=None,
                  xsplit=None, unaligned_ok=(), w13_form=None, twin=None, twin2=None):
        ldx = K if ldx is None else ldx
        ldy = N if ldy is None else ldy
        xs = self.cfg.xsplit if xsplit is None else xsplit
        ints = dict(T=T, N=N, K=K, ldx=ldx, ldy=ldy, pro=pro, epi=epi, ld_mod=ld_mod, x_row_mod=x_row_mod, add_rows_per_vec=add_rows_per_vec,
                    ld_gate=ld_gate, n_cfg=n_cfg, kgrid=kgrid, n_xa=n_xa, n_ya=n_ya, part_stride=part_stride, sl_n=sl_n, sl_T=sl_T,
                    sl_x=sl_x, sl_y=sl_y, xsplit=xs)
        for k, v in ints.items():
            if not isinstance(v, (int, np.integer)) or isinstance(v, bool) or v < 0 or v >= (1 << 30):
                raise ValueError(f"gemv_case: {k} = {v!r} is not an int in [0, 2^30)")
        if T < 1 or N < 1 or K < 1:
            raise ValueError(f"gemv_case: T, N, K = {T}, {N}, {K} must be positive")
        if xs not in (1, 2, 3):
            raise ValueError(f"gemv_case: xsplit = {xs}")
        if not 0 <= pro <= 4 or not 0 <= epi <= 6:
            raise ValueError(f"gemv_case: pro = {pro}, epi = {epi}")
        if ldx < K or ldy < N:
            raise ValueError(f"gemv_case: ldx = {ldx} < K = {K} or ldy = {ldy} < N = {N}")
        sl_id = [int(v) for v in sl_id]
        if sl_n > 8 or len(sl_id) < sl_n or len(sl_id) > 8 or any(v < 0 or v >= (1 << 20) for v in sl_id):
            raise ValueError(f"gemv_case: sl_n = {sl_n}, sl_id = {sl_id}")
        if sl_n > 0 and (sl_T < 1 or T != sl_n * sl_T):
            raise ValueError(f"gemv_case: T = {T} is not sl_n * sl_T = {sl_n} * {sl_T}")
        if sl_n == 0 and (sl_T or sl_x or sl_y or sl_id):
            raise ValueError("gemv_case: slot fields without sl_n")

        def need(name, t, numel, dtype=torch.float32, required=True):
            if t is None:
                if required:
                    raise ValueError(f"gemv_case: {name} is required here")
                return
            if not isinstance(t, torch.Tensor) or t.device != self.device:
                raise ValueError(f"gemv_case: {name} is not a tensor on {self.device}")
            if t.dtype != dtype:
                raise ValueError(f"gemv_case: {name} is {t.dtype}, expected {dtype}")
            if not t.is_contiguous():
                raise ValueError(f"gemv_case: {name} is not contiguous")
            if t.data_ptr() % 16 and name not in unaligned_ok:
                raise ValueError(f"gemv_case: {name} is not 16-byte aligned")
            if t.numel() < numel:
                raise ValueError(f"gemv_case: {name} holds {t.numel()} elements, the launch addresses {numel}")

        def extent(rows, ld, width, slot_stride):
            if sl_n > 0 and slot_stride > 0:
                return max(sl_id[:sl_n]) * slot_stride + (sl_T - 1) * ld + width
            return (rows - 1) * ld + width
        x_rows = x_row_mod if x_row_mod > 0 else T
        x_need = extent(x_rows, ldx, K, sl_x)
        y_need = extent(T, ldy, N, sl_y)
        wbytes = int(self.lib.vv_packed_bytes(N, K))
        need("wp", wp, wbytes, torch.uint8)
        need("w2p", w2p, wbytes, torch.uint8, required=epi == self.EPI_SWIGLU)
        if w13_form is None and (twin is not None or twin2 is not None):
            raise ValueError("gemv_case: twins without w13_form")
        if twin is not None or twin2 is not None:
            tbytes = int(self.lib.vv_w13_twin_bytes(N, K))
            if tbytes == 0:
                raise ValueError(f"gemv_case: no W13 twin for N = {N}, K = {K}")
            need("twin", twin, tbytes, torch.uint8)
            need("twin2", twin2, tbytes, torch.uint8, required=epi == self.EPI_SWIGLU)
        need("x", x, x_need)
        need("y", y, y_need, required=epi != self.EPI_CFG_DPM)
        need("nw", nw, K, required=False)
        need("bias", bias, N, required=False)
        need("nscale", nscale, N, required=False)
        is_mod = pro == self.PRO_RMS_MOD
        if is_mod and ld_mod < K:
            raise ValueError(f"gemv_case: ld_mod = {ld_mod} < K = {K}")
        need("mod_scale", mod_scale, (T - 1) * ld_mod + K, required=is_mod)
        need("mod_shift", mod_shift, (T - 1) * ld_mod + K, required=is_mod)
        n_vec = (T - 1) // add_rows_per_vec + 1 if add_rows_per_vec > 0 else 1
        need("addvec", addvec, n_vec * K, required=pro == self.PRO_ADD_SILU)
        is_gated = epi == self.EPI_GATED_RESID
        if is_gated and ld_gate < N:
            raise ValueError(f"gemv_case: ld_gate = {ld_gate} < N = {N}")
        need("gate", gate, (T - 1) * ld_gate + N, required=is_gated)
        is_cfg = epi == self.EPI_CFG_DPM
        if is_cfg and n_cfg < 1:
            raise ValueError("gemv_case: the CFG epilogue needs n_cfg >= 1")
        need("z", z, 2 * n_cfg * N, required=is_cfg)
        need("x0p", x0p, n_cfg * N, required=is_cfg)
        need("coef", coef, 6, required=is_cfg)
        need("sde_noise", sde_noise, n_cfg * N, required=False)
        need("cfg_rows", cfg_rows, n_cfg, required=False)
        if (kgrid > 1 or n_xa or n_ya) and part_stride < max(x_need if n_xa else 0, y_need if (kgrid > 1 or n_ya) else 0):
            raise ValueError(f"gemv_case: part_stride = {part_stride} is smaller than one part tensor")
        need("yparts", yparts, (kgrid - 2) * part_stride + y_need if kgrid > 1 else 0, required=kgrid > 1)
        need("xa", xa, (max(n_xa, 2) - 1) * part_stride + x_need, required=n_xa > 0)
        need("ya", ya, (max(n_ya, 2) - 1) * part_stride + y_need, required=n_ya > 0)
        is_dw = pro == self.PRO_NORMDW
        for name, t, rows in (("dw_hist", dw_hist, 6), ("dw_w", dw_w, 7), ("dw_b", dw_b, 1), ("dw_gamma", dw_gamma, 1), ("dw_nw", dw_nw, 1),
                              ("dw_xout", dw_xout, 1), ("dw_hnew", dw_hnew, 1)):
            need(name, t, rows * K, required=is_dw)

        a = _lib.VVGemvCase()
        p = lambda t: t.data_ptr() if t is not None else None
        a.W, a.W2, a.X, a.Y = p(wp), p(w2p), p(x), p(y)
        a.T, a.N, a.K, a.ldx, a.ldy, a.pro, a.epi = T, N, K, ldx, ldy, pro, epi
        a.nw, a.eps, a.bias, a.nscale = p(nw), float(eps), p(bias), p(nscale)
        a.mod_scale, a.mod_shift, a.ld_mod = p(mod_scale), p(mod_shift), ld_mod
        a.addvec, a.x_row_mod, a.add_rows_per_vec = p(addvec), x_row_mod, add_rows_per_vec
        a.gate, a.ld_gate = p(gate), ld_gate
        a.z, a.x0p, a.coef, a.cfg, a.n_cfg, a.sde_noise = p(z), p(x0p), p(coef), float(cfg), n_cfg, p(sde_noise)
        a.kgrid, a.yparts, a.xa, a.n_xa, a.ya, a.n_ya, a.part_stride = kgrid, p(yparts), p(xa), n_xa, p(ya), n_ya, part_stride
        a.sl_n, a.sl_T, a.sl_x, a.sl_y = sl_n, sl_T, sl_x, sl_y
        for j, v in enumerate(sl_id):
            a.sl_id[j] = v
        a.dw_hist, a.dw_w, a.dw_b, a.dw_gamma, a.dw_nw = p(dw_hist), p(dw_w), p(dw_b), p(dw_gamma), p(dw_nw)
        a.dw_xout, a.dw_hnew = p(dw_xout), p(dw_hnew)
        a.cfg_rows = p(cfg_rows)
        if w13_form is not None:
            mr, wpb = (int(v) for v in w13_form)
            if xs != 1 or T > mr:
                raise ValueError(f"gemv_case: the W13 form ({mr}, {wpb}) takes xsplit 1 and T <= {mr}")
            rc = self.lib.vv_w13_gemv_case(self._s, C.byref(a), p(twin), p(twin2), mr, wpb)
            if rc == _lib.GEMV_REFUSED:
                return None
            if rc != 0:
                raise EngineError(f"vv_w13_gemv_case failed ({rc})")
            return (1, mr, wpb, 0, 0)
        form = (C.c_int * 5)()
        rc = self.lib.vv_gemv_case(self._s, C.byref(a), xs, form)
        if rc == _lib.GEMV_REFUSED:
            return None
        if rc != 0:
            raise EngineError(f"vv_gemv_case failed ({rc})")
        return tuple(form)


class TempoCapacityError(EngineError):
    """A Tempo.push row that brings more input, or emits more output, than one launch takes per row; nothing ran, no state changed:
    push it in pieces."""


class _RowStage:
    KIND = ROW = ROWS_FN = RESET_FN = None
    NO_ROWS = ()

    def __init__(self, engine: Engine, slot: int, n_streams: int):
        self.engine, self.slot, self.n_streams = engine, slot, int(n_streams)
        self.total = [0] * self.n_streams

    def take(self, ids: Sequence[int], remaining: Sequence[int], flush: bool = False) -> int:
        raise NotImplementedError

    def _args(self, audio, stream_ids, flush, n_in, **more):
        e, name = self.engine, type(self).__name__
        ids = [int(i) for i in stream_ids]
        n = len(ids)
        samples = 0 if audio is None else int(audio.shape[-1])
        if audio is not None:
            if audio.dim() != 2 or audio.dtype != torch.float32 or not audio.is_contiguous() or audio.device != e.device or audio.shape[0] < n:
                raise ValueError(f"{name}.push: audio is a contiguous fp32 [n >= {n}, samples] tensor on {e.device}")
        nin = [samples] * n if n_in is None else [int(v) for v in n_in]
        fl = [bool(flush)] * n if isinstance(flush, (bool, int)) else [bool(v) for v in flush]
        rest = [[v] * n if not hasattr(v, "__len__") else list(v) for v in more.values()]
        if any(len(v) != n for v in [nin, fl] + rest):
            names = ["n_in", "flush"] + list(more)
            raise ValueError(f"{name}.push: {', '.join(names[:-1])} and {names[-1]} name one value per row")
        return (ids, samples, nin, fl, *rest)

    def _out(self, out, n, nin, pcm16):
        e, dt = self.engine, torch.int16 if pcm16 else torch.float32
        if out is None:
            return torch.empty((max(n, 1), self.max_out(max(nin, default=0))), dtype=dt, device=e.device)
        if out.dim() != 2 or out.dtype != dt or not out.is_contiguous() or out.device != e.device or out.shape[0] < n:
            raise ValueError(f"{type(self).__name__}.push: out is a contiguous {dt} [n >= {n}, capacity] tensor on {e.device}")
        return out

    def _refused(self, rc):
        self.engine._chk(rc, self.ROWS_FN)

    def _launch(self, audio, samples, ids, nin, rows, out, pcm16, stream, extra=lambda i0: (), took=lambda i: None):
        e, n, cap = self.engine, len(ids), int(out.shape[1])
        st = e._sp(stream if stream is not None else torch.cuda.current_stream(e.device))
        cnts = (C.c_int * max(n, 1))()
        for i0 in range(0, n, 16) or self.NO_ROWS:
            nn = min(16, n - i0)
            a = C.c_void_p(audio.data_ptr() + i0 * samples * 4) if audio is not None else C.c_void_p()
            o = C.c_void_p(out.data_ptr() + i0 * cap * out.element_size())
            self._refused(getattr(e.lib, self.ROWS_FN)(e._ctx, st, self.slot, nn, C.cast(C.byref(rows, i0 * C.sizeof(self.ROW)), C.POINTER(self.ROW)),
                                                       a, samples, o, cap, int(pcm16), C.cast(C.byref(cnts, i0 * 4), C.POINTER(C.c_int)), *extra(i0)))
            for i in range(i0, i0 + nn):
                self.total[ids[i]] += nin[i]
                took(i)
        return [int(cnts[i]) for i in range(n)]

    def reset(self, ids: Optional[Sequence[int]] = None, stream=None):
        e = self.engine
        st = e._sp(stream if stream is not None else torch.cuda.current_stream(e.device))
        arr = None if ids is None else (C.c_int * max(1, len(ids)))(*[int(i) for i in ids])
        e._chk(getattr(e.lib, self.RESET_FN)(e._ctx, st, self.slot, 0 if ids is None else len(ids), arr), self.RESET_FN)
        for i in range(self.n_streams) if ids is None else ids:
            self._cleared(int(i))

    def _cleared(self, stream_id):
        self.total[stream_id] = 0

# ... 157 lines not shown
```

Measured before the change: 17.90.

## Resolve W13 twin exactness for LM layers and take exact fast path

Adds a shared w13_resolve that gathers every twin's exactness flag with one device kernel and one copy, replacing the per-twin synchronous memcpy the head path used before. It now also runs for the LM twins, so LM GEMVs get a w13_exact flag, presumably letting the kernel skip fallback/correction work when the twin is exact. Graphs are dropped when exactness changes. The cost is an extra resolve check per LM pass, plus a host sync whenever twins are stale.

Result: no change. 17.89 (-0.1%).

```diff
diff --git a/include/vvhip.h b/include/vvhip.h
--- a/include/vvhip.h
+++ b/include/vvhip.h
@@ -162,6 +162,7 @@
 int vv_w13_pack_matrix(void* stream, const void* packed_dev, void* twin_dev, int N, int K);
 int vv_w13_unpack_matrix(void* stream, const void* twin_dev, void* packed_dev, int N, int K);
 int vv_w13_gemv_case(void* stream, const vv_gemv_case_args* args, const void* twin_dev, const void* twin2_dev, int mr, int wpb);
+int vv_w13_gemv_case_exact(void* stream, const vv_gemv_case_args* args, const void* twin_dev, const void* twin2_dev, int mr, int wpb, int exact);
 int vv_gemm3_raw(vv_ctx* ctx, void* stream, const void* w_packed_dev, const void* w2_packed_dev, const float* x_dev, int T, int N, int K,
                  int epi, const float* nw_dev, float eps, const float* bias_dev, float* y_dev, void* xp_scratch, void* yp_scratch);
 int vv_profile_begin(vv_ctx* ctx);
diff --git a/vibevoice_amd/_lib.py b/vibevoice_amd/_lib.py
--- a/vibevoice_amd/_lib.py
+++ b/vibevoice_amd/_lib.py
@@ -141,6 +141,7 @@
     "vv_w13_pack_matrix": (C.c_int, [_P, _P, _P, C.c_int, C.c_int]),
     "vv_w13_unpack_matrix": (C.c_int, [_P, _P, _P, C.c_int, C.c_int]),
     "vv_w13_gemv_case": (C.c_int, [_P, C.POINTER(VVGemvCase), _P, _P, C.c_int, C.c_int]),
+    "vv_w13_gemv_case_exact": (C.c_int, [_P, C.POINTER(VVGemvCase), _P, _P, C.c_int, C.c_int, C.c_int]),
     "vv_gemm3_raw": (C.c_int, [_P, _P, _P, _P, _P, C.c_int, C.c_int, C.c_int, C.c_int, _P, C.c_float, _P, _P, _P, _P]),
     "vv_profile_begin": (C.c_int, [_P]),
     "vv_profile_end": (C.c_int, [_P, C.POINTER(C.c_int64), C.POINTER(C.c_double), C.POINTER(C.c_double)]),
diff --git a/vibevoice_amd/csrc/engine.hip b/vibevoice_amd/csrc/engine.hip
--- a/vibevoice_amd/csrc/engine.hip
+++ b/vibevoice_amd/csrc/engine.hip
@@ -115,6 +115,7 @@
                 HIPCHK(ctx, hipGraphInstantiate(&ge.exec, graph, nullptr, nullptr, 0));
                 hipGraphDestroy(graph);
                 captured = true;
+                ctx->captures++;
             } else {
                 (void)hipGetLastError();
                 ctx->capture_fallbacks++;
@@ -232,14 +233,15 @@
         add_mat(ctx, p + "self_attn.q_proj.weight", Hq * D, H, L.wqkv, 0);
         add_mat(ctx, p + "self_attn.k_proj.weight", Hkv * D, H, L.wqkv, Hq * D / 16);
         add_mat(ctx, p + "self_attn.v_proj.weight", Hkv * D, H, L.wqkv, (Hq + Hkv) * D / 16);
-        L.tqkv = twin(ctx->w13_lm, true, L.wqkv, QKV, H, 3);
+        const auto row = [&](const void* t) { return t ? (int)ctx->twins.size() - 1 : -1; };
+        L.tqkv = twin(ctx->w13_lm, true, L.wqkv, QKV, H, 3); L.xqkv = row(L.tqkv);
         add_vec(ctx, p + "self_attn.q_proj.bias", Hq * D, L.bqkv);
         add_vec(ctx, p + "self_attn.k_proj.bias", Hkv * D, L.bqkv + Hq * D);
         add_vec(ctx, p + "self_attn.v_proj.bias", Hkv * D, L.bqkv + (Hq + Hkv) * D);
-        L.wo = alloc_packed(ctx, H, Hq * D); add_mat(ctx, p + "self_attn.o_proj.weight", H, Hq * D, L.wo, 0); L.to = twin(ctx->w13_lm, true, L.wo, H, Hq * D);
-        L.wg = alloc_packed(ctx, I, H); add_mat(ctx, p + "mlp.gate_proj.weight", I, H, L.wg, 0); L.tg = twin(ctx->w13_lm, true, L.wg, I, H);
-        L.wu = alloc_packed(ctx, I, H); add_mat(ctx, p + "mlp.up_proj.weight", I, H, L.wu, 0); L.tu = twin(ctx->w13_lm, true, L.wu, I, H);
-        L.wd = alloc_packed(ctx, H, I); add_mat(ctx, p + "mlp.down_proj.weight", H, I, L.wd, 0); L.td = twin(ctx->w13_lm, true, L.wd, H, I);
+        L.wo = alloc_packed(ctx, H, Hq * D); add_mat(ctx, p + "self_attn.o_proj.weight", H, Hq * D, L.wo, 0); L.to = twin(ctx->w13_lm, true, L.wo, H, Hq * D); L.xo = row(L.to);
+        L.wg = alloc_packed(ctx, I, H); add_mat(ctx, p + "mlp.gate_proj.weight", I, H, L.wg, 0); L.tg = twin(ctx->w13_lm, true, L.wg, I, H); L.xg = row(L.tg);
+        L.wu = alloc_packed(ctx, I, H); add_mat(ctx, p + "mlp.up_proj.weight", I, H, L.wu, 0); L.tu = twin(ctx->w13_lm, true, L.wu, I, H); L.xu = row(L.tu);
+        L.wd = alloc_packed(ctx, H, I); add_mat(ctx, p + "mlp.down_proj.weight", H, I, L.wd, 0); L.td = twin(ctx->w13_lm, true, L.wd, H, I); L.xd = row(L.td);
     }
     const int n_caches = 2 * c.n_slots;
     ctx->head_stride = (int64_t)c.max_ctx * D;
@@ -360,6 +362,7 @@
             if (ctx->w[i].name == "lm_head.weight") ctx->w[i].dev = parent->w[i].dev;
         }
         ctx->lm_head = parent->lm_head; ctx->lm_head_loaded = parent->lm_head_loaded;
+        for (size_t i = 0; i < ctx->twins.size() && i < parent->twins.size(); ++i) ctx->twins[i].exact = parent->twins[i].exact;
         ctx->scaling = parent->scaling; ctx->bias = parent->bias;
         { std::lock_guard<std::mutex> fl(g_family_mu); parent->n_children++; }
     }
@@ -498,7 +501,44 @@
     const int tile0 = (int)(((const char*)w.dev - (const char*)t.src) / ((int64_t)(t.K / 32) * 1024));
     VVCHK(vv_w13_pack_rows_launch(t.src, t.planes, t.N, t.K, tile0, w.N / 16, st));
     t.exact = -1;
-    return 0;
+    ctx->w13_stale[t.lm] = true;
+    return 0;
+}
+
+int w13_resolve(vv_ctx* ctx, hipStream_t st, bool lm) {
+    if (!(lm ? ctx->w13_lm : ctx->w13_on) || !ctx->w13_stale[lm]) return 0;
+    const int n = (int)ctx->twins.size();
+    bool any = false;
+    for (const W13Twin& t : ctx->twins) any |= t.lm == lm && t.exact < 0;
+    if (any) {
+        if (!ctx->w13_ok_ptrs) {
+            std::vector<const unsigned*> ptrs(n);
+            for (int i = 0; i < n; ++i) {
+                const W13Twin& t = ctx->twins[i];
+                ptrs[i] = reinterpret_cast<const unsigned*>((const char*)t.planes + vv_w13_plane_bytes(t.N, t.K)) + 2 * (t.N / 16);
+            }
+            ctx->w13_ok_ptrs = (const unsigned**)dalloc(ctx, (size_t)n * sizeof(void*));
+            ctx->w13_ok_dev = (unsigned*)dalloc(ctx, (size_t)n * 4);
+            if (!ctx->w13_ok_ptrs || !ctx->w13_ok_dev) return -1;
+            HIPCHK(ctx, hipMemcpy((void*)ctx->w13_ok_ptrs, ptrs.data(), (size_t)n * sizeof(void*), hipMemcpyHostToDevice));
+            ctx->w13_ok_host.resize(n);
+        }
+        VVCHK(vv_w13_gather_ok_launch(ctx->w13_ok_ptrs, ctx->w13_ok_dev, n, st));
+        HIPCHK(ctx, hipStreamSynchronize(st));
+        HIPCHK(ctx, hipMemcpy(ctx->w13_ok_host.data(), ctx->w13_ok_dev, (size_t)n * 4, hipMemcpyDeviceToHost));
+    }
+    bool changed = false;
+    for (int i = 0; i < n; ++i) {
+        W13Twin& t = ctx->twins[i];
+        if (t.lm != lm) continue;
+        if (t.exact < 0) t.exact = ctx->w13_ok_host[i] == 1;
+        if (t.used >= 0 && t.used != t.exact) changed = true;
+        t.used = t.exact;
+    }
+    ctx->w13_stale[lm] = false;
+    if (!changed) return 0;
+    if (lm) return drop_graphs(ctx, {"lm:"});
+    return drop_graphs(ctx, {"samp:", "sde:", "rows:", "gen:"});
 }
 
 static bool w13_ok_words(const W13Twin& t, std::vector<unsigned>& ok, bool folded) {
@@ -603,6 +643,8 @@
             }
             return n;
         }
+        case 12: return ctx->lm_w13_fallback;
+        case 13: return ctx->captures;
         case 10: {
             int64_t n = 0;
             for (const W13Twin& t : ctx->twins) n += t.lm;
diff --git a/vibevoice_amd/csrc/engine_ctx.h b/vibevoice_amd/csrc/engine_ctx.h
--- a/vibevoice_amd/csrc/engine_ctx.h
+++ b/vibevoice_amd/csrc/engine_ctx.h
@@ -92,7 +92,7 @@
     std::vector<Weight> w;
     std::map<std::string, int> widx;
     int H, D, Hq, Hkv, I, QKV;
-    struct Layer { float *ln1, *ln2, *bqkv; void *wqkv, *wo, *wg, *wu, *wd; void *tqkv, *to, *tg, *tu, *td; };
+    struct Layer { float *ln1, *ln2, *bqkv; void *wqkv, *wo, *wg, *wu, *wd; void *tqkv, *to, *tg, *tu, *td; int xqkv = -1, xo = -1, xg = -1, xu = -1, xd = -1; };
     std::vector<Layer> layers;
     float *lm_norm = nullptr, *inv_freq = nullptr;
     int ws_rows = 0;
@@ -120,6 +120,10 @@
     struct HLayer { float* norm; void *wg, *wu, *wd; int ig, iu, id; };
     bool w13_on = false, w13_lm = false;
     std::vector<W13Twin> twins;
+    bool w13_stale[2] = {true, true};
+    const unsigned** w13_ok_ptrs = nullptr; unsigned* w13_ok_dev = nullptr; std::vector<unsigned> w13_ok_host;
+    int64_t lm_w13_fallback = 0;
+    int64_t captures = 0;
     std::vector<HLayer> hl;
     void *h_in = nullptr, *h_cond = nullptr, *h_t0 = nullptr, *h_t2 = nullptr, *h_ada = nullptr, *h_out = nullptr;
     int n_steps = 0;
@@ -221,6 +225,7 @@
 int gemm_prof(vv_ctx* ctx, const VVGemm& g, hipStream_t st);
 int lora_rebase(vv_ctx* ctx, int widx, hipStream_t st);
 int w13_repack(vv_ctx* ctx, int widx, hipStream_t st);
+int w13_resolve(vv_ctx* ctx, hipStream_t st, bool lm);
 
 #ifdef VV_GEMM_TIMING
 int gemm_tl(vv_ctx* ctx, VVGemm g, hipStream_t st);
diff --git a/vibevoice_amd/csrc/engine_head.hip b/vibevoice_amd/csrc/engine_head.hip
--- a/vibevoice_amd/csrc/engine_head.hip
+++ b/vibevoice_amd/csrc/engine_head.hip
@@ -273,24 +273,9 @@
     return 0;
 }
 
-static int head_w13_resolve(vv_ctx* ctx, hipStream_t st) {
-    if (!ctx->w13_on) return 0;
-    bool changed = false, waited = false;
-    for (W13Twin& t : ctx->twins) {
-        if (t.lm || t.exact >= 0) continue;
-        if (!waited) { HIPCHK(ctx, hipStreamSynchronize(st)); waited = true; }
-        unsigned ok = 0;
-        HIPCHK(ctx, hipMemcpy(&ok, (const char*)t.planes + vv_w13_plane_bytes(t.N, t.K) + (size_t)2 * (t.N / 16) * 4, 4, hipMemcpyDeviceToHost));
-        t.exact = ok == 1;
-        if (t.used >= 0 && t.used != t.exact) changed = true;
-        t.used = t.exact;
-    }
-    return changed ? drop_graphs(ctx, {"samp:", "sde:", "rows:", "gen:"}) : 0;
-}
-
 static int run_sampler(vv_ctx* ctx, hipStream_t st, const char* key, const SampleReq& r) {
     ctx->launches = 0;
-    { VV_SHARED; VVTRY(head_w13_resolve(ctx, st)); }
+    { VV_SHARED; VVTRY(w13_resolve(ctx, st, false)); }
     const int rc = graphed(ctx, key, st, [&]() { return sample_body(ctx, st, r); });
     nan_probe_report(ctx, st, key);
     return rc;
@@ -348,7 +333,7 @@
     if (n < 1 || n > 16) return fail(ctx, "vv_head_forward: n must be in [1,16]");
     const int H = ctx->H;
     for (int i = 1; i < n; ++i) if (t_host[i] != t_host[0]) return fail(ctx, "vv_head_forward: all rows must share one timestep");
-    VVTRY(head_w13_resolve(ctx, st));
+    VVTRY(w13_resolve(ctx, st, false));
     float* tdev = ctx->tmp2 + 63 * 256;
     HIPCHK(ctx, hipStreamSynchronize(st));
     HIPCHK(ctx, hipMemcpy(tdev + 128, t_host, 4, hipMemcpyHostToDevice));
diff --git a/vibevoice_amd/csrc/engine_lm.hip b/vibevoice_amd/csrc/engine_lm.hip
--- a/vibevoice_amd/csrc/engine_lm.hip
+++ b/vibevoice_amd/csrc/engine_lm.hip
@@ -128,7 +128,13 @@
     g.pro = VV_PRO_RMS; g.nw = L.ln1; g.eps = c.lm_eps; g.epi = VV_EPI_BIAS; g.bias = L.bqkv; g.nt = 1;
     g.xa = ctx->h_parts; g.n_xa = hp; g.part_stride = hps;
     const auto w13 = [&](const VVGemm& a, const void* t) { return p.w13 && t && vv_gemv_w13_form(&a, c.xsplit) >= 0; };
-    if (w13(g, L.tqkv)) g.w13 = L.tqkv;
+    const auto exact = [&](int row) { return row >= 0 && ctx->twins[row].exact == 1; };
+    const auto twinned = [&](VVGemm& a, const void* t, int row, const void* t2 = nullptr, int row2 = -1) {
+        a.w13 = t; a.w13_2 = t2;
+        a.w13_exact = exact(row) && (!t2 || exact(row2));
+        ctx->lm_w13_fallback += !a.w13_exact;
+    };
+    if (w13(g, L.tqkv)) twinned(g, L.tqkv, L.xqkv);
     GEMM(g);
     if (p.attn == VV_ATTN_FUSED) {
         VVTRY(lm_decode_attn(ctx, st, R, l, p, nullptr));
@@ -155,12 +161,12 @@
     hp = 0;
     VVGemm gm = mk_gemm(L.wg, ctx->h, ctx->act, R, I, H, H, I);
     gm.W2 = (const u32x4*)L.wu; gm.pro = VV_PRO_RMS; gm.nw = L.ln2; gm.eps = c.lm_eps; gm.epi = VV_EPI_SWIGLU; gm.nt = 1;
-    if (L.tu && w13(gm, L.tg)) { gm.w13 = L.tg; gm.w13_2 = L.tu; }
+    if (L.tu && w13(gm, L.tg)) twinned(gm, L.tg, L.xg, L.tu, L.xu);
     GEMM(gm);
     VVGemm gd = mk_gemm(L.wd, ctx->act, ctx->h, R, H, I, I, H);
     gd.epi = VV_EPI_RESID; gd.nt = 1;
     if (l + 1 < l1) hp = ksplit_parts(ctx, gd, ctx->h_parts, hps);
-    if (w13(gd, L.td)) gd.w13 = L.td;
+    if (w13(gd, L.td)) twinned(gd, L.td, L.xd);
     GEMM(gd);
     return 0;
 }
@@ -170,6 +176,7 @@
     if (p.zero_v_tail) VVTRY(lm_zero_v_tail(ctx, st, R, l0, l1));
     if (p.route == VV_LM_PREFILL) return lm_prefill_layers(ctx, st, R, hidden_out, l0, l1, final_norm);
     int hp = 0;
+    ctx->lm_w13_fallback = 0;
     for (int l = l0; l < l1; ++l)
         VVTRY(p.route == VV_LM_P16 ? lm_p16_layer(ctx, st, R, l, l0, l1, p) : lm_gemv_layer(ctx, st, R, l, l1, p, hp));
     return lm_finish(ctx, st, R, hidden_out, final_norm);
@@ -210,6 +217,7 @@
         VVCHK(vv_rope_table_launch(ctx->inv_freq, ctx->rope_tab, ctx->c.max_ctx, ctx->D / 2, st));
         ctx->rope_ready = true;
     }
+    if (ctx->w13_lm) { VV_SHARED; VVTRY(w13_resolve(ctx, st, true)); }
     VVLmPlan plan;
     if (vv_lm_pass_plan(pin, n_rows, {ctx->ws_rows, ctx->c.attn_splits, ctx->Hkv, ctx->tile3_ok, ctx->attn2_ok, ctx->p16_ok, ctx->w13_lm}, &plan))
         return fail(ctx, "a launch of %d rows must be consecutive positions of one cache (decode / ragged launches take <= %d rows)", n_rows, ctx->ws_rows);
diff --git a/vibevoice_amd/csrc/engine_prof.hip b/vibevoice_amd/csrc/engine_prof.hip
--- a/vibevoice_amd/csrc/engine_prof.hip
+++ b/vibevoice_amd/csrc/engine_prof.hip
@@ -138,12 +138,15 @@
 extern "C" int vv_w13_unpack_matrix(void* stream, const void* twin_dev, void* packed_dev, int N, int K) {
     return vv_w13_unpack_launch(twin_dev, packed_dev, N, K, (hipStream_t)stream);
 }
-extern "C" int vv_w13_gemv_case(void* stream, const vv_gemv_case_args* c, const void* twin_dev, const void* twin2_dev, int mr, int wpb) {
+extern "C" int vv_w13_gemv_case_exact(void* stream, const vv_gemv_case_args* c, const void* twin_dev, const void* twin2_dev, int mr, int wpb, int exact) {
     if (!c) return -1;
     VVGemm g = case_gemm(c);
-    g.w13 = twin_dev; g.w13_2 = twin2_dev;
+    g.w13 = twin_dev; g.w13_2 = twin2_dev; g.w13_exact = exact != 0;
     const int r = vv_gemv_w13_form_launch(g, mr, wpb, (hipStream_t)stream);
     return r == VV_RC_NO_FORM ? VV_GEMV_REFUSED : r;
+}
+extern "C" int vv_w13_gemv_case(void* stream, const vv_gemv_case_args* c, const void* twin_dev, const void* twin2_dev, int mr, int wpb) {
+    return vv_w13_gemv_case_exact(stream, c, twin_dev, twin2_dev, mr, wpb, 0);
 }
 extern "C" int vv_gemm3_raw(vv_ctx* ctx, void* stream, const void* w, const void* w2, const float* x_dev, int T, int N, int K, int epi,
                             const float* nw_dev, float eps, const float* bias_dev, float* y_dev, void* xp_scratch, void* yp_scratch) {
diff --git a/vibevoice_amd/csrc/gemv.hip b/vibevoice_amd/csrc/gemv.hip
--- a/vibevoice_amd/csrc/gemv.hip
+++ b/vibevoice_amd/csrc/gemv.hip
@@ -64,7 +64,8 @@
     const u32x4* wbase2 = DUAL && !WF ? pW2 + (size_t)tile * k_tiles * 64 + lane : nullptr;
     const unsigned char* gbase = reinterpret_cast<const unsigned char*>(pW) + (size_t)tile * (k_tiles >> 2) * VV_W13_GROUP;
     const unsigned char* gbase2 = reinterpret_cast<const unsigned char*>(pW2) + (size_t)tile * (k_tiles >> 2) * VV_W13_GROUP;
-    constexpr int RG = WF ? (DUAL ? 2 : 3) : 1;
+    constexpr int RG = WF ? vv_gemv_w13_slots(PRO, EPI, MR, WPB) : 1;
+    static_assert(!WF || RG == 2 || RG == 3, "a W13 instantiation is a form of vv_gemv_w13_forms; the weight loop below is written for 2 and 3 slots");
     const unsigned g_lo = kt0 >> 2, g_hi = (kt1 + 3) >> 2, ph = kt0 & 3;
     VVW13Raw raw[RG][NM];
     auto g_load = [&](unsigned g, VVW13Raw (&dst)[NM]) {
diff --git a/vibevoice_amd/csrc/gemv_plan.h b/vibevoice_amd/csrc/gemv_plan.h
--- a/vibevoice_amd/csrc/gemv_plan.h
+++ b/vibevoice_amd/csrc/gemv_plan.h
@@ -127,11 +127,19 @@
     return true;
 }
 
-struct VVGemvW13Form { int pro, epi, mr, wpb; };
+struct VVGemvW13Form { int pro, epi, mr, wpb, slots, wgs_per_cu; };
+constexpr int VV_GEMV_CUS = 256;
 inline constexpr VVGemvW13Form vv_gemv_w13_forms[] = {
-    {VV_PRO_RMS_MOD, VV_EPI_SWIGLU, 2, 4}, {VV_PRO_RMS_MOD, VV_EPI_SWIGLU, 4, 8}, {VV_PRO_NONE, VV_EPI_GATED_RESID, 4, 8},
-    {VV_PRO_RMS, VV_EPI_BIAS, 2, 4}, {VV_PRO_RMS, VV_EPI_SWIGLU, 2, 4}, {VV_PRO_NONE, VV_EPI_RESID, 4, 8}};
+    {VV_PRO_RMS_MOD, VV_EPI_SWIGLU, 2, 4, 2, 0}, {VV_PRO_RMS_MOD, VV_EPI_SWIGLU, 4, 8, 2, 1}, {VV_PRO_NONE, VV_EPI_GATED_RESID, 4, 8, 3, 0},
+    {VV_PRO_RMS, VV_EPI_BIAS, 2, 4, 3, 0}, {VV_PRO_RMS, VV_EPI_SWIGLU, 2, 4, 2, 0}, {VV_PRO_NONE, VV_EPI_RESID, 4, 8, 3, 0}};
 constexpr int VV_GEMV_W13_FORMS = sizeof(vv_gemv_w13_forms) / sizeof(vv_gemv_w13_forms[0]);
+constexpr int vv_gemv_w13_slots(int pro, int epi, int mr, int wpb) {
+    for (int i = 0; i < VV_GEMV_W13_FORMS; ++i) {
+        const VVGemvW13Form& f = vv_gemv_w13_forms[i];
+        if (f.pro == pro && f.epi == epi && f.mr == mr && f.wpb == wpb) return f.slots;
+    }
+    return 0;
+}
 inline int vv_gemv_w13_find(int pro, int epi, int mr, int wpb) {
     for (int i = 0; i < VV_GEMV_W13_FORMS; ++i) {
         const VVGemvW13Form& f = vv_gemv_w13_forms[i];
diff --git a/vibevoice_amd/csrc/vv_launch.h b/vibevoice_amd/csrc/vv_launch.h
--- a/vibevoice_amd/csrc/vv_launch.h
+++ b/vibevoice_amd/csrc/vv_launch.h
@@ -101,6 +101,7 @@
 int vv_w13_pack_launch(const void* packed, void* twin, int N, int K, hipStream_t s);
 int vv_w13_pack_rows_launch(const void* packed, void* twin, int N, int K, int tile0, int tiles, hipStream_t s);
 int vv_w13_unpack_launch(const void* twin, void* packed, int N, int K, hipStream_t s);
+int vv_w13_gather_ok_launch(const unsigned* const* ptrs, unsigned* out, int n, hipStream_t s);
 int vv_tile_ok(const VVGemm* a, int xs);
 int vv_tile_launch(VVGemm a, int xs, hipStream_t s);
 int vv_lora_merge_launch(const void* base, void* dst, int N, int K, const float* a, const float* b, int r, float scale, int delta_bf16,
diff --git a/vibevoice_amd/csrc/w13.hip b/vibevoice_amd/csrc/w13.hip
--- a/vibevoice_amd/csrc/w13.hip
+++ b/vibevoice_amd/csrc/w13.hip
@@ -87,6 +87,11 @@
     if (threadIdx.x == 0) tail[2 * n_tiles] = red[0] & red[1] & red[2] & red[3];
 }
 
+__global__ __launch_bounds__(256) void vv_w13_gather_ok_kernel(const unsigned* const* __restrict__ ptrs, unsigned* __restrict__ out, int n) {
+    const int i = blockIdx.x * 256 + threadIdx.x;
+    if (i < n) out[i] = *ptrs[i];
+}
+
 __global__ __launch_bounds__(PACK_WAVES * 64) void vv_w13_unpack_kernel(const unsigned char* __restrict__ in, u32x4* __restrict__ W, int n_tiles, int k_tiles) {
     const int lane = threadIdx.x & 63, wave = threadIdx.x >> 6;
     const unsigned tile = blockIdx.x;
@@ -116,6 +121,11 @@
 extern "C" int vv_w13_pack_launch(const void* packed, void* twin, int N, int K, hipStream_t s) {
     return vv_w13_pack_rows_launch(packed, twin, N, K, 0, N / 16, s);
 }
+extern "C" int vv_w13_gather_ok_launch(const unsigned* const* ptrs, unsigned* out, int n, hipStream_t s) {
+    if (n < 1) return 0;
+    hipLaunchKernelGGL(vv_w13_gather_ok_kernel, dim3((n + 255) / 256), dim3(256), 0, s, ptrs, out, n);
+    return vv_launch_rc(0);
+}
 extern "C" int vv_w13_unpack_launch(const void* twin, void* packed, int N, int K, hipStream_t s) {
     if (!vv_w13_shape_ok(N, K)) return VV_RC_NO_FORM;
     const int n_tiles = N / 16, k_tiles = K / 32;
diff --git a/vibevoice_amd/engine.py b/vibevoice_amd/engine.py
--- a/vibevoice_amd/engine.py
+++ b/vibevoice_amd/engine.py
@@ -774,7 +774,7 @@
                   kgrid=0, yparts=None, xa=None, n_xa=0, ya=None, n_ya=0, part_stride=0,
                   sl_n=0, sl_T=0, sl_x=0, sl_y=0, sl_id=(),
                   dw_hist=None, dw_w=None, dw_b=None, dw_gamma=None, dw_nw=None, dw_xout=None, dw_hnew=None,
-                  xsplit=None, unaligned_ok=(), w13_form=None, twin=None, twin2=None):
+                  xsplit=None, unaligned_ok=(), w13_form=None, twin=None, twin2=None, w13_exact=False):
         ldx = K if ldx is None else ldx
         ldy = N if ldy is None else ldy
         xs = self.cfg.xsplit if xsplit is None else xsplit
@@ -828,6 +828,8 @@
         need("w2p", w2p, wbytes, torch.uint8, required=epi == self.EPI_SWIGLU)
         if w13_form is None and (twin is not None or twin2 is not None):
             raise ValueError("gemv_case: twins without w13_form")
+        if w13_exact and twin is None:
+            raise ValueError("gemv_case: w13_exact without twins")
         if twin is not None or twin2 is not None:
             tbytes = int(self.lib.vv_w13_twin_bytes(N, K))
             if tbytes == 0:
@@ -888,7 +890,7 @@
             mr, wpb = (int(v) for v in w13_form)
             if xs != 1 or T > mr:
                 raise ValueError(f"gemv_case: the W13 form ({mr}, {wpb}) takes xsplit 1 and T <= {mr}")
-            rc = self.lib.vv_w13_gemv_case(self._s, C.byref(a), p(twin), p(twin2), mr, wpb)
+            rc = self.lib.vv_w13_gemv_case_exact(self._s, C.byref(a), p(twin), p(twin2), mr, wpb, 1 if w13_exact else 0)
             if rc == _lib.GEMV_REFUSED:
                 return None
             if rc != 0:
```
